# flash4242/Promptable-Counterfactual-GAN

Measured on AMD Instinct MI355X. Metric: images/sec (G+D step) MNIST-28 cDCGAN bs512 @1/2/4/8 MI355X; % MFMA roofline, higher is better.
Workload: dtype f32

## Files before the change

### include/pcgan_hip.h

```cpp
#ifndef PCGAN_HIP_H
#define PCGAN_HIP_H

#include <stddef.h>
#include <stdint.h>

#ifdef __cplusplus
extern "C" {
#endif

typedef void* pcg_stream_t;

typedef enum pcg_status {
  PCG_OK = 0,
  PCG_ERR_INVALID = -1,
  PCG_ERR_WORKSPACE = -2,
  PCG_ERR_LAUNCH = -3,
  PCG_ERR_UNSUPPORTED = -4
} pcg_status;

typedef enum pcg_act {
  PCG_ACT_NONE = 0,
  PCG_ACT_RELU = 1,
  PCG_ACT_LRELU = 2,
  PCG_ACT_TANH = 3,
// ... 96 lines not shown

size_t pcg_bn_workspace_bytes(int64_t rows, int32_t C);
int pcg_bn_train_stats(const float* x, int64_t rows, int32_t C, float eps, float momentum,
                       float* save_mean, float* save_invstd, float* running_mean, float* running_var,
                       int64_t* num_batches_tracked ,
                       void* workspace, size_t workspace_bytes, pcg_stream_t stream);
int pcg_bn_train_stats_coef(const float* x, int64_t rows, int32_t C, float eps, float momentum,
                            float* save_mean, float* save_invstd, float* running_mean, float* running_var,
                            int64_t* num_batches_tracked, const float* gamma, const float* beta, float* coef_out,
                            void* workspace, size_t workspace_bytes, pcg_stream_t stream);
int pcg_bn_apply_act(const float* x, int64_t rows, int32_t C, const float* mean, const float* invstd_or_var,
                     float var_eps, const float* gamma, const float* beta, int act, float slope,
                     const float* residual , float alpha ,
                     float* y, pcg_stream_t stream);
int pcg_bn_act_bwd(const float* dy, const float* x, const float* y , int64_t rows, int32_t C,
                   const float* mean, const float* invstd, const float* gamma,
                   int act, float slope, float dy_scale ,
                   float* dx, float* dgamma, float* dbeta, int accumulate,
                   void* workspace, size_t workspace_bytes, pcg_stream_t stream);
int pcg_bn_act_bwd_premask(const float* dy, const float* x, int64_t rows, int32_t C, const float* mean, const float* invstd,
                           const float* gamma, const float* beta, int act, float slope, float dy_scale, float* dx, float* dgamma,
                           float* dbeta, int accumulate, void* workspace, size_t workspace_bytes, pcg_stream_t stream);

size_t pcg_bn_bwd_partial_workspace_bytes(int32_t C);
int pcg_bn_bwd_partial(const float* dm, const float* x, int64_t rows, int32_t C, const float* mean, const float* invstd,
                       const float* gamma, const void* partial, int32_t nparts, float* dx, float* dgamma, float* dbeta,
                       int accumulate, void* workspace, size_t workspace_bytes, pcg_stream_t stream);

size_t pcg_bn_db_workspace_bytes(int64_t rows, int32_t C);
int pcg_bn_act_bwd_db(const float* dy, const float* x, const float* y , int64_t rows, int32_t C, const float* mean,
                      const float* invstd, const float* gamma, const float* beta , int act, float slope, float dy_scale,
                      float* dx, float* dgamma, float* dbeta, int accumulate, float* dcol, int accumulate_col, void* workspace,
                      size_t workspace_bytes, pcg_stream_t stream);
size_t pcg_bn_bwd_partial_db_workspace_bytes(int32_t C);
int pcg_bn_bwd_partial_db(const float* dm, const float* x, int64_t rows, int32_t C, const float* mean, const float* invstd,
                          const float* gamma, const void* partial, int32_t nparts, float dm_scale, float* dx, float* dgamma,
                          float* dbeta, int accumulate, float* dcol , int accumulate_col, void* workspace,
                          size_t workspace_bytes, pcg_stream_t stream);

int pcg_conv2d_fwd_bn_g(const pcg_conv_geom* g, const float* x, const float* w, const float* bias , float* y, float eps,
                        float momentum, float* save_mean , float* save_invstd ,
                        float* running_mean , float* running_var , int64_t* num_batches_tracked ,
                        int32_t groups, void* workspace , size_t workspace_bytes, pcg_stream_t stream);
int pcg_bn_apply_act_g(const float* x, int64_t rows, int32_t C, const float* mean , const float* invstd ,
                       const float* gamma, const float* beta, int act, float slope, float* y, int32_t groups, pcg_stream_t stream);
int32_t pcg_conv2d_dgrad_bn_phases(const pcg_conv_geom* g);
int pcg_conv2d_dgrad_bnbwd_g(const pcg_conv_geom* g, const float* dy, const float* w, const float* z_below, const float* mean,
                             const float* invstd, const float* gamma, const float* beta, int act, float slope, float* dx,
                             void* partial, size_t partial_bytes, int32_t groups, pcg_stream_t stream);
size_t pcg_bn_bwd_partial_g_workspace_bytes(int32_t C, int32_t groups);
int pcg_bn_bwd_partial_g(const float* dm, const float* x, int64_t rows, int32_t C, const float* mean, const float* invstd,
                         const float* gamma, const void* partial, int32_t nparts, int32_t nphases, float* dx, float* dgamma,
                         float* dbeta, int accumulate, int32_t groups, void* workspace, size_t workspace_bytes, pcg_stream_t stream);
size_t pcg_bn_act_bwd_g_workspace_bytes(int64_t rows, int32_t C, int32_t groups);
int pcg_bn_act_bwd_premask_g(const float* dy, const float* x, int64_t rows, int32_t C, const float* mean, const float* invstd,
                             const float* gamma, const float* beta, int act, float slope, float* dx, float* dgamma, float* dbeta,
                             int accumulate, int32_t groups, void* workspace, size_t workspace_bytes, pcg_stream_t stream);

int32_t pcg_conv2d_fwd_bnbwd_thin_ok(const pcg_conv_geom* g);
size_t pcg_conv2d_fwd_bnbwd_thin_workspace_bytes(const pcg_conv_geom* g);
int pcg_conv2d_fwd_bnbwd_thin(const pcg_conv_geom* g, const float* x, const float* w, const float* z_below, const float* mean,
                              const float* invstd, const float* gamma, const float* beta, int act, float slope, float* dz,
                              float* dgamma , float* dbeta , int accumulate, void* workspace,
                              size_t workspace_bytes, pcg_stream_t stream);
int32_t pcg_conv2d_dgrad_bnbwd_full_ok(const pcg_conv_geom* g, int32_t groups);
size_t pcg_conv2d_dgrad_bnbwd_full_workspace_bytes(const pcg_conv_geom* g, int32_t groups);
int pcg_conv2d_dgrad_bnbwd_full(const pcg_conv_geom* g, const float* dy, const float* w, const float* z_below, const float* mean,
                                const float* invstd, const float* gamma, const float* beta, int act, float slope, float* dz,
                                float* dgamma , float* dbeta , int accumulate, int32_t groups, void* workspace,
                                size_t workspace_bytes, pcg_stream_t stream);

int32_t pcg_conv2d_bnin_full_ok(const pcg_conv_geom* g, int32_t groups);
int pcg_conv2d_fwd_bnin_full(const pcg_conv_geom* g, const float* z, const float* mean, const float* invstd, const float* gamma,
                             const float* beta, int in_act, float in_slope, int32_t groups, const float* w, const float* bias ,
                             int act, float slope, float* y, pcg_stream_t stream);
int pcg_conv2d_wgrad_bnin_full(const pcg_conv_geom* g, const float* z, const float* mean, const float* invstd, const float* gamma,
                               const float* beta, int in_act, float in_slope, int32_t groups, const float* dy, float* dw, int accumulate,
                               void* workspace, size_t workspace_bytes, pcg_stream_t stream);

int pcg_act_fwd(const float* x, int64_t n, int act, float slope, float* y, pcg_stream_t stream);
int pcg_act_bwd(const float* dy, const float* y, int64_t n, int act, float slope, float* dx, pcg_stream_t stream);

int pcg_bce_fwd_bwd(const float* p, const float* target , float target_const,
                    int64_t n, float grad_scale, const float* grad_out_dev ,
                    float* loss , float* dp , pcg_stream_t stream);
int pcg_bce_pair(const float* p, int64_t n_half, float target0, float target1, const float* g0_dev ,
                 const float* g1_dev , const float* g2_dev , float* loss3 , float* dp ,
                 pcg_stream_t stream);
int pcg_bce_logits_fwd_bwd(const float* z, float target_const, int64_t n, float grad_scale,
                           const float* grad_out_dev , float* loss , float* dz ,
                           pcg_stream_t stream);

int pcg_adam_step(float* param, const float* grad, float* exp_avg, float* exp_avg_sq, int64_t n,
                  double lr, double beta1, double beta2, double eps, double weight_decay, int decoupled_wd,
                  int64_t step, pcg_stream_t stream);

int pcg_adam_step_capturable(float* param, const float* grad, float* exp_avg, float* exp_avg_sq, int64_t n,
                             double lr, double beta1, double beta2, double eps, double weight_decay, int decoupled_wd,
                             int64_t* step_counter_dev, float* hyper_scratch2_dev, pcg_stream_t stream);

int pcg_embed_concat_fwd(const float* x, const int64_t* idx, const float* table, const float* mask ,
                         float* out, int32_t B, int32_t HW, int32_t C, int32_t K, pcg_stream_t stream);
int pcg_embed_concat_bwd(const float* dinp, const int64_t* idx, float* dtable , float* dx ,
                         int32_t B, int32_t HW, int32_t C, int32_t K, int accumulate, pcg_stream_t stream);
int pcg_embed_table_grad(const float* dinp, const int64_t* idx, float* dtable, int32_t B, int32_t HW, int32_t C, int32_t ch, int32_t K,
                         int accumulate, pcg_stream_t stream);
// ... 688 lines not shown
```

### promptable-counterfactual-gan_amd/_lib.py

```python
import ctypes
import os

import torch

_HERE = os.path.dirname(os.path.abspath(__file__))
LIB_PATH = os.environ.get("PCG_LIB") or os.path.join(_HERE, "libpcgan_hip.so")

PCG_OK = 0
ACT_NONE, ACT_RELU, ACT_LRELU, ACT_TANH, ACT_SIGMOID = 0, 1, 2, 3, 4
(PLAN_GEMM_ACT, PLAN_GEMM, PLAN_LINEAR_WGRAD, PLAN_LINEAR_WGRAD_GROUPED, PLAN_MEAN, PLAN_ABS_MEAN, PLAN_CROSS_ENTROPY,
 PLAN_EMBED_CONCAT_BWD, PLAN_ACT, PLAN_ELEMENTWISE, PLAN_BN_COLREDUCE, PLAN_BN_APPLY, PLAN_BN_FINALIZE, PLAN_INSTNORM,
 PLAN_SPECTRAL_NORM) = range(15)
PLAN_EW_TABULAR, PLAN_EW_CF_OPS, PLAN_EW_POINTWISE, PLAN_EW_GATHER_CHANNEL = range(4)


class PcgError(RuntimeError):
    pass


class ConvGeom(ctypes.Structure):

    _fields_ = [(n, ctypes.c_int32) for n in ("B", "IH", "IW", "Cin", "OH", "OW", "Cout", "KH", "KW", "stride", "pad")]

    def key(self):
        return tuple(getattr(self, n) for n, _ in self._fields_)


_I, _P = ctypes.c_int32, ctypes.c_void_p


class HouseGDesc(ctypes.Structure):
    _fields_ = ([("fc_in_w", _I), ("fc_in_b", _I)] +
                [(n, _I * 5) for n in ("fc1_w", "fc1_b", "bn1_g", "bn1_b", "fc2_w", "fc2_b", "bn2_g", "bn2_b",
                                       "film_gamma_w", "film_gamma_b", "film_beta_w", "film_beta_b")] +
                [("cont_w", _I), ("cont_b", _I), ("head_w", _I * 8), ("head_b", _I * 8), ("seg", _I * 9)] +
                [(n, _I) for n in ("nheads", "ncont", "D", "NC", "hidden", "nblocks")])


class WgradItem(ctypes.Structure):
    _fields_ = [("dy", _P), ("x", _P), ("dW", _P), ("db", _P)] + [(n, _I) for n in ("ldy", "ldx", "O", "I", "accumulate_w", "accumulate_b",
                                                                                      "tile_x", "tile_y")]


class HouseGFwdArgs(ctypes.Structure):
    _fields_ = ([(n, _P) for n in ("params", "x", "onehot", "mask", "noise", "inp", "H", "Z1", "Z2", "P", "SM")] +
                [("running_mean", _P * 10), ("running_var", _P * 10), ("num_batches_tracked", _P * 10)] +
                [(n, _P) for n in ("cont", "logits", "soft", "hard")] + [("B", ctypes.c_int32)] +
                [(n, ctypes.c_float) for n in ("eps", "momentum", "tau", "res_scale")])


class HouseGBwdArgs(ctypes.Structure):
    _fields_ = ([(n, _P) for n in ("params", "grads", "onehot", "mask", "H", "Z1", "Z2", "SM", "soft", "d_cont", "d_logits", "d_samples",
                                   "DH", "DZ1", "DZ2", "A1", "DN1", "DG", "DB", "DZIN", "DL", "DC", "Q")] +
                [("B", ctypes.c_int32), ("accumulate", ctypes.c_int32), ("tau", ctypes.c_float), ("res_scale", ctypes.c_float)])


class InXform(ctypes.Structure):
    _fields_ = [("scale", _P), ("shift", _P), ("act", _I), ("slope", ctypes.c_float)]


class MoonsCfDesc(ctypes.Structure):
    _fields_ = ([(n, _I) for n in ("hidden", "clf_hidden", "B", "N", "nG", "nD", "nC", "nG_adam", "nD_adam")] +
                [("g_off", _I * 14), ("d_off", _I * 8), ("c_off", _I * 6)] +
                [(n, ctypes.c_double) for n in ("lr_G", "lr_D", "beta1", "beta2", "adam_eps")] +
                [(n, ctypes.c_float) for n in ("bn_eps", "bn_momentum", "sn_eps", "slope", "lambda_cls", "lambda_l1", "lambda_l2",
                                               "lambda_mask")])


class MoonsCfTrainArgs(ctypes.Structure):
    _fields_ = ([(n, _P) for n in ("X", "Y", "rows", "target_y", "mask", "g_flat", "d_flat", "c_flat", "g_exp_avg", "g_exp_avg_sq", "g_step",
                                   "d_exp_avg", "d_exp_avg_sq", "d_step")] +
                [("bn_mean", _P * 3), ("bn_var", _P * 3), ("bn_nbt", _P * 3), ("sn_u", _P * 4), ("sn_v", _P * 4)] +
                [("logs", _P), ("scratch", _P), ("scratch_bytes", ctypes.c_size_t)])


class MoonsCfFwdArgs(ctypes.Structure):
    _fields_ = ([(n, _I) for n in ("which", "train", "B")] + [(n, _P) for n in ("x", "onehot", "mask", "params")] +
                [("bn_mean", _P * 3), ("bn_var", _P * 3), ("bn_nbt", _P * 3), ("sn_u", _P * 4), ("sn_v", _P * 4)] +
                [("out0", _P), ("out1", _P), ("scratch", _P), ("scratch_bytes", ctypes.c_size_t)])


class MoonsCfEvalArgs(ctypes.Structure):
    _fields_ = ([("N", ctypes.c_int64), ("M", _I), ("T", _I), ("group", _I)] +
                [(n, _P) for n in ("x", "y", "masks", "target", "row_mask", "g_flat", "c_flat")] + [("bn_mean", _P * 3), ("bn_var", _P * 3)] +
                [(n, _P) for n in ("raw", "masked", "x_cf", "logits_cf", "logits_x", "pred_cf", "pred_x", "gain", "sums")])


class HouseCfEvalArgs(ctypes.Structure):
    _fields_ = ([("N", ctypes.c_int64)] + [(n, _I) for n in ("T", "group", "clamp_cls", "mask_rows")] + [("g_flat", _P), ("nG", _I)] +
                [("bn_mean", _P * 10), ("bn_var", _P * 10)] + [(n, ctypes.c_float) for n in ("bn_eps", "tau", "res_scale")] +
                [("col_src", _I * 17), ("norm_vals", _P), ("c_w_kmajor", ctypes.POINTER(ctypes.c_void_p)), ("c_bias", ctypes.POINTER(ctypes.c_void_p))] +
                [(n, _P) for n in ("x", "y", "target", "mask", "noise", "cont", "logits", "chosen", "masked", "x_cf", "x_cf_raw", "logits_cf",
                                   "logits_x", "pred_cf", "pred_x", "gain", "tile_sums", "class_sums", "class_counts")])


class PatchMaskBitsArgs(ctypes.Structure):
    _fields_ = [("bits", _P), ("mask", _P)] + [(n, _I) for n in ("n", "H", "W", "ps")]


class MnistCfEntryArgs(ctypes.Structure):
    _fields_ = [(n, _P) for n in ("x", "table", "mask", "target", "out")] + [(n, _I) for n in ("B", "T", "HW", "K", "mask_mode", "q0", "nq")]


class MnistCfTailArgs(ctypes.Structure):
    _fields_ = ([(n, _P) for n in ("c", "x", "mask", "x_cf", "raw", "masked", "sums")] + [("scale", ctypes.c_float)] +
                [(n, _I) for n in ("B", "T", "HW", "mask_mode", "q0", "nq")])

# ... 95 lines not shown
class DeltaGanEntryArgs(ctypes.Structure):
    _fields_ = ([(n, _P) for n in ("x", "y", "target", "y_host", "target_host", "table_g", "table_d", "g_in", "d_in", "labels_2b", "head_w",
                                   "head_w_packed")] + [(n, _I) for n in ("B", "HW", "K", "mode", "head_C", "head_P")])


class DeltaGanTailFwdArgs(ctypes.Structure):
    _fields_ = ([(n, _P) for n in ("x", "delta", "x_cf", "d_in", "loss_reg", "workspace")] + [("workspace_bytes", ctypes.c_size_t)] +
                [(n, _I) for n in ("B", "HW", "grid")])


class LogitHeadFwdArgs(ctypes.Structure):
    _fields_ = [(n, _P) for n in ("a", "w", "bias", "logits", "loss", "dlogit", "db", "workspace")] + [(n, _I) for n in ("R", "F", "mode")]


class LogitHeadBwdArgs(ctypes.Structure):
    _fields_ = [(n, _P) for n in ("a", "w", "dlogit", "da", "dw")] + [("slope", _F)] + [(n, _I) for n in ("R", "F", "dw_C", "dw_P")]


class DeltaGanTailBwdArgs(ctypes.Structure):
    _fields_ = ([(n, _P) for n in ("dD", "dC", "delta", "d_delta")] + [("lambda_cls", _F), ("reg_scale", _F)] +
                [(n, _I) for n in ("B", "HW", "dD_stride")])


class DeltaCfEntryArgs(ctypes.Structure):
    _fields_ = [(n, _P) for n in ("x", "table", "target", "target_host", "out")] + [(n, _I) for n in ("B", "T", "HW", "K", "q0", "nq")]


class DeltaCfTailArgs(ctypes.Structure):
    _fields_ = [(n, _P) for n in ("delta", "x", "x_cf", "sums")] + [(n, _I) for n in ("B", "T", "HW", "q0", "nq")]


class DeltaGanTargetDrawArgs(ctypes.Structure):
    _fields_ = [("target", _P), ("counter", _P), ("seed", ctypes.c_uint64), ("offset", ctypes.c_uint64), ("B", _I), ("K", _I)]


class ProbHeadFwdArgs(ctypes.Structure):
    _fields_ = ([(n, _P) for n in ("a", "w", "bias", "logits", "prob", "loss", "dlogit", "db", "workspace")] +
                [("workspace_bytes", ctypes.c_size_t), ("eps", _F)] + [(n, _I) for n in ("R", "F", "mode", "slabs")])


class LogEpsLossArgs(ctypes.Structure):
    _fields_ = [(n, _P) for n in ("p", "grad_out", "loss", "dp")] + [("eps", _F), ("R", _I), ("mode", _I)]


DELTA_GAN_BUILD, DELTA_GAN_REGATHER = 0, 1
LOGIT_HEAD_D, LOGIT_HEAD_G = 0, 1
DELTA_GAN_CHUNK = 1024
PROB_HEAD_D, PROB_HEAD_G = 0, 1
PROB_HEAD_MAX_SLABS = 16
CLASS_PICK_FIRST, CLASS_PICK_BEST = 0, 1
CLASS_PICK_KMAX = 64
CF_PANELS_GRID, CF_PANELS_PANELS = 0, 1

STRUCTS = {"pcg_conv_geom": ConvGeom, "pcg_in_xform": InXform, "pcg_wgrad_item": WgradItem, "pcg_sn_fwd_batch": SnFwdBatch,
           "pcg_sn_bwd_batch": SnBwdBatch, "pcg_house_g_desc": HouseGDesc, "pcg_house_g_fwd_args": HouseGFwdArgs,
           "pcg_house_g_bwd_args": HouseGBwdArgs, "pcg_house_critic_fwd_args": HouseCriticFwdArgs,
           "pcg_house_critic_bwd_args": HouseCriticBwdArgs, "pcg_house_cls_fwd_args": HouseClsFwdArgs, "pcg_house_cls_bwd_args": HouseClsBwdArgs,
           "pcg_house_res_fwd_args": HouseResFwdArgs, "pcg_house_res_bwd_args": HouseResBwdArgs, "pcg_house_loss_args": HouseLossArgs,
           "pcg_house_diag_args": HouseDiagArgs, "pcg_moons_cf_desc": MoonsCfDesc, "pcg_moons_cf_train_args": MoonsCfTrainArgs,
           "pcg_moons_cf_fwd_args": MoonsCfFwdArgs, "pcg_moons_cf_eval_args": MoonsCfEvalArgs,
           "pcg_house_cf_eval_args": HouseCfEvalArgs, "pcg_patch_mask_bits_args": PatchMaskBitsArgs,
           "pcg_mnist_cf_entry_args": MnistCfEntryArgs, "pcg_mnist_cf_tail_args": MnistCfTailArgs,
           "pcg_mnist_cf_score_args": MnistCfScoreArgs, "pcg_dense_bn": DenseBn,
           "pcg_dense_bn_bwd": DenseBnBwd, "pcg_moons_gan_desc": MoonsGanDesc, "pcg_moons_gan_train_args": MoonsGanTrainArgs,
           "pcg_moons_gan_fwd_args": MoonsGanFwdArgs, "pcg_moons_clf_fit_desc": MoonsClfFitDesc,
           "pcg_moons_clf_fit_args": MoonsClfFitArgs, "pcg_delta_gan_entry_args": DeltaGanEntryArgs,
           "pcg_delta_gan_tail_fwd_args": DeltaGanTailFwdArgs, "pcg_logit_head_fwd_args": LogitHeadFwdArgs,
           "pcg_logit_head_bwd_args": LogitHeadBwdArgs, "pcg_delta_gan_tail_bwd_args": DeltaGanTailBwdArgs,
           "pcg_delta_cf_entry_args": DeltaCfEntryArgs, "pcg_delta_cf_tail_args": DeltaCfTailArgs,
           "pcg_delta_gan_target_draw_args": DeltaGanTargetDrawArgs, "pcg_prob_head_fwd_args": ProbHeadFwdArgs,
           "pcg_log_eps_loss_args": LogEpsLossArgs}

_c = ctypes
_vp, _f, _i, _i64, _sz = _c.c_void_p, _c.c_float, _c.c_int, _c.c_int64, _c.c_size_t
_d = _c.c_double
_i32 = _c.c_int32
_gp = _c.POINTER(ConvGeom)
_xp = _c.POINTER(InXform)

PROTOTYPES = {
    "pcg_abi_version": (_i, []),
    "pcg_abi_struct_bytes": (_sz, [_c.c_char_p]),
    "pcg_last_error": (_c.c_char_p, []),
    "pcg_target_arch": (_c.c_char_p, []),
    "pcg_tune_set": (_i, [_c.c_char_p, _i32]),
    "pcg_debug_stamp_buffer": (_i, [_vp, _i64]),
    "pcg_conv_plan_describe": (_i, [_c.POINTER(ConvGeom), _i32, _i32, _c.c_char_p, _sz]),
    "pcg_launch_plan_describe": (_i, [_i32, _c.POINTER(_i64), _i32, _c.c_char_p, _sz]),
    "pcg_conv_scratch_parts_bytes": (_sz, []),
    "pcg_conv_scratch_arrivals_bytes": (_sz, []),
    "pcg_conv_set_scratch": (_i, [_vp, _vp, _sz, _vp, _sz]),
    "pcg_conv_reset_scratch": (_i, [_vp]),
    "pcg_conv_pixtab_bytes": (_sz, [_gp]),
    "pcg_conv_pixtab_register": (_i, [_gp, _vp, _sz, _vp]),
    "pcg_conv_cliptab_bytes": (_sz, [_gp]),
    "pcg_conv_cliptab_register": (_i, [_gp, _vp, _sz, _vp]),
    "pcg_conv_sched_model": (_d, [_vp, _i32]),
    "pcg_conv_pad_clip_query": (_i, [_gp, _i32, _i32, _i32, _vp, _vp, _vp, _vp]),
    "pcg_conv2d_fwd_bn_g": (_i, [_gp, _vp, _vp, _vp, _vp, _f, _f, _vp, _vp, _vp, _vp, _vp, _i32, _vp, _sz, _vp]),
    "pcg_bn_apply_act_g": (_i, [_vp, _i64, _i32, _vp, _vp, _vp, _vp, _i, _f, _vp, _i32, _vp]),
    "pcg_conv2d_dgrad_bn_phases": (_i32, [_gp]),
    "pcg_conv2d_dgrad_bnbwd_g": (_i, [_gp, _vp, _vp, _vp, _vp, _vp, _vp, _vp, _i, _f, _vp, _vp, _sz, _i32, _vp]),
    "pcg_bn_bwd_partial_g_workspace_bytes": (_sz, [_i32, _i32]),
    "pcg_bn_bwd_partial_g": (_i, [_vp, _vp, _i64, _i32, _vp, _vp, _vp, _vp, _i32, _i32, _vp, _vp, _vp, _i, _i32, _vp, _sz, _vp]),
    "pcg_bn_act_bwd_g_workspace_bytes": (_sz, [_i64, _i32, _i32]),
    "pcg_bn_act_bwd_premask_g": (_i, [_vp, _vp, _i64, _i32, _vp, _vp, _vp, _vp, _i, _f, _vp, _vp, _vp, _i, _i32, _vp, _sz, _vp]),
    "pcg_bce_pair": (_i, [_vp, _i64, _f, _f, _vp, _vp, _vp, _vp, _vp, _vp]),
# ... 21 lines not shown
    "pcg_conv2d_dgrad": (_i, [_gp, _vp, _vp, _vp, _vp, _vp, _sz, _vp]),
    "pcg_conv2d_fwd_act": (_i, [_gp, _vp, _vp, _vp, _i, _f, _vp, _vp, _sz, _vp]),
    "pcg_conv2d_dgrad_act": (_i, [_gp, _vp, _vp, _vp, _i, _f, _vp, _vp, _sz, _vp]),
    "pcg_conv2d_fwd_bn_workspace_bytes": (_sz, [_gp]),
    "pcg_conv2d_dgrad_bn_workspace_bytes": (_sz, [_gp]),
    "pcg_conv2d_fwd_bn": (_i, [_gp, _vp, _vp, _vp, _vp, _f, _f, _vp, _vp, _vp, _vp, _vp, _vp, _sz, _vp]),
    "pcg_conv2d_dgrad_bn": (_i, [_gp, _vp, _vp, _vp, _vp, _f, _f, _vp, _vp, _vp, _vp, _vp, _vp, _sz, _vp]),
    "pcg_conv2d_dgrad_mask": (_i, [_gp, _vp, _vp, _vp, _i, _f, _vp, _vp, _sz, _vp]),
    "pcg_conv2d_dgrad_mask_thin_ok": (_i32, [_gp]),
    "pcg_conv2d_xf_thin_ok": (_i32, [_gp]),
    "pcg_conv2d_fwd_add_mask": (_i, [_gp, _vp, _vp, _vp, _vp, _i, _f, _vp, _vp]),
    "pcg_conv2d_dgrad_add_mask": (_i, [_gp, _vp, _vp, _vp, _vp, _i, _f, _vp, _vp]),
    "pcg_conv2d_fwd_mask": (_i, [_gp, _vp, _vp, _vp, _i, _f, _vp, _vp, _sz, _vp]),
    "pcg_conv2d_dgrad_bnbwd": (_i, [_gp, _vp, _vp, _vp, _vp, _vp, _vp, _vp, _i, _f, _vp, _vp, _sz, _vp]),
    "pcg_conv2d_fwd_bnbwd": (_i, [_gp, _vp, _vp, _vp, _vp, _vp, _vp, _vp, _i, _f, _vp, _vp, _sz, _vp]),
    "pcg_conv2d_dgrad_add": (_i, [_gp, _vp, _vp, _vp, _vp, _vp, _sz, _vp]),
    "pcg_conv2d_fwd_bn_partial_rows": (_c.c_int32, [_gp]),
    "pcg_conv2d_dgrad_bn_partial_rows": (_c.c_int32, [_gp]),
    "pcg_bn_bwd_partial_workspace_bytes": (_sz, [_c.c_int32]),
    "pcg_bn_bwd_partial": (_i, [_vp, _vp, _i64, _c.c_int32, _vp, _vp, _vp, _vp, _c.c_int32, _vp, _vp, _vp, _i, _vp, _sz, _vp]),
    "pcg_conv2d_fwd_bn_xf": (_i, [_gp, _vp, _xp, _vp, _vp, _vp, _f, _f, _vp, _vp, _vp, _vp, _vp, _vp, _vp, _vp, _vp, _sz, _vp]),
    "pcg_conv2d_dgrad_bn_xf": (_i, [_gp, _vp, _xp, _vp, _vp, _vp, _f, _f, _vp, _vp, _vp, _vp, _vp, _vp, _vp, _vp, _vp, _sz, _vp]),
    "pcg_conv2d_fwd_xf": (_i, [_gp, _vp, _xp, _vp, _vp, _i, _f, _vp, _vp, _sz, _vp]),
    "pcg_conv2d_dgrad_xf": (_i, [_gp, _vp, _xp, _vp, _vp, _i, _f, _vp, _vp, _sz, _vp]),
    "pcg_conv2d_wgrad_xf": (_i, [_gp, _vp, _xp, _vp, _xp, _vp, _i, _vp, _sz, _vp]),
    "pcg_bn_train_stats_coef": (_i, [_vp, _i64, _c.c_int32, _f, _f, _vp, _vp, _vp, _vp, _vp, _vp, _vp, _vp, _vp, _sz, _vp]),
    "pcg_bn_db_workspace_bytes": (_sz, [_i64, _c.c_int32]),
    "pcg_bn_act_bwd_db": (_i, [_vp, _vp, _vp, _i64, _c.c_int32, _vp, _vp, _vp, _vp, _i, _f, _f, _vp, _vp, _vp, _i, _vp, _i, _vp, _sz, _vp]),
    "pcg_bn_bwd_partial_db_workspace_bytes": (_sz, [_c.c_int32]),
    "pcg_bn_bwd_partial_db": (_i, [_vp, _vp, _i64, _c.c_int32, _vp, _vp, _vp, _vp, _c.c_int32, _f, _vp, _vp, _vp, _i, _vp, _i, _vp, _sz, _vp]),
    "pcg_conv2d_dgrad_add_bnsum": (_i, [_gp, _vp, _vp, _vp, _vp, _vp, _vp, _f, _vp, _vp, _sz, _vp]),
    "pcg_conv2d_fwd_add": (_i, [_gp, _vp, _vp, _vp, _vp, _vp, _sz, _vp]),
    "pcg_conv2d_fwd_add_bnsum": (_i, [_gp, _vp, _vp, _vp, _vp, _vp, _vp, _f, _vp, _vp, _sz, _vp]),
    "pcg_conv_weight_adjoint": (_i, [_vp, _vp, _i32, _i32, _i32, _i32, _vp]),
    "pcg_conv_weight_adjoint_many": (_i, [_vp, _vp, _i32, _i32, _i32, _i32, _i32, _vp]),
    "pcg_house_losses": (_i, [_vp, _vp, _vp, _i64, _vp, _vp, _vp, _f, _f, _f, _f, _vp, _vp]),
    "pcg_dp_unique_id": (_i, [_vp]),
    "pcg_dp_init": (_i, [_vp, _i32, _i32]),
    "pcg_dp_world": (_i32, []),
    "pcg_dp_rank": (_i32, []),
    "pcg_dp_side_stream": (_vp, []),
    "pcg_dp_allreduce": (_i, [_vp, _i64, _vp]),
    "pcg_dp_allreduce_begin": (_i, [_vp, _i64, _i32, _vp]),
    "pcg_dp_record": (_i, [_i32]),
    "pcg_dp_allreduce_wait": (_i, [_i32, _vp]),
    "pcg_dp_allreduce_sum_f64": (_i, [_vp, _i64, _vp]),
    "pcg_dp_broadcast": (_i, [_vp, _i64, _i32, _vp]),
    "pcg_dp_sync_batchnorm": (_i, [_i32]),
    "pcg_dp_barrier": (_i, [_vp]),
    "pcg_dp_rccl_version": (_i32, []),
    "pcg_dp_shutdown": (_i, []),
    "pcg_conv2d_wgrad_workspace_bytes": (_sz, [_gp]),
    "pcg_conv2d_wgrad": (_i, [_gp, _vp, _vp, _vp, _i, _vp, _sz, _vp]),
    "pcg_colsum_workspace_bytes": (_sz, [_i64, _c.c_int32]),
    "pcg_colsum": (_i, [_vp, _i64, _c.c_int32, _vp, _i, _vp, _sz, _vp]),
    "pcg_bn_workspace_bytes": (_sz, [_i64, _c.c_int32]),
    "pcg_bn_train_stats": (_i, [_vp, _i64, _c.c_int32, _f, _f, _vp, _vp, _vp, _vp, _vp, _vp, _sz, _vp]),
    "pcg_bn_apply_act": (_i, [_vp, _i64, _c.c_int32, _vp, _vp, _f, _vp, _vp, _i, _f, _vp, _f, _vp, _vp]),
    "pcg_bn_act_bwd": (_i, [_vp, _vp, _vp, _i64, _c.c_int32, _vp, _vp, _vp, _i, _f, _f, _vp, _vp, _vp, _i, _vp, _sz, _vp]),
    "pcg_bn_act_bwd_premask": (_i, [_vp, _vp, _i64, _c.c_int32, _vp, _vp, _vp, _vp, _i, _f, _f, _vp, _vp, _vp, _i, _vp, _sz, _vp]),
    "pcg_embed_concat_fwd": (_i, [_vp, _vp, _vp, _vp, _vp, _c.c_int32, _c.c_int32, _c.c_int32, _c.c_int32, _vp]),
    "pcg_embed_concat_bwd": (_i, [_vp, _vp, _vp, _vp, _c.c_int32, _c.c_int32, _c.c_int32, _c.c_int32, _i, _vp]),
    "pcg_embed_table_grad": (_i, [_vp, _vp, _vp, _i32, _i32, _i32, _i32, _i32, _i, _vp]),
    "pcg_gather_channel": (_i, [_vp, _vp, _i32, _i32, _i32, _vp]),
    "pcg_axpby": (_i, [_vp, _f, _vp, _f, _vp, _i64, _vp]),
    "pcg_scale_mask_fwd": (_i, [_vp, _vp, _f, _vp, _vp, _i64, _vp]),
    "pcg_scale_mask_bwd": (_i, [_vp, _vp, _vp, _f, _vp, _i64, _vp]),
    "pcg_clamp_add_fwd": (_i, [_vp, _vp, _f, _f, _vp, _i64, _vp]),
    "pcg_clamp_add_bwd": (_i, [_vp, _vp, _vp, _f, _f, _vp, _i64, _vp]),
    "pcg_abs_mean_workspace_bytes": (_sz, []),
    "pcg_abs_mean_fwd": (_i, [_vp, _vp, _i, _i64, _vp, _vp, _sz, _vp]),
    "pcg_abs_mean_bwd": (_i, [_vp, _vp, _i, _i64, _vp, _f, _vp, _i, _vp]),
    "pcg_avgpool_fwd": (_i, [_vp, _vp, _c.c_int32, _c.c_int32, _c.c_int32, _vp]),
    "pcg_avgpool_bwd": (_i, [_vp, _vp, _c.c_int32, _c.c_int32, _c.c_int32, _vp]),
    "pcg_cross_entropy_fwd_bwd": (_i, [_vp, _vp, _c.c_int32, _c.c_int32, _f, _vp, _vp, _vp, _vp]),
    "pcg_act_fwd": (_i, [_vp, _i64, _i, _f, _vp, _vp]),
    "pcg_act_bwd": (_i, [_vp, _vp, _i64, _i, _f, _vp, _vp]),
    "pcg_bce_fwd_bwd": (_i, [_vp, _vp, _f, _i64, _f, _vp, _vp, _vp, _vp]),
    "pcg_bce_logits_fwd_bwd": (_i, [_vp, _f, _i64, _f, _vp, _vp, _vp, _vp]),
    "pcg_adam_step": (_i, [_vp, _vp, _vp, _vp, _i64, _d, _d, _d, _d, _d, _i, _i64, _vp]),
    "pcg_adam_step_capturable": (_i, [_vp, _vp, _vp, _vp, _i64, _d, _d, _d, _d, _d, _i, _vp, _vp, _vp]),
    "pcg_patch_mask": (_i, [_vp, _c.c_int32, _c.c_int32, _c.c_int32, _c.c_int32, _c.c_int32, _c.c_uint64, _c.c_uint64, _vp]),
    "pcg_randint": (_i, [_vp, _i64, _c.c_int32, _c.c_int32, _vp, _c.c_uint64, _c.c_uint64, _vp]),
    "pcg_randn": (_i, [_vp, _i64, _f, _f, _c.c_uint64, _c.c_uint64, _vp]),
    "pcg_fill": (_i, [_vp, _i64, _f, _vp]),
    "pcg_add_bias_rows": (_i, [_vp, _i64, _i32, _vp, _vp]),
    "pcg_sumsq": (_i, [_vp, _i64, _vp, _i, _vp]),
    "pcg_norm_sum": (_i, [_vp, _vp, _i32, _vp, _vp]),
    "pcg_instnorm_fwd": (_i, [_vp, _i32, _i32, _i32, _vp, _vp, _f, _i, _f, _vp, _vp, _vp, _vp]),
    "pcg_instnorm_bwd": (_i, [_vp, _vp, _i32, _i32, _i32, _vp, _vp, _vp, _vp, _vp, _vp, _vp]),
    "pcg_instnorm_bwd_bwd": (_i, [_vp, _vp, _vp, _i32, _i32, _i32, _vp, _vp, _vp, _vp, _vp, _vp, _vp]),
    "pcg_instnorm_bwd_fused": (_i, [_vp, _vp, _f, _vp, _i32, _i32, _i32, _vp, _vp, _vp, _vp, _vp, _vp, _vp, _vp, _vp, _vp]),
    "pcg_instnorm_bwd_bwd_act": (_i, [_vp, _vp, _vp, _i32, _i32, _i32, _vp, _vp, _vp, _vp, _f, _vp, _vp, _vp, _vp]),
    "pcg_rowsum3": (_i, [_i32, _vp, _vp, _i, _vp, _vp, _i, _vp, _vp, _i, _i32, _i32, _vp]),
    "pcg_nhwc_to_nchw_flat": (_i, [_vp, _vp, _i32, _i32, _i32, _i, _vp]),
    "pcg_interpolate": (_i, [_vp, _vp, _vp, _vp, _i32, _i32, _vp]),
    "pcg_interpolate_stack": (_i, [_vp, _vp, _vp, _vp, _i32, _i32, _vp]),
    "pcg_gradient_penalty_fwd": (_i, [_vp, _i32, _i32, _f, _vp, _vp, _vp]),
    "pcg_gradient_penalty_bwd": (_i, [_vp, _vp, _vp, _i32, _i32, _f, _vp, _vp]),
    "pcg_rand_uniform": (_i, [_vp, _i64, _c.c_uint64, _c.c_uint64, _vp]),
    "pcg_cross_entropy_weighted_fwd_bwd": (_i, [_vp, _vp, _vp, _i32, _i32, _f, _vp, _vp, _vp, _vp]),
    "pcg_dropout_apply": (_i, [_vp, _vp, _i64, _i32, _i32, _f, _vp, _vp]),
    "pcg_rand_bernoulli": (_i, [_vp, _i64, _f, _c.c_uint64, _c.c_uint64, _vp]),
    "pcg_resize8_normalize": (_i, [_vp, _i32, _i32, _i32, _i32, _i32, _vp, _vp, _i32, _vp, _vp, _i32, _f, _f, _vp, _vp]),
    "pcg_house_g_fwd": (_i, [_c.POINTER(HouseGDesc), _c.POINTER(HouseGFwdArgs), _vp]),
    "pcg_house_g_bwd": (_i, [_c.POINTER(HouseGDesc), _c.POINTER(HouseGBwdArgs), _vp]),
# ... 124 lines not shown
```

### promptable-counterfactual-gan_amd/csrc/batchnorm.hip

```cpp
#include "pcg_common.h"
#include "launch_plan.h"
#include <cstdlib>

namespace pcg {
bool dp_sync_bn();
int dp_world();
int dp_allreduce_f64(double* buf, int64_t n, hipStream_t s);

namespace {

constexpr int CR_THREADS = 256;
constexpr int CR_MAX_BLOCKS = 512;
constexpr int FIN_CH = 8, FIN_SL = 128;
static inline int fin_threads(int nparts) { return nparts <= 1024 ? FIN_CH * 32 : FIN_CH * FIN_SL; }

struct ColPlan { int vec, CG, TX, TY, nblocks, rows_per_block; };

ColPlan plan_cols(int64_t rows, int C, bool aligned16) {
  ColPlan p;
  p.vec = (C % 4 == 0 && aligned16) ? 4 : 1;
  p.CG = C / p.vec;
  int tx = 1;
  while (tx * 2 <= p.CG && tx * 2 <= CR_THREADS) tx *= 2;
  p.TX = tx;
  p.TY = CR_THREADS / tx;
  int64_t rpb = ceil_div64(rows, CR_MAX_BLOCKS);
  const int64_t min_rpb = (int64_t)p.TY * 4;
  if (rpb < min_rpb) rpb = min_rpb;
  p.rows_per_block = (int)rpb;
  p.nblocks = (int)ceil_div64(rows, rpb);
  if (p.nblocks < 1) p.nblocks = 1;
  return p;
}

template <int VEC>
__device__ __forceinline__ void ldv(const float* p, size_t idx, float (&v)[VEC]) {
  if constexpr (VEC == 4) {
    const float4 q = *reinterpret_cast<const float4*>(p + idx);
    v[0] = q.x; v[1] = q.y; v[2] = q.z; v[3] = q.w;
  } else {
    v[0] = p[idx];
  }
}
struct FnStats {
  static constexpr int NVAL = 2;
  const float* x;
  template <int VEC>
  __device__ __forceinline__ void eval(size_t idx, int c0, double (&o)[2][VEC]) const {
    (void)c0;
    float v[VEC];
    ldv<VEC>(x, idx, v);
#pragma unroll
    for (int e = 0; e < VEC; ++e) { o[0][e] = (double)v[e]; o[1][e] = (double)v[e] * (double)v[e]; }
  }
// ... 305 lines not shown
      float sc, sh;
      bn_fold(gamma ? gamma[c] : 1.f, beta ? beta[c] : 0.f, mean[c], is, sc, sh);
      v[e] = fmaf(alpha, act_apply(fmaf(v[e], sc, sh), act, slope), rs[e]);
    }
    if constexpr (VEC == 4) reinterpret_cast<float4*>(y)[i] = make_float4(v[0], v[1], v[2], v[3]);
    else y[i] = v[0];
  }
}

template <int VEC>
__global__ void __launch_bounds__(256) bn_bwd_apply_kernel(const float* __restrict__ dy, const float* __restrict__ x,
                                                           const float* __restrict__ y, size_t n, int C,
                                                           const float* __restrict__ mean, const float* __restrict__ invstd,
                                                           const float* __restrict__ coef, int act, float slope,
                                                           float dy_scale, float* __restrict__ dx, const float* __restrict__ gamma,
                                                           const float* __restrict__ beta) {
  const size_t nv = n / VEC;
  for (size_t i = (size_t)blockIdx.x * blockDim.x + threadIdx.x; i < nv; i += (size_t)gridDim.x * blockDim.x) {
    const int c0 = (int)((i * VEC) % (size_t)C);
    float g[VEC], xv[VEC], yv[VEC];
    if constexpr (VEC == 4) {
      const float4 a = reinterpret_cast<const float4*>(dy)[i];
      const float4 b = reinterpret_cast<const float4*>(x)[i];
      const float4 c = (act != PCG_ACT_NONE && y) ? reinterpret_cast<const float4*>(y)[i] : make_float4(1.f, 1.f, 1.f, 1.f);
      g[0] = a.x; g[1] = a.y; g[2] = a.z; g[3] = a.w;
      xv[0] = b.x; xv[1] = b.y; xv[2] = b.z; xv[3] = b.w;
      yv[0] = c.x; yv[1] = c.y; yv[2] = c.z; yv[3] = c.w;
    } else {
      g[0] = dy[i]; xv[0] = x[i]; yv[0] = (act != PCG_ACT_NONE && y) ? y[i] : 1.f;
    }
#pragma unroll
    for (int e = 0; e < VEC; ++e) {
      const int c = c0 + e;
      if (act != PCG_ACT_NONE && !y) { float sc, sh; bn_fold(gamma[c], beta[c], mean[c], invstd[c], sc, sh); yv[e] = fmaf(xv[e], sc, sh); }
      const float dz = dy_scale * g[e] * (act != PCG_ACT_NONE ? act_grad_from_out(yv[e], act, slope) : 1.f);
      const float xh = (xv[e] - mean[c]) * invstd[c];
      g[e] = coef[c] * (dz - coef[C + c] - xh * coef[2 * C + c]);
    }
    if constexpr (VEC == 4) reinterpret_cast<float4*>(dx)[i] = make_float4(g[0], g[1], g[2], g[3]);
    else dx[i] = g[0];
  }
}

struct BnTune { int blocks, depth, nt; size_t nt_bytes; };
static const BnTune& bn_tune() {
  static const BnTune t = [] {
    auto env = [](const char* k, int d) { const char* e = getenv(k); return e ? atoi(e) : d; };
    return BnTune{env("PCG_BN_BLOCKS", 4096), env("PCG_BN_DEPTH", 2), env("PCG_BN_NT", -1), (size_t)env("PCG_BN_NT_MB", 160) * 1000000u};
  }();
  return t;
}
static bool bn_use_nt(size_t n4) { const BnTune& t = bn_tune(); return t.nt < 0 ? n4 * 16 >= t.nt_bytes : t.nt != 0; }
static int bn_apply_depth() { return bn_tune().depth == 4 ? 4 : 2; }
template <bool NT>
__device__ __forceinline__ void bn_store4(float4* at, const float4& v) {
  typedef float nt_f32x4 __attribute__((ext_vector_type(4)));
  if constexpr (NT) __builtin_nontemporal_store(nt_f32x4{v.x, v.y, v.z, v.w}, reinterpret_cast<nt_f32x4*>(at)); else *at = v;
}

template <int DEPTH, bool NT>
__global__ void __launch_bounds__(256) bn_apply_act_fast_kernel(const float4* __restrict__ x, size_t n4, int C,
                                                                const float* __restrict__ mean, const float* __restrict__ invstd,
                                                                float var_eps, const float* __restrict__ gamma,
                                                                const float* __restrict__ beta, int act, float slope,
                                                                const float4* __restrict__ residual, float alpha,
                                                                float4* __restrict__ y, size_t group_n4) {
  if (group_n4) {
    const size_t g = blockIdx.y;
    x += g * group_n4; y += g * group_n4; if (residual) residual += g * group_n4;
    mean += g * C; invstd += g * C; n4 = group_n4;
  }
  const size_t gtid = (size_t)blockIdx.x * 256 + threadIdx.x, stride = (size_t)gridDim.x * 256;
  const int c0 = (int)(gtid % (size_t)(C >> 2)) * 4;
  float sc[4], sh[4];
#pragma unroll
  for (int e = 0; e < 4; ++e) {
    const int c = c0 + e;
    const float is = var_eps >= 0.f ? 1.f / sqrtf(invstd[c] + var_eps) : invstd[c];
    bn_fold(gamma ? gamma[c] : 1.f, beta ? beta[c] : 0.f, mean[c], is, sc[e], sh[e]);
  }
  auto one = [&](float4 q, float4 r) {
    q.x = fmaf(alpha, act_apply(fmaf(q.x, sc[0], sh[0]), act, slope), r.x);
    q.y = fmaf(alpha, act_apply(fmaf(q.y, sc[1], sh[1]), act, slope), r.y);
    q.z = fmaf(alpha, act_apply(fmaf(q.z, sc[2], sh[2]), act, slope), r.z);
    q.w = fmaf(alpha, act_apply(fmaf(q.w, sc[3], sh[3]), act, slope), r.w);
    return q;
  };
  const float4 zero = make_float4(0.f, 0.f, 0.f, 0.f);
  auto put = [&](size_t at, const float4& v) { bn_store4<NT>(y + at, v); };
  size_t i = gtid;
  for (; i + (DEPTH - 1) * stride < n4; i += DEPTH * stride) {
    float4 q[DEPTH], r[DEPTH];
#pragma unroll
    for (int j = 0; j < DEPTH; ++j) { q[j] = x[i + j * stride]; r[j] = residual ? residual[i + j * stride] : zero; }
#pragma unroll
    for (int j = 0; j < DEPTH; ++j) put(i + j * stride, one(q[j], r[j]));
  }
  for (; i < n4; i += stride) put(i, one(x[i], residual ? residual[i] : zero));
}
template <class... A>
static void launch_bn_apply_fast(dim3 grid, hipStream_t s, size_t n4_all, A... a) {
  const int depth = bn_apply_depth();
  const bool nt = bn_use_nt(n4_all);
  if (depth == 4 && nt) hipLaunchKernelGGL((bn_apply_act_fast_kernel<4, true>), grid, dim3(256), 0, s, a...);
  else if (depth == 4) hipLaunchKernelGGL((bn_apply_act_fast_kernel<4, false>), grid, dim3(256), 0, s, a...);
  else if (nt) hipLaunchKernelGGL((bn_apply_act_fast_kernel<2, true>), grid, dim3(256), 0, s, a...);
  else hipLaunchKernelGGL((bn_apply_act_fast_kernel<2, false>), grid, dim3(256), 0, s, a...);
}

template <bool NT>
__global__ void __launch_bounds__(256) bn_bwd_apply_fast_kernel(const float4* __restrict__ dy, const float4* __restrict__ x,
                                                                const float4* __restrict__ y, size_t n4, int C,
                                                                const float* __restrict__ mean, const float* __restrict__ invstd,
                                                                const float* __restrict__ coef, int act, float slope,
                                                                float dy_scale, float4* __restrict__ dx, const float* __restrict__ gamma,
                                                                const float* __restrict__ beta, double* __restrict__ colpart,
                                                                size_t group_n4) {
  if (group_n4) {
    const size_t g = blockIdx.y;
    dy += g * group_n4; x += g * group_n4; dx += g * group_n4; if (y) y += g * group_n4;
    mean += g * C; invstd += g * C; coef += g * 3 * C; n4 = group_n4;
  }
  const size_t gtid = (size_t)blockIdx.x * 256 + threadIdx.x, stride = (size_t)gridDim.x * 256;
  const int c0 = (int)(gtid % (size_t)(C >> 2)) * 4;
  float mu[4], is[4], k0[4], k1[4], k2[4], msc[4], msh[4];
  double cs[4] = {0.0, 0.0, 0.0, 0.0};
  const bool premask = act != PCG_ACT_NONE && y == nullptr;
#pragma unroll
  for (int e = 0; e < 4; ++e) {
    const int c = c0 + e;
    mu[e] = mean[c]; is[e] = invstd[c]; k0[e] = coef[c]; k1[e] = coef[C + c]; k2[e] = coef[2 * C + c];
    msc[e] = 0.f; msh[e] = 0.f;
    if (premask) bn_fold(gamma[c], beta[c], mean[c], invstd[c], msc[e], msh[e]);
  }
  const bool has_act = act != PCG_ACT_NONE;
  auto one = [&](float4 g, float4 xv, float4 yv) {
    float gg[4] = {g.x, g.y, g.z, g.w}, xx[4] = {xv.x, xv.y, xv.z, xv.w}, yy[4] = {yv.x, yv.y, yv.z, yv.w};
#pragma unroll
    for (int e = 0; e < 4; ++e) {
      if (premask) yy[e] = fmaf(xx[e], msc[e], msh[e]);
      const float grad = has_act ? act_grad_from_out(yy[e], act, slope) : 1.f;
      const float xh = (xx[e] - mu[e]) * is[e];
      gg[e] = k0[e] * fmaf(-xh, k2[e], fmaf(dy_scale * gg[e], grad, -k1[e]));
    }
    return make_float4(gg[0], gg[1], gg[2], gg[3]);
  };
  const float4 ones = make_float4(1.f, 1.f, 1.f, 1.f);
  auto tally = [&](const float4& v) { cs[0] += (double)v.x; cs[1] += (double)v.y; cs[2] += (double)v.z; cs[3] += (double)v.w; };
  size_t i = gtid;
  for (; i + stride < n4; i += 2 * stride) {
    const float4 g0 = dy[i], g1 = dy[i + stride], x0 = x[i], x1 = x[i + stride];
    const float4 y0 = (has_act && !premask) ? y[i] : ones, y1 = (has_act && !premask) ? y[i + stride] : ones;
    const float4 o0 = one(g0, x0, y0), o1 = one(g1, x1, y1);
    bn_store4<NT>(dx + i, o0);
    bn_store4<NT>(dx + i + stride, o1);
    if (colpart) { tally(o0); tally(o1); }
  }
  if (i < n4) {
    const float4 o = one(dy[i], x[i], (has_act && !premask) ? y[i] : ones);
    bn_store4<NT>(dx + i, o);
    if (colpart) tally(o);
  }
  if (colpart) {
    __shared__ double red[4][256];
#pragma unroll
    for (int e = 0; e < 4; ++e) red[e][threadIdx.x] = cs[e];
    __syncthreads();
    const int nq = C >> 2;
    if ((int)threadIdx.x < nq) {
#pragma unroll
      for (int e = 0; e < 4; ++e) {
        double sum = 0.0;
        for (int t = threadIdx.x; t < 256; t += nq) sum += red[e][t];
        colpart[(size_t)blockIdx.x * C + 4 * threadIdx.x + e] = sum;
      }
    }
  }
}

template <class... A>
static void launch_bn_bwd_apply_fast(dim3 grid, hipStream_t s, size_t n4_all, A... a) {
  if (bn_use_nt(n4_all)) hipLaunchKernelGGL((bn_bwd_apply_fast_kernel<true>), grid, dim3(256), 0, s, a...);
  else hipLaunchKernelGGL((bn_bwd_apply_fast_kernel<false>), grid, dim3(256), 0, s, a...);
}

bool fast_channels(int C) { return C % 4 == 0 && C / 4 <= 256 && ((C / 4) & (C / 4 - 1)) == 0; }

template <class Fn>
int launch_colreduce(const Fn& fn, int64_t rows, int C, const ColPlan& cp, double* partial, hipStream_t s) {
  if (cp.vec == 4)
    hipLaunchKernelGGL((colreduce_kernel<4, Fn>), dim3(cp.nblocks), dim3(CR_THREADS), 0, s, fn, rows, C, cp.CG, cp.TX, cp.TY,
                       cp.rows_per_block, partial);
  else
    hipLaunchKernelGGL((colreduce_kernel<1, Fn>), dim3(cp.nblocks), dim3(CR_THREADS), 0, s, fn, rows, C, cp.CG, cp.TX, cp.TY,
                       cp.rows_per_block, partial);
  return launch_status("colreduce_kernel");
}

unsigned ew_blocks(size_t nv) {
  size_t b = (nv + 255) / 256;
  if (b > 8192) b = 8192;
  if (b < 1) b = 1;
  return (unsigned)b;
}

bool al16(const void* p) { return ((uintptr_t)p & 15) == 0; }

constexpr int COL_MAX_BLOCKS = 4096;
constexpr int COL_SUM_BLOCKS = 1024;
enum { BN_PASS_APPLY = 0, BN_PASS_BWD = 1, BN_PASS_BWD_COLSUM = 2 };
enum { BN_LANES_FAST = 0, BN_LANES_FLOAT4 = 1, BN_LANES_SCALAR = 2 };
struct ApplyPlan { int lanes, depth; bool nt; unsigned blocks; };
ApplyPlan plan_apply(int pass, int64_t rows, int C, bool aligned) {
  const size_t n = (size_t)rows * C;
  if (fast_channels(C) && aligned) {
    const unsigned cap = pass == BN_PASS_APPLY ? (unsigned)bn_tune().blocks : pass == BN_PASS_BWD_COLSUM ? COL_SUM_BLOCKS : COL_MAX_BLOCKS;
    unsigned blocks = (unsigned)((n / 4 + 511) / 512);
    if (blocks > cap) blocks = cap;
    if (blocks < 1) blocks = 1;
    return ApplyPlan{BN_LANES_FAST, pass == BN_PASS_APPLY ? bn_apply_depth() : 2, bn_use_nt(n / 4), blocks};
  }
  if (C % 4 == 0 && aligned) return ApplyPlan{BN_LANES_FLOAT4, 1, false, ew_blocks(n / 4)};
  return ApplyPlan{BN_LANES_SCALAR, 1, false, ew_blocks(n)};
}

}
}

namespace pcg {
size_t bn_partial_buffer_bytes(int nparts, int C) {
  const PrePlan q = plan_presum(nparts);
  return (presum_offset(nparts, 2 * C) + (size_t)q.nchunks * 2 * C + 4 * (size_t)C) * sizeof(double);
}
int launch_bn_bwd_finalize(const double* partial, int nblocks, int64_t rows, int C, const float* gamma, const float* invstd, float* coef,
                           float* dgamma, float* dbeta, int accumulate, hipStream_t s) {
  PCG_REQUIRE(!dp_sync_bn(), "fused thin BatchNorm backward: not available in the exact global-batch mode");
  hipLaunchKernelGGL(bn_bwd_finalize_kernel<double>, dim3((C + FIN_CH - 1) / FIN_CH), dim3(fin_threads(nblocks)), 0, s, partial, nblocks, C,
                     1.0 / (double)rows, gamma, invstd, coef, dgamma, dbeta, accumulate, (const double*)nullptr);
  return launch_status("bn_bwd_finalize_kernel");
}
int launch_bn_bwd_finalize_g(const double* partial, int rows_per_group, int groups, int64_t rows_g, int C, const float* gamma, const float* invstd,
                             float* coef, float* dgamma, float* dbeta, int accumulate, hipStream_t s) {
  PCG_REQUIRE(!dp_sync_bn(), "fused thin BatchNorm backward: not available in the exact global-batch mode");
  hipLaunchKernelGGL(bn_bwd_finalize_g_kernel<double>, dim3((C + FIN_CH - 1) / FIN_CH), dim3(fin_threads(rows_per_group)), 0, s, partial,
                     rows_per_group, groups, rows_per_group, rows_per_group * groups, C, 1.0 / (double)rows_g, gamma, invstd, coef, dgamma, dbeta,
                     accumulate);
  return launch_status("bn_bwd_finalize_g_kernel");
}
int launch_bn_stats_finalize(const double* partial, int nparts, int64_t rows, int C, float eps, float momentum, float* save_mean,
                             float* save_invstd, float* running_mean, float* running_var, int64_t* nbt, hipStream_t s,
                             bool has_presum_tail, const float* gamma, const float* beta, float* coef) {
  int nchunks = 0;
  const double* pre = has_presum_tail ? launch_presum(partial, nparts, 2 * C, &nchunks, s) : nullptr;
  if (dp_sync_bn()) {
    PCG_REQUIRE(has_presum_tail, "exact BatchNorm: buffer without scratch tail");
    double* scratch = const_cast<double*>(partial) + presum_offset(nparts, 2 * C) + (size_t)plan_presum(nparts).nchunks * 2 * C;
    if (int e = sync_exchange(pre ? pre : partial, pre ? nchunks : nparts, C, scratch, s)) return e;
    partial = scratch + 2 * C; nparts = 1; pre = nullptr;
    rows *= dp_world();
  }
  const double unbias = rows > 1 ? (double)rows / (double)(rows - 1) : 1.0;
  if (pre)
    hipLaunchKernelGGL(bn_stats_finalize_kernel<double>, dim3((C + FIN_CH - 1) / FIN_CH), dim3(fin_threads(nchunks)), 0, s, pre, nchunks, C,
                       1.0 / (double)rows, unbias, eps, momentum, save_mean, save_invstd, running_mean, running_var, nbt, gamma, beta, coef);
  else
    hipLaunchKernelGGL(bn_stats_finalize_kernel<double>, dim3((C + FIN_CH - 1) / FIN_CH), dim3(fin_threads(nparts)), 0, s, partial, nparts, C,
                       1.0 / (double)rows, unbias, eps, momentum, save_mean, save_invstd, running_mean, running_var, nbt, gamma, beta, coef);
  return launch_status("bn_stats_finalize_kernel");
}
}

using namespace pcg;

extern "C" size_t pcg_bn_workspace_bytes(int64_t rows, int32_t C) {
  if (rows <= 0 || C <= 0) return 0;
  const ColPlan a = plan_cols(rows, C, true), b = plan_cols(rows, C, false);
  const int nb = a.nblocks > b.nblocks ? a.nblocks : b.nblocks;
  return ((size_t)nb * 2 * C + 4 * (size_t)C) * sizeof(double) + 3 * (size_t)C * sizeof(float);
}
// ... 99 lines not shown
    launch_bn_bwd_apply_fast(dim3(blocks), s, n / 4, reinterpret_cast<const float4*>(dy),
                             reinterpret_cast<const float4*>(x), reinterpret_cast<const float4*>(y), n / 4, C, mean, invstd,
                             (const float*)coef, act, slope, dy_scale, reinterpret_cast<float4*>(dx), gamma, beta, fused_col ? colpart : (double*)nullptr,
                             (size_t)0);
    if (fused_col) {
      if (int e = launch_status("bn_bwd_apply_kernel")) return e;
      hipLaunchKernelGGL(colsum_finalize_kernel, dim3((C + FIN_CH - 1) / FIN_CH), dim3(fin_threads((int)blocks)), 0, s, (const double*)colpart,
                         (int)blocks, C, dcol, accumulate_col);
      return launch_status("colsum_finalize_kernel");
    }
  } else if (ap.lanes == BN_LANES_FLOAT4)
    hipLaunchKernelGGL(bn_bwd_apply_kernel<4>, dim3(ap.blocks), dim3(256), 0, s, dy, x, y, n, C, mean, invstd,
                       (const float*)coef, act, slope, dy_scale, dx, gamma, beta);
  else
    hipLaunchKernelGGL(bn_bwd_apply_kernel<1>, dim3(ap.blocks), dim3(256), 0, s, dy, x, y, n, C, mean, invstd,
                       (const float*)coef, act, slope, dy_scale, dx, gamma, beta);
  if (int e = launch_status("bn_bwd_apply_kernel")) return e;
  if (dcol) {
    const ColPlan cq = plan_cols(rows, C, al16(dx));
    FnSum fs{dx};
    if (int e = launch_colreduce(fs, rows, C, cq, partial, s)) return e;
    hipLaunchKernelGGL(colsum_finalize_kernel, dim3((C + FIN_CH - 1) / FIN_CH), dim3(fin_threads(cq.nblocks)), 0, s, (const double*)partial, cq.nblocks, C,
                       dcol, accumulate_col);
    return launch_status("colsum_finalize_kernel");
  }
  return PCG_OK;
}

extern "C" int pcg_bn_act_bwd(const float* dy, const float* x, const float* y, int64_t rows, int32_t C, const float* mean,
                              const float* invstd, const float* gamma, int act, float slope, float dy_scale, float* dx,
                              float* dgamma, float* dbeta, int accumulate, void* workspace, size_t workspace_bytes,
                              pcg_stream_t stream) {
  PCG_REQUIRE(y || act == PCG_ACT_NONE, "pcg_bn_act_bwd: y is required with an activation (or use pcg_bn_act_bwd_premask)");
  return bn_act_bwd_impl(dy, x, y, rows, C, mean, invstd, gamma, nullptr, act, slope, dy_scale, dx, dgamma, dbeta, accumulate, workspace,
                         workspace_bytes, stream);
}

extern "C" int pcg_bn_act_bwd_premask(const float* dy, const float* x, int64_t rows, int32_t C, const float* mean, const float* invstd,
                                      const float* gamma, const float* beta, int act, float slope, float dy_scale, float* dx,
                                      float* dgamma, float* dbeta, int accumulate, void* workspace, size_t workspace_bytes,
                                      pcg_stream_t stream) {
  return bn_act_bwd_impl(dy, x, nullptr, rows, C, mean, invstd, gamma, beta, act, slope, dy_scale, dx, dgamma, dbeta, accumulate, workspace,
                         workspace_bytes, stream);
}

extern "C" size_t pcg_bn_bwd_partial_workspace_bytes(int32_t C) { return (size_t)3 * C * sizeof(float); }
extern "C" size_t pcg_bn_bwd_partial_db_workspace_bytes(int32_t C) {
  return C > 0 ? (((size_t)3 * C * sizeof(float) + 7) & ~(size_t)7) + (size_t)4096 * C * sizeof(double) : 0;
}

static int bn_bwd_partial_impl(const float* dm, const float* x, int64_t rows, int32_t C, const float* mean, const float* invstd,
                               const float* gamma, const void* partial_, int32_t nparts, float* dx, float* dgamma, float* dbeta,
                               int accumulate, void* workspace, size_t workspace_bytes, pcg_stream_t stream, float* dcol,
                               int accumulate_col, float dm_scale = 1.f) {
  const double* partial = static_cast<const double*>(partial_);
  PCG_REQUIRE(!dcol || workspace_bytes >= pcg_bn_bwd_partial_db_workspace_bytes(C),
              "pcg_bn_bwd_partial_db: workspace smaller than pcg_bn_bwd_partial_db_workspace_bytes");
  PCG_REQUIRE(dm && x && mean && invstd && partial && dx && rows > 0 && C > 0 && nparts > 0, "pcg_bn_bwd_partial: bad arguments");
  PCG_REQUIRE(((uintptr_t)partial & 7) == 0, "pcg_bn_bwd_partial: the partial-sum buffer must be 8-byte aligned");
  if (!workspace || workspace_bytes < pcg_bn_bwd_partial_workspace_bytes(C)) {
    set_error("pcg_bn_bwd_partial: workspace %zu B < required %zu B", workspace_bytes, pcg_bn_bwd_partial_workspace_bytes(C));
    return PCG_ERR_WORKSPACE;
  }
  hipStream_t s = (hipStream_t)stream;
  float* coef = (float*)workspace;
  int nchunks = 0;
  const double* pre = launch_presum(partial, nparts, 2 * C, &nchunks, s);
  const double* src = pre ? pre : partial;
  const double* local = nullptr;
  int nsrc = pre ? nchunks : nparts;
  int64_t rows_all = rows;
  if (dp_sync_bn()) {
    double* scratch = const_cast<double*>(partial) + presum_offset(nparts, 2 * C) + (size_t)plan_presum(nparts).nchunks * 2 * C;
    if (int e = sync_exchange(src, nsrc, C, scratch, s)) return e;
    src = scratch + 2 * C; nsrc = 1; local = scratch;
    rows_all = rows * dp_world();
  }
  hipLaunchKernelGGL(bn_bwd_finalize_kernel<double>, dim3((C + FIN_CH - 1) / FIN_CH), dim3(fin_threads(nsrc)), 0, s, src, nsrc, C,
                     1.0 / (double)rows_all, gamma, invstd, coef, dgamma, dbeta, accumulate, local);
  if (int e = launch_status("bn_bwd_finalize_kernel")) return e;
  const bool aligned = al16(dm) && al16(x) && al16(dx);
  const size_t n = (size_t)rows * C;
  double* colpart = reinterpret_cast<double*>(reinterpret_cast<char*>(workspace) + (((size_t)3 * C * sizeof(float) + 7) & ~(size_t)7));
  const ApplyPlan ap = plan_apply(dcol ? BN_PASS_BWD_COLSUM : BN_PASS_BWD, rows, C, aligned);
  if (ap.lanes == BN_LANES_FAST) {
    const unsigned blocks = ap.blocks;
    launch_bn_bwd_apply_fast(dim3(blocks), s, n / 4, reinterpret_cast<const float4*>(dm),
                             reinterpret_cast<const float4*>(x), (const float4*)nullptr, n / 4, C, mean, invstd, (const float*)coef, (int)PCG_ACT_NONE,
                             0.f, dm_scale, reinterpret_cast<float4*>(dx), gamma, (const float*)nullptr, dcol ? colpart : (double*)nullptr, (size_t)0);
    if (int e = launch_status("bn_bwd_apply_kernel")) return e;
    if (dcol) {
      hipLaunchKernelGGL(colsum_finalize_kernel, dim3((C + FIN_CH - 1) / FIN_CH), dim3(fin_threads((int)blocks)), 0, s, (const double*)colpart,
                         (int)blocks, C, dcol, accumulate_col);
      return launch_status("colsum_finalize_kernel");
    }
    return PCG_OK;
  } else if (ap.lanes == BN_LANES_FLOAT4)
    hipLaunchKernelGGL(bn_bwd_apply_kernel<4>, dim3(ap.blocks), dim3(256), 0, s, dm, x, (const float*)nullptr, n, C, mean, invstd,
                       (const float*)coef, PCG_ACT_NONE, 0.f, dm_scale, dx, gamma, (const float*)nullptr);
  else
    hipLaunchKernelGGL(bn_bwd_apply_kernel<1>, dim3(ap.blocks), dim3(256), 0, s, dm, x, (const float*)nullptr, n, C, mean, invstd,
                       (const float*)coef, PCG_ACT_NONE, 0.f, dm_scale, dx, gamma, (const float*)nullptr);
  if (int e = launch_status("bn_bwd_apply_kernel")) return e;
  if (dcol) {
    const ColPlan cq = plan_cols(rows, C, al16(dx));
    FnSum fs{dx};
    if (int e = launch_colreduce(fs, rows, C, cq, colpart, s)) return e;
    hipLaunchKernelGGL(colsum_finalize_kernel, dim3((C + FIN_CH - 1) / FIN_CH), dim3(fin_threads(cq.nblocks)), 0, s, (const double*)colpart, cq.nblocks, C,
                       dcol, accumulate_col);
    return launch_status("colsum_finalize_kernel");
  }
  return PCG_OK;
}

extern "C" int pcg_bn_bwd_partial(const float* dm, const float* x, int64_t rows, int32_t C, const float* mean, const float* invstd,
                                  const float* gamma, const void* partial, int32_t nparts, float* dx, float* dgamma, float* dbeta,
                                  int accumulate, void* workspace, size_t workspace_bytes, pcg_stream_t stream) {
  return bn_bwd_partial_impl(dm, x, rows, C, mean, invstd, gamma, partial, nparts, dx, dgamma, dbeta, accumulate, workspace, workspace_bytes,
                             stream, nullptr, 0);
}
extern "C" int pcg_bn_bwd_partial_db(const float* dm, const float* x, int64_t rows, int32_t C, const float* mean, const float* invstd,
                                     const float* gamma, const void* partial, int32_t nparts, float dm_scale, float* dx, float* dgamma,
                                     float* dbeta, int accumulate, float* dcol, int accumulate_col, void* workspace,
                                     size_t workspace_bytes, pcg_stream_t stream) {
  return bn_bwd_partial_impl(dm, x, rows, C, mean, invstd, gamma, partial, nparts, dx, dgamma, dbeta, accumulate, workspace, workspace_bytes,
                             stream, dcol, accumulate_col, dm_scale);
}
extern "C" size_t pcg_bn_db_workspace_bytes(int64_t rows, int32_t C) {
  return rows > 0 && C > 0 ? ((pcg_bn_workspace_bytes(rows, C) + 7) & ~(size_t)7) + colpart_bytes(C) : 0;
}
extern "C" int pcg_bn_act_bwd_db(const float* dy, const float* x, const float* y, int64_t rows, int32_t C, const float* mean,
                                 const float* invstd, const float* gamma, const float* beta, int act, float slope, float dy_scale, float* dx,
                                 float* dgamma, float* dbeta, int accumulate, float* dcol, int accumulate_col, void* workspace,
                                 size_t workspace_bytes, pcg_stream_t stream) {
  PCG_REQUIRE(dcol != nullptr, "pcg_bn_act_bwd_db: null column-sum output");
  return bn_act_bwd_impl(dy, x, y, rows, C, mean, invstd, gamma, beta, act, slope, dy_scale, dx, dgamma, dbeta, accumulate, workspace,
                         workspace_bytes, stream, dcol, accumulate_col);
}

namespace pcg {
int launch_bn_stats_finalize_g(const double* partial, int nparts, int nphases, int groups, int64_t rows_per_group, int C, float eps,
                               float momentum, float* save_mean, float* save_invstd, float* running_mean, float* running_var,
                               int64_t* nbt, hipStream_t s) {
  PCG_REQUIRE(!dp_sync_bn(), "grouped BatchNorm: not available in the exact global-batch mode (pcg_dp_sync_batchnorm)");
  PCG_REQUIRE(groups >= 1 && nphases >= 1 && nparts % (nphases * groups) == 0, "grouped BatchNorm: %d partial rows do not split into %d phases x %d groups", nparts, nphases, groups);
  int per_phase = nparts / nphases, seg = per_phase / groups;
  const GroupPre gp = launch_presum_g(&partial, nparts, 2 * C, &per_phase, &seg, s);
  (void)gp;
  const int rpg = seg * nphases;
  const double unbias = rows_per_group > 1 ? (double)rows_per_group / (double)(rows_per_group - 1) : 1.0;
  hipLaunchKernelGGL(bn_stats_finalize_g_kernel<double>, dim3((C + FIN_CH - 1) / FIN_CH), dim3(fin_threads(rpg)), 0, s, partial, rpg, groups,
                     seg, per_phase, C, 1.0 / (double)rows_per_group, unbias, eps, momentum, save_mean, save_invstd, running_mean, running_var, nbt);
  return launch_status("bn_stats_finalize_g_kernel");
}
}

static bool grouped_shape_ok(int64_t rows, int32_t C, int32_t groups) {
  return groups >= 1 && groups <= 8 && rows > 0 && rows % groups == 0 && fast_channels(C);
}
static unsigned grouped_apply_blocks(size_t n4_group) {
  unsigned blocks = (unsigned)((n4_group + 511) / 512);
  if (blocks > (unsigned)bn_tune().blocks) blocks = (unsigned)bn_tune().blocks;
  return blocks < 1 ? 1 : blocks;
}

extern "C" int pcg_bn_apply_act_g(const float* x, int64_t rows, int32_t C, const float* mean, const float* invstd, const float* gamma,
                                  const float* beta, int act, float slope, float* y, int32_t groups, pcg_stream_t stream) {
  PCG_REQUIRE(x && y && mean && invstd, "pcg_bn_apply_act_g: null pointer");
  PCG_REQUIRE(grouped_shape_ok(rows, C, groups) && al16(x) && al16(y),
              "pcg_bn_apply_act_g: needs rows %% groups == 0, C / 4 a power of two <= 256 and 16-byte aligned tensors (rows %lld, C %d, groups %d)",
              (long long)rows, C, groups);
  const size_t n4g = (size_t)(rows / groups) * C / 4;
  launch_bn_apply_fast(dim3(grouped_apply_blocks(n4g), groups), (hipStream_t)stream, n4g * groups,
                       reinterpret_cast<const float4*>(x), n4g, C, mean, invstd, -1.f, gamma, beta, act, slope, (const float4*)nullptr, 1.f,
                       reinterpret_cast<float4*>(y), n4g);
  return launch_status("bn_apply_act_fast_kernel");
}

extern "C" size_t pcg_bn_bwd_partial_g_workspace_bytes(int32_t C, int32_t groups) { return (size_t)3 * C * groups * sizeof(float); }

static int launch_bwd_finalize_apply_g(const float* dm, const float* x, int64_t rows, int32_t C, const float* mean, const float* invstd,
                                       const float* gamma, const float* beta, int act, float slope, const double* partial, int rpg, int seg,
                                       int seg_stride, float* dx, float* dgamma, float* dbeta, int accumulate, int32_t groups, float* coef,
                                       hipStream_t s) {
  const int64_t rows_g = rows / groups;
  hipLaunchKernelGGL(bn_bwd_finalize_g_kernel<double>, dim3((C + FIN_CH - 1) / FIN_CH), dim3(fin_threads(rpg)), 0, s, partial, rpg, groups, seg,
                     seg_stride, C, 1.0 / (double)rows_g, gamma, invstd, coef, dgamma, dbeta, accumulate);
  if (int e = launch_status("bn_bwd_finalize_g_kernel")) return e;
  const size_t n4g = (size_t)rows_g * C / 4;
  launch_bn_bwd_apply_fast(dim3(grouped_apply_blocks(n4g), groups), s, n4g * groups, reinterpret_cast<const float4*>(dm),
                           reinterpret_cast<const float4*>(x), (const float4*)nullptr, n4g, C, mean, invstd, (const float*)coef, act, slope, 1.f,
                           reinterpret_cast<float4*>(dx), gamma, beta, (double*)nullptr, n4g);
  return launch_status("bn_bwd_apply_fast_kernel");
}

extern "C" int pcg_bn_bwd_partial_g(const float* dm, const float* x, int64_t rows, int32_t C, const float* mean, const float* invstd,
                                    const float* gamma, const void* partial_, int32_t nparts, int32_t nphases, float* dx, float* dgamma,
                                    float* dbeta, int accumulate, int32_t groups, void* workspace, size_t workspace_bytes, pcg_stream_t stream) {
  const double* partial = static_cast<const double*>(partial_);
  PCG_REQUIRE(dm && x && mean && invstd && partial && dx && nparts > 0 && nphases > 0, "pcg_bn_bwd_partial_g: bad arguments");
  PCG_REQUIRE(grouped_shape_ok(rows, C, groups) && al16(dm) && al16(x) && al16(dx) && ((uintptr_t)partial & 7) == 0,
              "pcg_bn_bwd_partial_g: needs rows %% groups == 0, C / 4 a power of two <= 256 and aligned tensors (rows %lld, C %d, groups %d)",
              (long long)rows, C, groups);
  PCG_REQUIRE(nparts % (nphases * groups) == 0, "pcg_bn_bwd_partial_g: %d partial rows do not split into %d phases x %d groups", nparts, nphases, groups);
  PCG_REQUIRE(!dp_sync_bn(), "pcg_bn_bwd_partial_g: not available in the exact global-batch mode");
  if (!workspace || workspace_bytes < pcg_bn_bwd_partial_g_workspace_bytes(C, groups)) {
    set_error("pcg_bn_bwd_partial_g: workspace %zu B < required %zu B", workspace_bytes, pcg_bn_bwd_partial_g_workspace_bytes(C, groups));
    return PCG_ERR_WORKSPACE;
  }
  int per_phase = nparts / nphases, seg = per_phase / groups;
  (void)launch_presum_g(&partial, nparts, 2 * C, &per_phase, &seg, (hipStream_t)stream);
  return launch_bwd_finalize_apply_g(dm, x, rows, C, mean, invstd, gamma, nullptr, PCG_ACT_NONE, 0.f, partial, seg * nphases, seg, per_phase, dx,
                                     dgamma, dbeta, accumulate, groups, (float*)workspace, (hipStream_t)stream);
}

extern "C" size_t pcg_bn_act_bwd_g_workspace_bytes(int64_t rows, int32_t C, int32_t groups) {
  if (rows <= 0 || C <= 0 || groups <= 0 || rows % groups) return 0;
  const ColPlan a = plan_cols(rows / groups, C, true);
  return ((size_t)groups * a.nblocks * 2 * C) * sizeof(double) + (size_t)3 * C * groups * sizeof(float);
}
extern "C" int pcg_bn_act_bwd_premask_g(const float* dy, const float* x, int64_t rows, int32_t C, const float* mean, const float* invstd,
                                        const float* gamma, const float* beta, int act, float slope, float* dx, float* dgamma, float* dbeta,
                                        int accumulate, int32_t groups, void* workspace, size_t workspace_bytes, pcg_stream_t stream) {
  PCG_REQUIRE(dy && x && mean && invstd && gamma && beta && dx, "pcg_bn_act_bwd_premask_g: null pointer");
  PCG_REQUIRE(act == PCG_ACT_NONE || act == PCG_ACT_RELU || act == PCG_ACT_LRELU, "pcg_bn_act_bwd_premask_g: activation %d is not none / ReLU / LeakyReLU", act);
  PCG_REQUIRE(grouped_shape_ok(rows, C, groups) && al16(dy) && al16(x) && al16(dx) && ((rows / groups) * C) % 4 == 0,
              "pcg_bn_act_bwd_premask_g: needs rows %% groups == 0, C / 4 a power of two <= 256 and aligned tensors (rows %lld, C %d, groups %d)",
              (long long)rows, C, groups);
  PCG_REQUIRE(!dp_sync_bn(), "pcg_bn_act_bwd_premask_g: not available in the exact global-batch mode");
  const size_t need = pcg_bn_act_bwd_g_workspace_bytes(rows, C, groups);
  if (!workspace || workspace_bytes < need) { set_error("pcg_bn_act_bwd_premask_g: workspace %zu B < required %zu B", workspace_bytes, need); return PCG_ERR_WORKSPACE; }
  hipStream_t s = (hipStream_t)stream;
  const int64_t rows_g = rows / groups;
  const ColPlan cp = plan_cols(rows_g, C, true);
  double* partial = (double*)workspace;
  float* coef = reinterpret_cast<float*>(partial + (size_t)groups * cp.nblocks * 2 * C);
  for (int g = 0; g < groups; ++g) {
    const size_t off = (size_t)g * rows_g * C;
    FnBnBwd fn{dy + off, x + off, nullptr, mean + (size_t)g * C, invstd + (size_t)g * C, act, slope, 1.f, gamma, beta};
    if (int e = launch_colreduce(fn, rows_g, C, cp, partial + (size_t)g * cp.nblocks * 2 * C, s)) return e;
  }
  return launch_bwd_finalize_apply_g(dy, x, rows, C, mean, invstd, gamma, beta, act, slope, partial, cp.nblocks, cp.nblocks, cp.nblocks * groups,
                                     dx, dgamma, dbeta, accumulate, groups, coef, s);
}

extern "C" int pcg_colsum(const float* dy, int64_t rows, int32_t C, float* db, int accumulate, void* workspace,
                          size_t workspace_bytes, pcg_stream_t stream) {
  PCG_REQUIRE(dy && db && rows > 0 && C > 0, "pcg_colsum: bad arguments");
  if (!workspace || workspace_bytes < pcg_colsum_workspace_bytes(rows, C)) {
    set_error("pcg_colsum: workspace %zu B < required %zu B", workspace_bytes, pcg_colsum_workspace_bytes(rows, C));
    return PCG_ERR_WORKSPACE;
  }
  hipStream_t s = (hipStream_t)stream;
  const ColPlan cp = plan_cols(rows, C, al16(dy));
  double* partial = (double*)workspace;
  FnSum fn{dy};
  if (int e = launch_colreduce(fn, rows, C, cp, partial, s)) return e;
  hipLaunchKernelGGL(colsum_finalize_kernel, dim3((C + FIN_CH - 1) / FIN_CH), dim3(fin_threads(cp.nblocks)), 0, s, (const double*)partial, cp.nblocks, C, db, accumulate);
  return launch_status("colsum_finalize_kernel");
}

int pcg::describe_batchnorm_plan(int32_t op, const int64_t* a, int32_t n_args, char* buf, size_t bytes) {
  switch (op) {
    case PCG_PLAN_BN_COLREDUCE: {
      PCG_REQUIRE(n_args == 3 && a[0] > 0 && a[1] > 0 && a[1] <= INT32_MAX, "pcg_launch_plan_describe: bn_colreduce takes (rows, C, aligned)");
      const ColPlan p = plan_cols(a[0], (int)a[1], a[2] != 0);
// ... 37 lines not shown
```

### promptable-counterfactual-gan_amd/csrc/conv_igemm.hip

```cpp
#include <string.h>
#include <array>
#include <map>
#include <mutex>
#include "conv_loaders.h"
#include "conv_pixtab.h"
#include "conv_cliptab.h"
#include "thin_conv.h"

namespace pcg {
namespace {

__device__ __forceinline__ int wave_id() { return __builtin_amdgcn_readfirstlane((int)(threadIdx.x >> 6)); }

__device__ __forceinline__ void prio_entry(const ConvP& p) { if (p.edge_prio & 1) __builtin_amdgcn_s_setprio(3); }
__device__ __forceinline__ void prio_epilogue(const ConvP& p) { if (p.edge_prio & 2) __builtin_amdgcn_s_setprio(3); }

__device__ __forceinline__ int epi_group_off(const ConvP& p, int m_block) {
  return p.epi.group_rows > 0 ? __builtin_amdgcn_readfirstlane(m_block / p.epi.group_rows) * p.N : 0;
}

template <class Cfg, bool XF, bool CLIP = false>
__global__ void __launch_bounds__(IG_THREADS, Cfg::MINW) conv_fwd_kernel(ConvP p) {
  extern __shared__ __attribute__((aligned(16))) float smem[];
  prio_entry(p);
  if constexpr (CLIP) {
    uint32_t nt, idx;
    clip_block_tile(blockIdx.x, (uint32_t)p.tilesN, gridDim.x / (uint32_t)p.tilesN, p.clip_order, false, 0u, nt, idx);
    nt = __builtin_amdgcn_readfirstlane(nt); idx = __builtin_amdgcn_readfirstlane(idx);
    const ClipTile t = clip_tile(p, 0, idx, Cfg::BM);
    const int n_block = (int)nt * Cfg::BN;
    const int ktiles = t.nh * t.nw * ((p.Cin + IG_BK - 1) / IG_BK);
    if (wave_id() >= 4) {
      const int tid = threadIdx.x - IG_LOADERS;
      FwdALoader<Cfg::BM, XF, true> la(p, t, tid);
      FwdBLoader<Cfg::BN, true> lb(p, n_block, tid);
      lb.it.clip(t.h0, t.nh, t.w0, t.nw);
      igemm_produce<Cfg>(la, lb, ktiles, smem, tid, ClockStamp{p.stamps, p.stamp_slots});
      return;
    }
    f32x16 acc[Cfg::TM][Cfg::TN];
    ClockStamp cs{p.stamps, p.stamp_slots};
    cs.phase(0);
    igemm_consume<Cfg, true, true>(ktiles, acc, smem, cs);
    prio_epilogue(p);
    const size_t npix = (size_t)p.OH * p.OW;
    igemm_store_tile<Cfg>(acc, smem, n_block, p.N, p.bias, [&](int row) -> float* {
      const int b = t.img0 + row;
      return b < p.B ? p.out + ((size_t)b * npix + t.pos) * p.N + n_block : nullptr;
    }, p.stat_partial ? p.stat_partial + (size_t)t.stat_tile * Cfg::WAVES_M * 2 * p.N : nullptr, p.act, p.slope, &p.epi,
       p.epi.group_rows > 0 ? t.group * p.N : 0);
    cs.phase(3);
    return;
  }
  const uint32_t tile = xcd_remap(blockIdx.x, gridDim.x);
  const int mt = tile / p.tilesN, nt = tile % p.tilesN;
  const int m_block = mt * Cfg::BM, n_block = nt * Cfg::BN;
  const int kt_begin = blockIdx.y * p.ktiles_per_split;
  int ktiles = p.ktiles - kt_begin;
  if (ktiles > p.ktiles_per_split) ktiles = p.ktiles_per_split;

// ... 223 lines not shown
  const int nseg = sk_segments(sk, s0, s1);
  fwd_sk_segment<Cfg, XF>(p, sk, s0, smem);
  if (nseg == 1) return;
  lds_barrier();
  fwd_sk_segment<Cfg, XF>(p, sk, s1, smem);
}

template <class Cfg, bool XF>
__device__ __forceinline__ void dgrad_sk_segment(const ConvP& p, const DgradPhases& phases, const SkPlan& sk, const SkSeg& sg, int tiles_per_phase,
                                                 float* smem, int* rowpix) {
  const int py = __builtin_amdgcn_readfirstlane(sg.tile / tiles_per_phase), tile = sg.tile - py * tiles_per_phase;
  const PhaseInfo& f = phases.p[py];
  const int mt = __builtin_amdgcn_readfirstlane(tile / p.tilesN), nt = tile - mt * p.tilesN;
  const int m_block = mt * Cfg::BM, n_block = nt * Cfg::BN;
  if (wave_id() >= 4) {
    const int tid = threadIdx.x - IG_LOADERS;
    for (int r = tid; r < Cfg::BM; r += IG_LOADERS) {
      const int m = m_block + r;
      int pix = -1;
      if (m < f.Mp) {
        uint32_t t, cc, b, aa;
        f.dPHw.divmod((uint32_t)m, t, cc);
        f.dPHh.divmod(t, b, aa);
        pix = ((int)b * p.IH + (int)aa * p.stride + f.ph) * p.IW + (int)cc * p.stride + f.pw;
      }
      rowpix[r] = pix;
    }
    DgradALoader<Cfg::BM, XF> la(p, f, m_block, tid);
    DgradBLoader<Cfg::BN> lb(p, f, n_block, tid);
    if (sg.kt_begin) { la.seek(sg.kt_begin); lb.seek(sg.kt_begin); }
    igemm_produce<Cfg>(la, lb, sg.nkt, smem, tid, ClockStamp{nullptr, 0});
    return;
  }
  f32x16 acc[Cfg::TM][Cfg::TN];
  igemm_consume<Cfg, true, false>(sg.nkt, acc, smem);
  if (sk_combine<Cfg>(sk, sg, acc))
    igemm_store_tile<Cfg>(acc, smem, n_block, p.N, p.bias, [&](int row) -> float* {
      const int pix = rowpix[row];
      return pix >= 0 ? p.out + (size_t)pix * p.Cin + n_block : nullptr;
    }, p.stat_partial ? p.stat_partial + (size_t)(f.prow0 + mt * Cfg::WAVES_M) * 2 * p.N : nullptr, p.act, p.slope, &p.epi, epi_group_off(p, m_block));
}
template <class Cfg, bool XF>
__global__ void __launch_bounds__(IG_THREADS, Cfg::MINW) conv_dgrad_sk_kernel(ConvP p, DgradPhases phases, SkPlan sk, int tiles_per_phase) {
  extern __shared__ __attribute__((aligned(16))) float smem[];
  __shared__ int rowpix[Cfg::BM];
  SkSeg s0, s1{};
  const int nseg = sk_segments(sk, s0, s1);
  dgrad_sk_segment<Cfg, XF>(p, phases, sk, s0, tiles_per_phase, smem, rowpix);
  if (nseg == 1) return;
  lds_barrier();
  dgrad_sk_segment<Cfg, XF>(p, phases, sk, s1, tiles_per_phase, smem, rowpix);
}

template <class Cfg, bool XFA, bool XFB, bool TAB = false>
__global__ void __launch_bounds__(IG_THREADS, 4) conv_wgrad_kernel(ConvP p, int ktiles_total, int ktiles_per_split, int tiles,
                                                                   int slice_major) {
  extern __shared__ __attribute__((aligned(16))) float smem[];
  prio_entry(p);
  uint32_t tile, split;
  if (slice_major) {
    const uint32_t l = xcd_remap(blockIdx.x, gridDim.x);
    split = l / (uint32_t)tiles; tile = l - split * (uint32_t)tiles;
  } else {
    tile = xcd_remap(blockIdx.x, gridDim.x); split = blockIdx.y;
  }
  const int mt = tile / p.tilesN, nt = tile % p.tilesN;
  const int m_block = mt * Cfg::BM, n_block = nt * Cfg::BN;
  const int kt_begin = split * ktiles_per_split;
  int ktiles = ktiles_total - kt_begin;
  if (ktiles > ktiles_per_split) ktiles = ktiles_per_split;

  if (wave_id() >= 4) {
    const int tid = threadIdx.x - IG_LOADERS;
    WgradALoader<Cfg::BM, XFA> la(p, m_block, kt_begin, tid);
    WgradBLoader<Cfg::BN, XFB, TAB> lb(p, n_block, kt_begin, tid);
    igemm_produce<Cfg>(la, lb, ktiles, smem, tid, ClockStamp{p.stamps, p.stamp_slots});
    return;
  }
  f32x16 acc[Cfg::TM][Cfg::TN];
  igemm_consume<Cfg, false, false>(ktiles, acc, smem, ClockStamp{p.stamps, p.stamp_slots});
  prio_epilogue(p);
  float* slab = p.out + (size_t)split * (size_t)p.M * (size_t)p.N;
  igemm_store_tile<Cfg>(acc, smem, n_block, p.N, nullptr, [&](int row) -> float* {
    const int m = m_block + row;
    return m < p.M ? slab + (size_t)m * p.N + n_block : nullptr;
  });
}


struct SkNPlan {
  int nph, blocks, total;
  int tile0[5], it0[5], kt[4];
  float* parts; int* arrivals;
};
__device__ __forceinline__ int skn_start(int g, const SkNPlan& sk) {
  return __builtin_amdgcn_readfirstlane((int)((uint32_t)g * (uint32_t)sk.total / (uint32_t)sk.blocks));
}
__device__ __forceinline__ int skn_owner(int x, const SkNPlan& sk) {
  return __builtin_amdgcn_readfirstlane((int)((((uint32_t)x + 1u) * (uint32_t)sk.blocks - 1u) / (uint32_t)sk.total));
}
struct SkNSeg { int py, tin, t_begin, e, kt_begin, nkt, fb, nparts, mt, nt; };
__device__ __forceinline__ SkNSeg skn_segment(int it, int it1, const SkNPlan& sk, int tilesN) {
  SkNSeg s;
  s.py = 0;
  if (sk.nph > 1 && it >= sk.it0[1]) s.py = 1;
  if (sk.nph > 2 && it >= sk.it0[2]) s.py = 2;
  if (sk.nph > 3 && it >= sk.it0[3]) s.py = 3;
  const int KT = sk.kt[s.py], local = it - sk.it0[s.py];
  s.tin = __builtin_amdgcn_readfirstlane(local / KT);
  s.t_begin = sk.it0[s.py] + s.tin * KT;
  const int t_end = s.t_begin + KT;
  s.e = it1 < t_end ? it1 : t_end;
  s.kt_begin = it - s.t_begin; s.nkt = s.e - it;
  s.fb = skn_owner(s.t_begin, sk); s.nparts = skn_owner(t_end - 1, sk) - s.fb + 1;
  s.mt = __builtin_amdgcn_readfirstlane(s.tin / tilesN); s.nt = s.tin - s.mt * tilesN;
  return s;
}
template <class Cfg, bool XF>
__global__ void __launch_bounds__(IG_THREADS, Cfg::MINW) conv_dgrad_skn_kernel(ConvP p, DgradPhases phases, SkNPlan sk) {
  extern __shared__ __attribute__((aligned(16))) float smem[];
  __shared__ int rowpix[Cfg::BM];
  const int g = (int)xcd_remap(blockIdx.x, (uint32_t)sk.blocks);
  const int it1 = skn_start(g + 1, sk);
  if (wave_id() >= 4) {
    const int tid = threadIdx.x - IG_LOADERS;
#pragma unroll 1
    for (int it = skn_start(g, sk); it < it1;) {
      const SkNSeg sg = skn_segment(it, it1, sk, p.tilesN);
      const PhaseInfo& f = phases.p[sg.py];
      const int m_block = sg.mt * Cfg::BM, n_block = sg.nt * Cfg::BN;
      for (int r = tid; r < Cfg::BM; r += IG_LOADERS) {
        const int m = m_block + r;
        int pix = -1;
        if (m < f.Mp) {
          uint32_t t, cc, b, aa;
          f.dPHw.divmod((uint32_t)m, t, cc);
          f.dPHh.divmod(t, b, aa);
          pix = ((int)b * p.IH + (int)aa * p.stride + f.ph) * p.IW + (int)cc * p.stride + f.pw;
        }
// ... 108 lines not shown
    for (int kh = 0; kh < KH; ++kh) {
      const int th = (int)ih + pad - kh;
      if (th < 0 || th % stride) continue;
      const int oh = th / stride;
      if (oh >= OH) continue;
      for (int kw = 0; kw < KW; ++kw) {
        const int tw = (int)iw + pad - kw;
        if (tw < 0 || tw % stride) continue;
        const int ow = tw / stride;
        if (ow >= OW) continue;
        const float4 v = dcol[((size_t)(((int)b * OH + oh) * OW + ow) * (KH * KW) + (kh * KW + kw)) * CQ + cq];
        acc.x += v.x; acc.y += v.y; acc.z += v.z; acc.w += v.w;
      }
    }
    if (act != PCG_ACT_NONE) {
      acc.x = act_neg_scale(acc.x, neg); acc.y = act_neg_scale(acc.y, neg); acc.z = act_neg_scale(acc.z, neg); acc.w = act_neg_scale(acc.w, neg);
    }
    dx[idx] = acc;
  }
}

using Cfg128x128 = TileCfg<128, 128, 2, 2>;
#ifndef PCG_PAD_CLIP_DEFAULT
#define PCG_PAD_CLIP_DEFAULT 1
#endif
#ifndef PCG_TILE64_SWZ
#define PCG_TILE64_SWZ 1
#endif
using Cfg128x64P = TileCfg<128, 64, 2, 2>;
#if PCG_TILE64_SWZ
using Cfg128x64 = TileCfg<128, 64, 2, 2, true, 6, 1>;
#else
using Cfg128x64 = Cfg128x64P;
#endif

template <class C>
using Bf16Twin = TileCfg<C::BM, C::BN, C::WAVES_M, C::WAVES_N, false, C::MINW, C::PF, true>;


int check_geom(const pcg_conv_geom* g) {
  PCG_REQUIRE(g != nullptr, "conv geometry is null");
  PCG_REQUIRE(g->B > 0 && g->IH > 0 && g->IW > 0 && g->Cin > 0 && g->OH > 0 && g->OW > 0 && g->Cout > 0,
              "conv geometry: non-positive extent");
  PCG_REQUIRE(g->KH > 0 && g->KW > 0 && g->stride > 0 && g->pad >= 0, "conv geometry: bad kernel/stride/pad");
  PCG_REQUIRE(g->OH == (g->IH + 2 * g->pad - g->KH) / g->stride + 1 && g->OW == (g->IW + 2 * g->pad - g->KW) / g->stride + 1,
              "conv geometry: OH/OW inconsistent with IH/IW, kernel %dx%d stride %d pad %d", g->KH, g->KW, g->stride, g->pad);
  PCG_REQUIRE((int64_t)g->B * g->IH * g->IW * g->Cin * 4 < (1ll << 31) && (int64_t)g->B * g->OH * g->OW * g->Cout * 4 < (1ll << 31) &&
                  (int64_t)g->Cout * g->KH * g->KW * g->Cin * 4 < (1ll << 31),
              "conv geometry: an operand tensor reaches 2 GiB (32-bit buffer offsets); split the batch");
  PCG_REQUIRE(g->KH * g->KW <= 32, "conv geometry: more than 32 taps (%dx%d) unsupported", g->KH, g->KW);
  return PCG_OK;
}

struct Tune { int edge_prio = -1, dgrad_swz3 = -1, wgrad_rounds = -1, korder = -1, wgrad_order = -1, dgrad_interleave = -1, fwd_splits = -1, stream_k = -1, sk_blocks = -1, dgrad_gemm = -1, t64 = -1, wgrad_pixtab = -1, pad_clip = -1, pad_clip_dgrad = -1; unsigned long long* stamps = nullptr; int stamp_slots = 0; };
Tune g_tune;

ConvP make_params(const pcg_conv_geom* g) {
  ConvP p{};
  static const int korder_env = getenv("PCG_KORDER") ? atoi(getenv("PCG_KORDER")) : 1;
  p.korder = g_tune.korder >= 0 ? g_tune.korder : korder_env;
  static const int edge_env = getenv("PCG_EDGE_PRIO") ? atoi(getenv("PCG_EDGE_PRIO")) : 2;
  p.edge_prio = g_tune.edge_prio >= 0 ? g_tune.edge_prio : edge_env;
  p.stamps = g_tune.stamps; p.stamp_slots = g_tune.stamp_slots;
  p.B = g->B; p.IH = g->IH; p.IW = g->IW; p.Cin = g->Cin; p.OH = g->OH; p.OW = g->OW; p.Cout = g->Cout;
  p.KH = g->KH; p.KW = g->KW; p.stride = g->stride; p.pad = g->pad;
  p.dOW = FastDiv((uint32_t)g->OW);
  p.dOH = FastDiv((uint32_t)g->OH);
  p.dOHW = FastDiv((uint32_t)(g->OH * g->OW));
  p.x_bytes = (uint32_t)((int64_t)g->B * g->IH * g->IW * g->Cin * 4);
  p.dy_bytes = (uint32_t)((int64_t)g->B * g->OH * g->OW * g->Cout * 4);
  p.w_bytes = (uint32_t)((int64_t)g->Cout * g->KH * g->KW * g->Cin * 4);
  return p;
}

int set_xform(const char* who, const pcg_in_xform* xf, int C, ConvP* p) {
  if (!xf || !xf->scale) return PCG_OK;
  PCG_REQUIRE(xf->shift != nullptr, "%s: input transform without shift", who);
  PCG_REQUIRE(xf->act == PCG_ACT_NONE || xf->act == PCG_ACT_RELU || xf->act == PCG_ACT_LRELU,
              "%s: input transform activation %d is not none / ReLU / LeakyReLU", who, xf->act);
  PCG_REQUIRE(C % 4 == 0 && (((uintptr_t)xf->scale | (uintptr_t)xf->shift) & 15) == 0,
              "%s: input transform needs a channel count %% 4 == 0 and 16-byte aligned scale / shift", who);
  p->in_sc = xf->scale; p->in_sh = xf->shift; p->in_neg = act_neg_of(xf->act, xf->slope); p->in_c_bytes = (uint32_t)C * 4u;
  return PCG_OK;
}

template <class Cfg, bool AK, bool BK_>
constexpr size_t smem_bytes() {
  constexpr int a = igemm_smem_floats<Cfg, AK, BK_>(), b = epilogue_smem_floats<Cfg>();
  return sizeof(float) * (size_t)(a > b ? a : b);
}

template <class K>
int set_smem(K kernel, size_t bytes) {
  hipError_t e = hipFuncSetAttribute(reinterpret_cast<const void*>(kernel), hipFuncAttributeMaxDynamicSharedMemorySize, (int)bytes);
  if (e != hipSuccess) { set_error("hipFuncSetAttribute(max dynamic LDS=%zu): %s", bytes, hipGetErrorString(e)); return PCG_ERR_LAUNCH; }
  return PCG_OK;
}

constexpr int SK_MAX_BLOCKS = 512, SK_MAX_TILES = 4096;
constexpr size_t SK_PARTS_BYTES = (size_t)2 * SK_MAX_BLOCKS * 128 * 128 * sizeof(float);
constexpr size_t SK_ARRIVALS_BYTES = (size_t)SK_MAX_TILES * 4 * sizeof(int);
struct SkScratch { int device; hipStream_t stream; float* parts; int* arrivals; };
SkScratch g_sk_scratch[64];
int g_sk_scratch_n = 0;
std::mutex g_sk_mutex;
int current_device() { int d = 0; return hipGetDevice(&d) == hipSuccess ? d : 0; }
bool sk_scratch_of(hipStream_t s, SkPlan* sk) {
// ... 983 lines not shown
                                           const float* invstd, const float* gamma, const float* beta, int act, float slope, float* dz,
                                           float* dgamma, float* dbeta, int accumulate, int32_t groups, void* workspace, size_t workspace_bytes,
                                           pcg_stream_t stream) {
  if (int e = check_geom(g)) return e;
  PCG_REQUIRE(dy && w && z_below && mean && invstd && gamma && beta && dz, "pcg_conv2d_dgrad_bnbwd_full: null pointer");
  PCG_REQUIRE(act == PCG_ACT_NONE || act == PCG_ACT_RELU || act == PCG_ACT_LRELU, "pcg_conv2d_dgrad_bnbwd_full: activation %d is not none / ReLU / LeakyReLU", act);
  PCG_REQUIRE(pcg_conv2d_dgrad_bnbwd_full_ok(g, groups), "pcg_conv2d_dgrad_bnbwd_full: geometry / batch not eligible (pcg_conv2d_dgrad_bnbwd_full_ok)");
  PCG_REQUIRE((((uintptr_t)z_below | (uintptr_t)dz | (uintptr_t)w) & 15) == 0, "pcg_conv2d_dgrad_bnbwd_full: tensors must be 16-byte aligned");
  return thin_conv_dgrad_bnbwd_full(g, dy, w, z_below, mean, invstd, gamma, beta, act, slope, dz, dgamma, dbeta, accumulate, groups, workspace,
                                    workspace_bytes, (hipStream_t)stream);
}
extern "C" int32_t pcg_conv2d_bnin_full_ok(const pcg_conv_geom* g, int32_t groups) {
  return check_geom(g) == PCG_OK && thin_conv_bnin_full_ok(g, groups) ? 1 : 0;
}
static int bnin_args(const char* who, const pcg_conv_geom* g, const float* z, const float* mean, const float* invstd, const float* gamma, const float* beta,
                     int in_act, int32_t groups) {
  if (int e = check_geom(g)) return e;
  PCG_REQUIRE(z && mean && invstd && gamma && beta, "%s: null pointer", who);
  PCG_REQUIRE(in_act == PCG_ACT_NONE || in_act == PCG_ACT_RELU || in_act == PCG_ACT_LRELU, "%s: input activation %d is not none / ReLU / LeakyReLU", who, in_act);
  PCG_REQUIRE(pcg_conv2d_bnin_full_ok(g, groups), "%s: geometry / batch not eligible (pcg_conv2d_bnin_full_ok)", who);
  return PCG_OK;
}
extern "C" int pcg_conv2d_fwd_bnin_full(const pcg_conv_geom* g, const float* z, const float* mean, const float* invstd, const float* gamma,
                                        const float* beta, int in_act, float in_slope, int32_t groups, const float* w, const float* bias, int act,
                                        float slope, float* y, pcg_stream_t stream) {
  if (int e = bnin_args("pcg_conv2d_fwd_bnin_full", g, z, mean, invstd, gamma, beta, in_act, groups)) return e;
  PCG_REQUIRE(w && y && act >= PCG_ACT_NONE && act <= PCG_ACT_SIGMOID, "pcg_conv2d_fwd_bnin_full: bad arguments");
  const ThinBnIn bi{mean, invstd, gamma, beta, in_act, in_slope, groups};
  return thin_conv_fwd(g, z, w, bias, y, nullptr, 0, (hipStream_t)stream, act, slope, &bi);
}
extern "C" int pcg_conv2d_wgrad_bnin_full(const pcg_conv_geom* g, const float* z, const float* mean, const float* invstd, const float* gamma,
                                          const float* beta, int in_act, float in_slope, int32_t groups, const float* dy, float* dw, int accumulate,
                                          void* workspace, size_t workspace_bytes, pcg_stream_t stream) {
  if (int e = bnin_args("pcg_conv2d_wgrad_bnin_full", g, z, mean, invstd, gamma, beta, in_act, groups)) return e;
  PCG_REQUIRE(dy && dw, "pcg_conv2d_wgrad_bnin_full: null pointer");
  const ThinBnIn bi{mean, invstd, gamma, beta, in_act, in_slope, groups};
  return thin_conv_wgrad(g, z, dy, dw, accumulate, workspace, workspace_bytes, (hipStream_t)stream, nullptr, &bi);
}
extern "C" int32_t pcg_conv2d_fwd_bn_partial_rows(const pcg_conv_geom* g) { return check_geom(g) == PCG_OK ? fwd_stat_rows(g) : 0; }
extern "C" int32_t pcg_conv2d_dgrad_bn_partial_rows(const pcg_conv_geom* g) { return check_geom(g) == PCG_OK ? dgrad_stat_rows(g) : 0; }

extern "C" int pcg_slab_defer_begin(pcg_stream_t stream) { return slab_defer_begin((hipStream_t)stream); }
extern "C" int pcg_slab_defer_flush(pcg_stream_t stream) { return slab_defer_flush((hipStream_t)stream); }
extern "C" int32_t pcg_slab_defer_pending(void) { return slab_defer_pending(); }

extern "C" size_t pcg_conv2d_wgrad_workspace_bytes(const pcg_conv_geom* g) {
  if (check_geom(g) != PCG_OK) return 0;
  if (thin_is_cin(g) || thin_is_cout(g)) return thin_conv_wgrad_workspace_bytes(g);
  const WgradPlan w = plan_wgrad(g);
  return (size_t)w.splits * (size_t)g->Cout * (size_t)g->KH * g->KW * g->Cin * sizeof(float);
}

template <class Cfg, bool XFA, bool XFB, bool TAB = false>
static int launch_wgrad_x(const ConvP& p, const WgradPlan& wp, int slice_major, hipStream_t s) {
  if constexpr (!TAB) {
    if (p.pixtab) return launch_wgrad_x<Cfg, XFA, XFB, true>(p, wp, slice_major, s);
  }
  constexpr size_t smem = smem_bytes<Cfg, false, false>();
  static int once = set_smem(conv_wgrad_kernel<Cfg, XFA, XFB, TAB>, smem);
  if (once != PCG_OK) return once;
  hipLaunchKernelGGL((conv_wgrad_kernel<Cfg, XFA, XFB, TAB>), slice_major ? dim3((unsigned)wp.tiles * wp.splits) : dim3((unsigned)wp.tiles, wp.splits),
                     dim3(IG_THREADS), smem, s, p, wp.ktiles_total, wp.ktiles_per_split, wp.tiles, slice_major);
  return launch_status("conv_wgrad_kernel");
}
template <class Cfg, bool XFA, bool XFB, bool TAB = false>
static int launch_wgrad_sk_x(const ConvP& p, const SkPlan& sk, hipStream_t s) {
  if constexpr (!Cfg::BF16) {
    if (conv_bf16()) return launch_wgrad_sk_x<Bf16Twin<Cfg>, XFA, XFB>(p, sk, s);
  }
  if constexpr (!TAB) {
    if (p.pixtab) return launch_wgrad_sk_x<Cfg, XFA, XFB, true>(p, sk, s);
  }
  constexpr size_t smem = smem_bytes<Cfg, false, false>();
  static int once = set_smem(conv_wgrad_sk_kernel<Cfg, XFA, XFB, TAB>, smem);
  if (once != PCG_OK) return once;
  hipLaunchKernelGGL((conv_wgrad_sk_kernel<Cfg, XFA, XFB, TAB>), dim3((unsigned)(sk.dp_tiles + sk.sk_blocks)), dim3(IG_THREADS), smem, s, p, sk);
  return launch_status("conv_wgrad_sk_kernel");
}
template <class Cfg, bool TAB = false>
static int launch_wgrad192(const ConvP& p, const WgradPlan& wp, int slice_major, hipStream_t s) {
  if constexpr (!TAB) {
    if (p.pixtab) return launch_wgrad192<Cfg, true>(p, wp, slice_major, s);
  }
  constexpr size_t smem = smem_bytes<Cfg, false, false>();
  static int once = set_smem(conv_wgrad192_kernel<Cfg, TAB>, smem);
  if (once != PCG_OK) return once;
  hipLaunchKernelGGL((conv_wgrad192_kernel<Cfg, TAB>), slice_major ? dim3((unsigned)wp.tiles * wp.splits) : dim3((unsigned)wp.tiles, wp.splits),
                     dim3(IG_THREADS), smem, s, p, wp.ktiles_total, wp.ktiles_per_split, wp.tiles, slice_major);
  return launch_status("conv_wgrad192_kernel");
}
template <class Cfg>
static int launch_wgrad(const ConvP& p, const WgradPlan& wp, int slice_major, int xf_side, hipStream_t s) {
  if constexpr (!Cfg::BF16) {
    if (conv_bf16()) return launch_wgrad<Bf16Twin<Cfg>>(p, wp, slice_major, xf_side, s);
  }
  if (xf_side == 1) return launch_wgrad_x<Cfg, false, true>(p, wp, slice_major, s);
  if (xf_side == 2) return launch_wgrad_x<Cfg, true, false>(p, wp, slice_major, s);
  return launch_wgrad_x<Cfg, false, false>(p, wp, slice_major, s);
}

extern "C" int pcg_conv2d_wgrad_xf(const pcg_conv_geom* g, const float* x, const pcg_in_xform* xf_x, const float* dy,
                                   const pcg_in_xform* xf_dy, float* dw, int accumulate, void* workspace, size_t workspace_bytes,
                                   pcg_stream_t stream) {
  if (int e = check_geom(g)) return e;
  PCG_REQUIRE(x && dy && dw, "pcg_conv2d_wgrad: null pointer");
  const bool hx = xf_x && xf_x->scale, hy = xf_dy && xf_dy->scale;
  PCG_REQUIRE(!(hx && hy), "pcg_conv2d_wgrad_xf: at most one operand can carry an input transform");
  if (thin_is_cin(g) || thin_is_cout(g)) {
    PCG_REQUIRE(!hx && (!hy || thin_conv_xf_ok(g)), "pcg_conv2d_wgrad: input transforms on the MFMA path (Cin > 3 and Cout > 3) and, on the dy side, on the thin forms of pcg_conv2d_xf_thin_ok only");
    PCG_REQUIRE(!hy || (xf_dy->act == PCG_ACT_NONE || xf_dy->act == PCG_ACT_RELU || xf_dy->act == PCG_ACT_LRELU), "pcg_conv2d_wgrad: transform activation %d", hy ? xf_dy->act : 0);
    const ThinXf tx{hy ? xf_dy->scale : nullptr, hy ? xf_dy->shift : nullptr, hy ? act_neg_of(xf_dy->act, xf_dy->slope) : 1.f};
    return thin_conv_wgrad(g, x, dy, dw, accumulate, workspace, workspace_bytes, (hipStream_t)stream, &tx);
  }
  PCG_REQUIRE(g->Cin % 4 == 0 && g->Cout % 4 == 0, "pcg_conv2d_wgrad: Cin=%d and Cout=%d must be multiples of 4", g->Cin, g->Cout);
  const WgradPlan wp = plan_wgrad(g);
  const size_t need = pcg_conv2d_wgrad_workspace_bytes(g);
  if (workspace == nullptr || workspace_bytes < need) {
    set_error("pcg_conv2d_wgrad: workspace %zu B < required %zu B", workspace_bytes, need);
    return PCG_ERR_WORKSPACE;
  }
  PCG_REQUIRE(((uintptr_t)workspace & 15) == 0 && ((uintptr_t)dw & 15) == 0, "pcg_conv2d_wgrad: workspace/dw must be 16-byte aligned");
  ConvP p = make_params(g);
  p.x = x; p.dy = dy; p.out = (float*)workspace;
  p.M = g->Cout; p.N = g->KH * g->KW * g->Cin;
  p.tilesN = ceil_div(p.N, 128);
  p.pixtab = pixtab_of(g);
  if (int e = hx ? set_xform("pcg_conv2d_wgrad_xf", xf_x, g->Cin, &p) : set_xform("pcg_conv2d_wgrad_xf", xf_dy, g->Cout, &p)) return e;
  hipStream_t s = (hipStream_t)stream;
  static const int order_env0 = getenv("PCG_WGRAD_ORDER") ? atoi(getenv("PCG_WGRAD_ORDER")) : -1;
  const int order_env = g_tune.wgrad_order >= 0 ? g_tune.wgrad_order : order_env0;
  const int slice_major = order_env >= 0 ? order_env : (wp.tiles <= 8 ? 1 : 0);
  const int side = hx ? 1 : hy ? 2 : 0;
  if (!wp.narrow && !wp.wide192 && wp.tiles > 96 && sk_mode() != 0) {
    SkPlan sk{};
    bool take = plan_sk(wp.tiles, wp.ktiles_total, s, &sk);
    if (!take && wp.splits == 1) { sk = SkPlan{wp.tiles, 0, 0, wp.ktiles_total, nullptr, nullptr}; take = true; }
    if (take) {
      p.out = dw;
      if (accumulate) { p.epi.mode = EPI_ADD; p.epi.neg = 1.f; p.epi.delta_bytes = 0; }
      return side == 1 ? launch_wgrad_sk_x<Cfg128x128, false, true>(p, sk, s)
           : side == 2 ? launch_wgrad_sk_x<Cfg128x128, true, false>(p, sk, s) : launch_wgrad_sk_x<Cfg128x128, false, false>(p, sk, s);
    }
  }
  int rc;
  if (wp.wide192 && side == 0) {
    p.tilesN = p.N / 192;
    rc = conv_bf16() ? launch_wgrad192<Bf16Twin<Cfg64x192>>(p, wp, slice_major, s) : launch_wgrad192<Cfg64x192>(p, wp, slice_major, s);
  } else {
    WgradPlan wq = wp;
    if (wp.wide192) {
      wq.wide192 = false;
      wq.tiles = ceil_div(p.M, 64) * ceil_div(p.N, 128);
    }
    rc = wq.narrow ? launch_wgrad<TileCfg<64, 128, 1, 4>>(p, wq, slice_major, side, s) : launch_wgrad<Cfg128x128>(p, wq, slice_major, side, s);
  }
  if (rc != PCG_OK) return rc;
  const size_t n = (size_t)p.M * p.N;
  return launch_slab_reduce((const float*)workspace, dw, n, n, wp.splits, accumulate, s, true);
}

extern "C" int pcg_conv2d_wgrad(const pcg_conv_geom* g, const float* x, const float* dy, float* dw, int accumulate,
                                void* workspace, size_t workspace_bytes, pcg_stream_t stream) {
  return pcg_conv2d_wgrad_xf(g, x, nullptr, dy, nullptr, dw, accumulate, workspace, workspace_bytes, stream);
}

extern "C" int pcg_conv_plan_describe(const pcg_conv_geom* g, int32_t op, int32_t assume_scratch, char* out, size_t out_bytes) {
  if (int e = check_geom(g)) return e;
  PCG_REQUIRE(out && out_bytes > 0 && op >= 0 && op <= 2, "pcg_conv_plan_describe: bad arguments");
  const int have = assume_scratch ? (sk_mode() != 0 ? 1 : 0) : (have_sk_scratch() ? 1 : 0);
  char buf[512];
  buf[0] = 0;
  auto say = [&](const char* fmt, auto... a) { snprintf(buf + strlen(buf), sizeof(buf) - strlen(buf), fmt, a...); };
  if (thin_is_cin(g) || thin_is_cout(g)) {
    say("%s", "thin (Cin or Cout <= 3): no matrix-core launch");
  } else if (op == 0) {
    const int M = g->B * g->OH * g->OW, N = g->Cout, kt = g->KH * g->KW * ceil_div(g->Cin, IG_BK);
    const FwdPlan f = plan_fwd(g, have);
    SkPlan sk{};
    if (N <= 64) say("128x64 tiles: %d", ceil_div(M, 128));
    else if (fwd_use_t64(M, N, f.splits)) say("64x128 tiles: %d", ceil_div(M, 64) * ceil_div(N, 128));
    else if (f.splits == 1 && have && plan_sk_shape(ceil_div(M, 128) * ceil_div(N, 128), kt, &sk))
      say("stream-K: %d whole tiles + %d tiles x %d k-tiles over %d ranges", sk.dp_tiles, sk.sk_tiles, kt, sk.sk_blocks);
    else if (f.splits > 1) say("128x128 tiles: %d x %d K-slices of %d k-tiles (slabs)", ceil_div(M, 128) * ceil_div(N, 128), f.splits, f.ktiles_per_split);
    else say("128x128 tiles: %d", ceil_div(M, 128) * ceil_div(N, 128));
  } else if (op == 1) {
    if (dgrad_as_gemm(g, have)) {
      const int M = g->B * g->OH * g->OW, N = g->KH * g->KW * g->Cin, kt = ceil_div(g->Cout, IG_BK), tiles = ceil_div(M, 128) * ceil_div(N, 128);
      SkPlan sk{};
      say("%s", "GEMM + col2im: ");
      if (have && plan_sk_shape(tiles, kt, &sk)) say("stream-K: %d whole tiles + %d tiles x %d k-tiles over %d ranges", sk.dp_tiles, sk.sk_tiles, kt, sk.sk_blocks);
      else say("128x128 tiles: %d", tiles);
    } else {
      DgradPhases ph{};
      int maxMp = 0;
      const int nph = build_phases(g, &ph, &maxMp);
      const int N = g->Cin, tilesN = ceil_div(N, N > 64 ? 128 : 64);
      bool uniform = true;
      for (int i = 0; i < nph; ++i)
        uniform = uniform && ph.p[i].Mp == ph.p[0].Mp && ph.p[i].nth * ph.p[i].ntw == ph.p[0].nth * ph.p[0].ntw && ph.p[i].nth > 0 && ph.p[i].ntw > 0;
      SkNPlan sn{};
      SkPlan sk{};
      say("%d phase%s: ", nph, nph == 1 ? "" : "s");
      if (N > 64 && have && !uniform && plan_skn_shape(ph, nph, 128, tilesN, g->Cout, &sn))
        say("stream-K over unequal phases: %d tiles, %d k-tile iterations over %d ranges", sn.tile0[nph], sn.total, sn.blocks);
      else if (N > 64 && have && uniform && nph > 0 &&
               plan_sk_shape(ceil_div(maxMp, 128) * tilesN * nph, ph.p[0].nth * ph.p[0].ntw * ceil_div(g->Cout, IG_BK), &sk))
        say("stream-K: %d whole tiles + %d tiles over %d ranges", sk.dp_tiles, sk.sk_tiles, sk.sk_blocks);
      else say("%s tiles: %d per phase", N > 64 ? "128x128" : "128x64", ceil_div(maxMp, 128) * tilesN);
    }
  } else {
    const WgradPlan w = plan_wgrad(g);
    SkPlan sk{};
    if (!w.narrow && !w.wide192 && w.tiles > 96 && have && plan_sk_shape(w.tiles, w.ktiles_total, &sk))
      say("stream-K: %d whole tiles + %d tiles x %d k-tiles over %d ranges, dw written by the epilogue", sk.dp_tiles, sk.sk_tiles, w.ktiles_total, sk.sk_blocks);
    else if (!w.narrow && !w.wide192 && w.tiles > 96 && w.splits == 1 && sk_mode() != 0) say("128x128 tiles: %d, dw written by the epilogue", w.tiles);
    else say("%s tiles: %d x %d K-slices of %d k-tiles (slabs + slab_reduce)", w.wide192 ? "64x192" : w.narrow ? "64x128" : "128x128", w.tiles, w.splits, w.ktiles_per_split);
  }
  snprintf(out, out_bytes, "%s", buf);
  return PCG_OK;
}

extern "C" int pcg_conv_pad_clip_query(const pcg_conv_geom* g, int32_t op, int32_t groups, int32_t assume_scratch, int32_t* taken,
                                       int32_t* order, int32_t* tile_rows, double* predicted) {
  if (int e = check_geom(g)) return e;
  PCG_REQUIRE((op == 0 || op == 1) && groups >= 1, "pcg_conv_pad_clip_query: bad arguments");
  const int have = assume_scratch && sk_mode() != 0 ? 1 : 0;
  ClipPlan cp{false, 0, 0, 1.0};
  if (mfma_layer(g) && op == 0) {
    const int M = g->B * g->OH * g->OW, N = g->Cout, kt = g->KH * g->KW * ceil_div(g->Cin, IG_BK);
    const FwdPlan f = plan_fwd(g, have);
    const bool t64 = fwd_use_t64(M, N, f.splits);
    SkPlan sk{};
    const bool plain = f.splits == 1 && !(N > 64 && !t64 && have && plan_sk_shape(ceil_div(M, 128) * ceil_div(N, 128), kt, &sk));
    cp = clip_fwd_plan(g, groups, t64, plain);
  } else if (mfma_layer(g) && g->stride <= 2 && !dgrad_as_gemm(g, have)) {
    DgradPhases ph{};
    int maxMp = 0;
    const int nph = build_phases(g, &ph, &maxMp);
    SkPlan sk{};
    const bool plain = nph == 4 && !(g->Cin > 64 && have && plan_sk_shape(ceil_div(maxMp, 128) * ceil_div(g->Cin, 128) * nph, 4 * ceil_div(g->Cout, IG_BK), &sk));
    const uint32_t w_bytes = (uint32_t)((int64_t)g->Cout * g->KH * g->KW * g->Cin * 4);
    cp = clip_dgrad_plan(g, groups, dgrad_interleaved(w_bytes, ph, nph), plain);
  }
  if (taken) *taken = cp.take && cliptab_of(g) ? 1 : 0;
  if (order) *order = cp.order;
  if (tile_rows) *tile_rows = cp.bm;
  if (predicted) *predicted = cp.ratio;
  return PCG_OK;
}

extern "C" int pcg_tune_set(const char* name, int32_t value) {
  PCG_REQUIRE(name != nullptr, "pcg_tune_set: null name");
  if (!strcmp(name, "korder")) g_tune.korder = value;
  else if (!strcmp(name, "edge_prio")) g_tune.edge_prio = value;
  else if (!strcmp(name, "dgrad_swz3")) g_tune.dgrad_swz3 = value;
  else if (!strcmp(name, "wgrad_rounds")) g_tune.wgrad_rounds = value;
  else if (!strcmp(name, "wgrad_order")) g_tune.wgrad_order = value;
  else if (!strcmp(name, "dgrad_interleave")) g_tune.dgrad_interleave = value;
  else if (!strcmp(name, "fwd_splits")) g_tune.fwd_splits = value;
  else if (!strcmp(name, "stream_k")) g_tune.stream_k = value;
  else if (!strcmp(name, "sk_blocks")) g_tune.sk_blocks = value;
  else if (!strcmp(name, "dgrad_gemm")) g_tune.dgrad_gemm = value;
  else if (!strcmp(name, "t64")) g_tune.t64 = value;
  else if (!strcmp(name, "wgrad_pixtab")) g_tune.wgrad_pixtab = value;
  else if (!strcmp(name, "pad_clip")) g_tune.pad_clip = value;
  else if (!strcmp(name, "pad_clip_dgrad")) {
    PCG_REQUIRE(value >= -1 && value <= 2, "pcg_tune_set: pad_clip_dgrad is 0, 1 or 2 (-1: built-in), not %d", (int)value);
    g_tune.pad_clip_dgrad = value;
  }
  else {
    set_error("pcg_tune_set: unknown switch '%s' (korder, edge_prio, dgrad_swz3, wgrad_rounds, wgrad_order, dgrad_interleave, fwd_splits, "
              "stream_k, sk_blocks, dgrad_gemm, t64); the loader switches wgrad_pixtab, pad_clip and pad_clip_dgrad are accepted as well", name);
    return PCG_ERR_INVALID;
  }
  return PCG_OK;
}

extern "C" int pcg_debug_stamp_buffer(void* buf, int64_t bytes) {
  g_tune.stamps = static_cast<unsigned long long*>(buf);
  g_tune.stamp_slots = buf ? (int)(bytes / 16) : 0;
#ifdef PCG_CLOCK_STAMP
  return 1;
#else
  return 0;
#endif
}
```

### promptable-counterfactual-gan_amd/csrc/runtime.hip

```cpp
#include "pcg_common.h"
#include <stdarg.h>
#include <stdio.h>
#include <string.h>

namespace pcg {
namespace {
thread_local char g_err[512] = "";
thread_local int32_t g_conv_prec = PCG_PREC_F32;
}

bool conv_bf16() { return g_conv_prec == PCG_PREC_BF16; }

void set_error(const char* fmt, ...) {
  va_list ap;
  va_start(ap, fmt);
  vsnprintf(g_err, sizeof(g_err), fmt, ap);
  va_end(ap);
}

int launch_status(const char* what) {
  const hipError_t e = hipGetLastError();
  if (e == hipSuccess) return PCG_OK;
  set_error("%s: launch failed: %s", what, hipGetErrorString(e));
  return PCG_ERR_LAUNCH;
}
}

extern "C" int pcg_abi_version(void) { return 6; }
extern "C" size_t pcg_abi_struct_bytes(const char* name) {
#define PCG_STRUCT(T) {#T, sizeof(T)}
  static const struct { const char* name; size_t bytes; } table[] = {
      PCG_STRUCT(pcg_conv_geom), PCG_STRUCT(pcg_in_xform), PCG_STRUCT(pcg_wgrad_item), PCG_STRUCT(pcg_sn_fwd_batch), PCG_STRUCT(pcg_sn_bwd_batch),
      PCG_STRUCT(pcg_house_g_desc), PCG_STRUCT(pcg_house_g_fwd_args), PCG_STRUCT(pcg_house_g_bwd_args), PCG_STRUCT(pcg_house_critic_fwd_args),
      PCG_STRUCT(pcg_house_critic_bwd_args), PCG_STRUCT(pcg_house_cls_fwd_args), PCG_STRUCT(pcg_house_cls_bwd_args),
      PCG_STRUCT(pcg_house_res_fwd_args), PCG_STRUCT(pcg_house_res_bwd_args), PCG_STRUCT(pcg_house_loss_args), PCG_STRUCT(pcg_house_diag_args),
      PCG_STRUCT(pcg_moons_cf_desc), PCG_STRUCT(pcg_moons_cf_train_args), PCG_STRUCT(pcg_moons_cf_fwd_args), PCG_STRUCT(pcg_moons_cf_eval_args),
      PCG_STRUCT(pcg_house_cf_eval_args), PCG_STRUCT(pcg_patch_mask_bits_args), PCG_STRUCT(pcg_mnist_cf_entry_args),
      PCG_STRUCT(pcg_mnist_cf_tail_args), PCG_STRUCT(pcg_mnist_cf_score_args),
      PCG_STRUCT(pcg_dense_bn), PCG_STRUCT(pcg_dense_bn_bwd), PCG_STRUCT(pcg_moons_gan_desc), PCG_STRUCT(pcg_moons_gan_train_args),
      PCG_STRUCT(pcg_moons_gan_fwd_args), PCG_STRUCT(pcg_moons_clf_fit_desc), PCG_STRUCT(pcg_moons_clf_fit_args),
      PCG_STRUCT(pcg_delta_gan_entry_args), PCG_STRUCT(pcg_delta_gan_tail_fwd_args), PCG_STRUCT(pcg_logit_head_fwd_args),
      PCG_STRUCT(pcg_logit_head_bwd_args), PCG_STRUCT(pcg_delta_gan_tail_bwd_args), PCG_STRUCT(pcg_delta_cf_entry_args),
      PCG_STRUCT(pcg_delta_cf_tail_args), PCG_STRUCT(pcg_delta_gan_target_draw_args), PCG_STRUCT(pcg_prob_head_fwd_args),
      PCG_STRUCT(pcg_log_eps_loss_args)};
#undef PCG_STRUCT
  if (name)
    for (const auto& t : table)
      if (!strcmp(t.name, name)) return t.bytes;
  return 0;
}
extern "C" const char* pcg_last_error(void) { return pcg::g_err; }
extern "C" const char* pcg_target_arch(void) { return "gfx950"; }
extern "C" int pcg_conv_precision_set(int32_t precision) {
  PCG_REQUIRE(precision == PCG_PREC_F32 || precision == PCG_PREC_BF16, "pcg_conv_precision_set: unknown precision %d (0 fp32, 1 bf16)", precision);
  pcg::g_conv_prec = precision;
  return PCG_OK;
}
extern "C" int32_t pcg_conv_precision_get(void) { return pcg::g_conv_prec; }
```

### promptable-counterfactual-gan_amd/nn.py

```python
import contextlib
import functools
import os

import torch
import torch.nn as nn

from . import ops
from ._lib import ACT_LRELU, ACT_NONE, ACT_RELU, ACT_SIGMOID, ACT_TANH, PcgError


def _pad4(n):
    return (n + 3) // 4 * 4


def in_conv_precision(fn):
    @functools.wraps(fn)
    def run(self, *args, **kwargs):
        with ops.conv_precision(self.conv_precision):
            return fn(self, *args, **kwargs)
    return run


class FlatModule(nn.Module):

# ... 226 lines not shown
        if isinstance(m, nn.BatchNorm2d):
            if b.bn is not None or b.act != ACT_NONE:
                raise PcgError("expected conv -> [BatchNorm2d] -> [activation]")
            if not m.affine or not m.track_running_stats or m.momentum is None:
                raise PcgError(f"unsupported BatchNorm2d configuration: {m}")
            b.bn = m
        elif isinstance(m, nn.LeakyReLU):
            b.act, b.slope = ACT_LRELU, float(m.negative_slope)
        elif isinstance(m, nn.ReLU):
            b.act = ACT_RELU
        elif isinstance(m, nn.Tanh):
            b.act = ACT_TANH
        elif isinstance(m, nn.Sigmoid):
            b.act = ACT_SIGMOID
        else:
            raise PcgError(f"layer {type(m).__name__} has no libpcgan_hip implementation")
    if not blocks:
        raise PcgError("empty network")
    return blocks


class _WgradDefer:

    def __init__(self, side, main):
        self.side, self.main, self.job, self.inflight = side, main, None, False

    def submit(self, fn, tensors):
        self.job = (fn, tensors)

    def start_pending(self):
        if self.job is None:
            return
        fn, tensors = self.job
        self.job = None
        self.side.wait_stream(self.main)
        for t in tensors:
            t.record_stream(self.side)
        with torch.cuda.stream(self.side):
            fn()
        self.inflight = True

    def join(self):
        if self.inflight:
            self.main.wait_stream(self.side)
            self.inflight = False

    def finish(self):
        if self.job is not None:
            fn, _ = self.job
            self.job = None
            self.join()
            fn()
        self.join()


class _SeqFn(torch.autograd.Function):

    @staticmethod
    def forward(ctx, net, x, *params):
        y, saved = net._run_forward(x)
        ctx.net, ctx.saved = net, saved
        return y

    @staticmethod
    def backward(ctx, dy):
        need_x = ctx.needs_input_grad[1]
        need_p = any(ctx.needs_input_grad[2:])
        dx = ctx.net._run_backward(ctx.saved, dy, need_x, need_p)
        return (None, dx) + (None,) * (len(ctx.needs_input_grad) - 2)


class _SeqGroupFn(torch.autograd.Function):

    @staticmethod
    def forward(ctx, net, ngroups, *rest):
        xs = rest[:ngroups]
        y, saved = net._run_forward_groups(xs)
        ctx.net, ctx.saved, ctx.ngroups = net, saved, ngroups
        return y

    @staticmethod
    def backward(ctx, dy):
        if any(ctx.needs_input_grad[2:2 + ctx.ngroups]):
            raise PcgError("forward_groups: gradients w.r.t. the inputs are not implemented (detach them: the D step of mnist_dcgan.py:159)")
        if any(ctx.needs_input_grad[2 + ctx.ngroups:]):
            ctx.net._run_backward_groups(ctx.saved, dy)
        return (None,) * len(ctx.needs_input_grad)


class SequentialConvNet(FlatModule):

    fuse_backward_epilogue = True
    fold_bn_apply = False
    fold_bn_apply_thin = os.environ.get("PCG_FOLD_THIN", "1") != "0"

    def __init__(self, main):
        super().__init__()
        self.main = main
        self._blocks = None

    def forward(self, input):
        self._ensure_flat()
        if self._blocks is None:
            self._blocks = _compile(self.main)
        flat_in = input.dim() == 2
        if flat_in:
# ... 156 lines not shown
    @in_conv_precision
    def _run_forward_groups(self, xs, keep=True):
        G = len(xs)
        B, H, W, C = xs[0].shape
        saved = []
        a = None
        xf = None
        for idx, b in enumerate(self._blocks):
            c = b.conv
            w = _w_ohwi(c.weight.data)
            bias = c.bias.data if c.bias is not None else None
            mean = invstd = z = None
            xf_in, xf = xf, None
            if idx == 0:
                g = ops.conv_geom(B, H, W, c.in_channels, c.out_channels, b.kh, b.kw, b.stride, b.pad)
                y = torch.empty((G * B, g.OH, g.OW, c.out_channels), dtype=torch.float32, device=xs[0].device)
                for k, x in enumerate(xs):
                    ops.conv2d_fwd(g, x, w, bias, out=y[k * B:(k + 1) * B], act=b.act, slope=b.slope)
                a_in = tuple(xs)
            else:
                g = ops.conv_geom(G * B, H, W, c.in_channels, c.out_channels, b.kh, b.kw, b.stride, b.pad)
                a_in = a
                if b.bn is not None and b.bn.training:
                    bn = b.bn
                    z, mean, invstd = ops.conv_bn_train_g(g, a, w, bias, bn.eps, bn.momentum, bn.running_mean, bn.running_var,
                                                          bn.num_batches_tracked, G)
                    if self._next_reads_bn_input(idx, G * B, g.OH, g.OW, G):
                        y, xf = None, ops.BnInput(mean, invstd, bn.weight.data, bn.bias.data, b.act, b.slope, G)
                    else:
                        y = ops.bn_apply_act_g(z, c.out_channels, mean, invstd, bn.weight.data, bn.bias.data, b.act, b.slope, G)
                elif b.bn is not None:
                    bn = b.bn
                    z = ops.conv2d_fwd(g, a, w, bias)
                    y = ops.bn_apply_act(z, c.out_channels, bn.running_mean, bn.running_var, bn.weight.data, bn.bias.data, b.act, b.slope,
                                         var_eps=bn.eps, out=z)
                    z = None
                else:
                    y = ops.conv2d_fwd(g, a, w, bias, act=b.act, slope=b.slope, xf=xf_in)
            if xf_in is not None and (idx == 0 or b.bn is not None):
                raise PcgError("grouped forward: a BatchNorm input reached a layer that cannot read it")
            if keep:
                saved.append((g, a_in, z, mean, invstd, y, b.bn is not None and not b.bn.training, xf_in))
            a, H, W = (y if xf is None else z), g.OH, g.OW
        return a, (saved, G, B)

    @in_conv_precision
    def _run_backward_groups(self, saved_all, dy):
        saved, G, B = saved_all
        if not dy.is_contiguous():
            dy = dy.contiguous()
        d, own = dy, False
        fused = None
        defer = self._defer()
        try:
            with ops.slab_reductions_deferred(self.defer_slab_reductions and defer is None):
                self._run_backward_groups_impl(saved, G, B, d, own, fused, defer)
        finally:
            if defer is not None:
                defer.finish()

    def _run_backward_groups_impl(self, saved, G, B, d, own, fused, defer):
        for idx in range(len(self._blocks) - 1, -1, -1):
            b = self._blocks[idx]
            g, a, z, mean, invstd, y, bn_eval, xf_in = saved[idx]
            c = b.conv
            C = c.out_channels
            if defer is not None:
                defer.start_pending()
            if b.bn is not None:
                if bn_eval:
                    raise PcgError("backward through an eval-mode BatchNorm2d is not implemented")
                bn = b.bn
                dg = db = None
                acc = False
                if bn.weight.requires_grad:
                    dg, acc = self._grad_view(bn.weight)
                    db, _ = self._grad_view(bn.bias)
                if fused is not None and fused[0] == "done":
                    dz = d
                elif fused is not None:
                    dz = ops.bn_bwd_partial_g(d, z, C, mean, invstd, bn.weight.data, fused[1], fused[2], fused[3], dg, db, acc, G, out=d)
                else:
                    dz = ops.bn_act_bwd_g(d, z, C, mean, invstd, bn.weight.data, bn.bias.data, b.act, b.slope, dg, db, acc, G,
                                          out=d if own else None)
            elif fused is not None or b.act == ACT_NONE:
                dz = d
            else:
                dz = ops.act_bwd(d, y, b.act, b.slope, out=d if own else None)
            own = True
            if c.weight.requires_grad:
                gw, acc = self._grad_view(c.weight)
                gw = _w_ohwi(gw)

                def wgrad_job(idx=idx, g=g, a=a, dz=dz, gw=gw, acc=acc, c=c, C=C, xf_in=xf_in):
                    if idx == 0:
                        for k, x in enumerate(a):
                            ops.conv2d_wgrad(g, x, dz[k * B:(k + 1) * B], gw, acc or k > 0)
                    else:
                        ops.conv2d_wgrad(g, a, dz, gw, acc, xf_x=xf_in)
                    if c.bias is not None and c.bias.requires_grad:
                        gb, accb = self._grad_view(c.bias)
                        ops.colsum(dz.numel() // C, C, dz, gb, accb)
                if defer is not None:
                    defer.join()
                if defer is not None and idx > 0 and g.Cin > 3 and g.Cout > 3:
                    defer.submit(wgrad_job, (dz, a))
                else:
                    wgrad_job()
            elif defer is not None:
                defer.join()
            if idx == 0:
                return None
            lo = self._blocks[idx - 1]
            _, _, zl, ml, il, yl, lo_eval, _ = saved[idx - 1]
            w = _w_ohwi(c.weight.data)
            fused = None
            mfma = g.Cin > 3 and g.Cout > 3 and g.Cin % 4 == 0 and g.Cout % 4 == 0 and g.stride <= 2
            if self.fuse_backward_epilogue and mfma and lo.act in (ACT_NONE, ACT_RELU, ACT_LRELU):
                if lo.bn is not None and not lo_eval and zl is not None and ops.group_dgrad_ok(g, G):
                    d, partial, nparts, nphases = ops.conv_bwd_data_fused_g(g, dz, w, lo.act, lo.slope, zl,
                                                                            (ml, il, lo.bn.weight.data, lo.bn.bias.data), G)
                    fused = ("bn", partial, nparts, nphases)
                    continue
                if lo.bn is None and lo.act != ACT_NONE:
                    res = ops.conv_bwd_data_fused(g, dz, w, False, lo.act, lo.slope, a_below=yl)
                    if res is not None:
                        d, fused = res[0], ("mask",)
                        continue
            if (self.fuse_backward_epilogue and lo.bn is not None and lo.act in (ACT_NONE, ACT_RELU, ACT_LRELU) and not lo_eval and zl is not None
                    and lo.bn.weight.requires_grad and self.fuse_full_window_bn and ops.full_dgrad_bn_bwd_ok(g, G)):
                dgl, accl = self._grad_view(lo.bn.weight)
                dbl, _ = self._grad_view(lo.bn.bias)
                d = ops.full_dgrad_bn_bwd(g, dz, w, zl, ml, il, lo.bn.weight.data, lo.bn.bias.data, lo.act, lo.slope, dgl, dbl, accl, groups=G)
                fused = ("done",)
                continue
            d = ops.conv2d_dgrad(g, dz, w)

    defer_slab_reductions = False

    fuse_full_window_bn = True

    wgrad_stream = None

    wgrad_overlap = None

    def _defer(self):
        if self.wgrad_overlap != "bn":
            return None
        side = self.__dict__.get("_overlap_stream")
        if side is None:
            side = self.__dict__["_overlap_stream"] = torch.cuda.Stream()
        return _WgradDefer(side, torch.cuda.current_stream())

    @in_conv_precision
    def _run_backward(self, saved, dy, need_x, need_p):
        if not dy.is_contiguous():
            dy = dy.contiguous()
        side = self.wgrad_stream
        main = torch.cuda.current_stream() if side is not None else None
        defer = self._defer() if side is None else None
        try:
            with ops.slab_reductions_deferred(self.defer_slab_reductions and side is None and defer is None):
                return self._run_backward_impl(saved, dy, need_x, need_p, side, main, defer)
        finally:
            if side is not None:
                main.wait_stream(side)
            if defer is not None:
                defer.finish()

    def _run_backward_impl(self, saved, dy, need_x, need_p, side, main, defer=None):
        d = dy
        own = False
        nblk = len(self._blocks)
        fused = None
        for idx in range(nblk - 1, -1, -1):
            b = self._blocks[idx]
            g, a, z, mean, invstd, y, bn_eval, xf_in = saved[idx]
            c = b.conv
            C = c.out_channels
            if defer is not None:
                defer.start_pending()
            if b.bn is not None:
                if bn_eval:
                    raise PcgError("backward through an eval-mode BatchNorm2d is not implemented")
                bn = b.bn
                dg = db = None
                acc = False
                if need_p and bn.weight.requires_grad:
                    dg, acc = self._grad_view(bn.weight)
                    db, acc2 = self._grad_view(bn.bias)
                    if acc != acc2:
                        raise PcgError("inconsistent .grad state on BatchNorm weight/bias")
                if fused is not None and fused[0] == "done":
                    dz = d
                elif fused is not None:
                    dz = ops.bn_bwd_partial(d, z, C, mean, invstd, bn.weight.data, fused[1], fused[2], dg, db, acc, out=d)
                else:
                    dz = ops.bn_act_bwd(d, z, None if b.act in (ACT_RELU, ACT_LRELU) else y, C, mean, invstd, bn.weight.data, b.act, b.slope, dg,
                                        db, acc, beta=bn.bias.data)
            elif fused is not None or b.act == ACT_NONE:
                dz = d
            else:
                dz = ops.act_bwd(d, y, b.act, b.slope, out=d if own else None)
            own = True
            if need_p and c.weight.requires_grad:
                gw, acc = self._grad_view(c.weight)
                gw = _w_ohwi(gw)
                if side is not None:
                    side.wait_stream(main)
                    dz.record_stream(side); a.record_stream(side)

                def wgrad_job(b=b, g=g, a=a, dz=dz, gw=gw, acc=acc, xf_in=xf_in, c=c, C=C):
                    if not b.transposed:
                        ops.conv2d_wgrad(g, a, dz, gw, acc, xf_x=xf_in)
                    else:
                        ops.conv2d_wgrad(g, dz, a, gw, acc, xf_dy=xf_in)
                    if c.bias is not None and c.bias.requires_grad:
                        gb, accb = self._grad_view(c.bias)
                        ops.colsum(dz.numel() // C, C, dz, gb, accb)
                mfma = g.Cin > 3 and g.Cout > 3
                if defer is not None and mfma and idx > 0:
                    defer.join()
                    defer.submit(wgrad_job, (dz, a))
                else:
                    if defer is not None:
                        defer.join()
                    with torch.cuda.stream(side) if side is not None else contextlib.nullcontext():
                        wgrad_job()
            elif defer is not None:
                defer.join()
            last = idx == 0
            if last and not need_x:
                return None
            fused = None
            if not last and self.fuse_backward_epilogue:
                lo = self._blocks[idx - 1]
                _, _, zl, ml, il, yl, lo_eval, _ = saved[idx - 1]
                w = _w_ohwi(c.weight.data)
                res = None
                if lo.act in (ACT_NONE, ACT_RELU, ACT_LRELU) and not (b.transposed and b.flat):
                    if lo.bn is not None and not lo_eval and zl is not None:
                        res = ops.conv_bwd_data_fused(g, dz, w, b.transposed, lo.act, lo.slope, z_below=zl,
                                                      bn=(ml, il, lo.bn.weight.data, lo.bn.bias.data))
                        if res is not None:
                            d, fused = res[0], ("bn", res[1], res[2])
                    elif lo.bn is None and lo.act != ACT_NONE:
                        res = ops.conv_bwd_data_fused(g, dz, w, b.transposed, lo.act, lo.slope, a_below=yl)
                        if res is not None:
                            d, fused = res[0], ("mask",)
                if res is not None:
                    continue
            if not b.transposed:
                lo = self._blocks[idx - 1] if not last else None
                if (lo is not None and self.fuse_backward_epilogue and lo.bn is not None and lo.act in (ACT_NONE, ACT_RELU, ACT_LRELU)
                        and not saved[idx - 1][6] and saved[idx - 1][2] is not None
                        and self.fuse_full_window_bn and ops.full_dgrad_bn_bwd_ok(g)):
                    _, _, zl, ml, il, _, _, _ = saved[idx - 1]
                    dgl = dbl = None
                    accl = False
                    if need_p and lo.bn.weight.requires_grad:
                        dgl, accl = self._grad_view(lo.bn.weight)
                        dbl, _ = self._grad_view(lo.bn.bias)
                    d = ops.full_dgrad_bn_bwd(g, dz, _w_ohwi(c.weight.data), zl, ml, il, lo.bn.weight.data, lo.bn.bias.data, lo.act, lo.slope,
                                              dgl, dbl, accl)
                    fused = ("done",)
                    continue
                d = ops.conv2d_dgrad(g, dz, _w_ohwi(c.weight.data))
            else:
                lo = self._blocks[idx - 1] if not last else None
                if (lo is not None and self.fuse_backward_epilogue and lo.bn is not None and lo.act in (ACT_NONE, ACT_RELU, ACT_LRELU)
                        and not saved[idx - 1][6] and saved[idx - 1][2] is not None and lo.bn.weight.requires_grad and need_p
                        and ops.thin_fwd_bn_bwd_ok(g)):
                    _, _, zl, ml, il, _, _, _ = saved[idx - 1]
                    dgl, accl = self._grad_view(lo.bn.weight)
                    dbl, _ = self._grad_view(lo.bn.bias)
                    d = ops.thin_fwd_bn_bwd(g, dz, _w_ohwi(c.weight.data), zl, ml, il, lo.bn.weight.data, lo.bn.bias.data, lo.act, lo.slope,
# ... 290 lines not shown
```

### promptable-counterfactual-gan_amd/ops.py

```python
import ctypes
import threading

import torch

from . import _lib
from ._lib import ACT_LRELU, ACT_NONE, ACT_RELU, ACT_SIGMOID, ACT_TANH, ConvGeom, check

_ws_cache = {}

_conv_hook = None


def set_conv_hook(hook):
    global _conv_hook
    _conv_hook = hook


def _conv_label(g, op):
    if g.Cin <= 3 or g.Cout <= 3:
        return f"thin_{op}"
    if op == "wgrad":
        n = g.KH * g.KW * g.Cin
        if g.Cout <= 64:
            return "conv_wgrad192_kernel<64x192>" if (n % 192 == 0 and n % 128 != 0) else "conv_wgrad_kernel<64x128>"
# ... 466 lines not shown
    return "bf16" if _lib.load().pcg_conv_precision_get() == 1 else "fp32"


_slab_defer = threading.local()
_SLAB_SLOT0 = 16


class slab_reductions_deferred:

    def __init__(self, enabled=True):
        self.enabled = enabled and not getattr(_slab_defer, "on", False)

    def __enter__(self):
        if self.enabled:
            check(_lib.load().pcg_slab_defer_begin(_stream()), "pcg_slab_defer_begin")
            _slab_defer.on, _slab_defer.n = True, 0
        return self

    def __exit__(self, et, ev, tb):
        if self.enabled:
            _slab_defer.on = False
            rc = _lib.load().pcg_slab_defer_flush(_stream())
            if et is None:
                check(rc, "pcg_slab_defer_flush")
        return False


def conv2d_wgrad(g, x, dy, dw, accumulate, xf_x=None, xf_dy=None):
    _chk(x, "x"); _chk(dy, "dy"); _chk(dw, "dw")
    assert dw.numel() == g.Cout * g.KH * g.KW * g.Cin
    lib = _lib.load()
    need = lib.pcg_conv2d_wgrad_workspace_bytes(ctypes.byref(g))
    if getattr(_slab_defer, "on", False):
        ws = _scratch(_SLAB_SLOT0 + _slab_defer.n, need, x.device)
        _slab_defer.n += 1
    else:
        ws = workspace(need, x.device)
    if g.Cin > 3 and g.Cout > 3 and _pixtab_key(g, x.device.index) not in _pixtabs:
        prepare_conv_pixtab(g, x.device)
    with _Timed(g, "wgrad"):
        if isinstance(xf_x, BnInput):
            check(lib.pcg_conv2d_wgrad_bnin_full(ctypes.byref(g), _p(x), _p(xf_x.mean), _p(xf_x.invstd), _p(xf_x.gamma), _p(xf_x.beta), xf_x.act,
                                                 xf_x.slope, xf_x.groups, _p(dy), _p(dw), int(bool(accumulate)), _p(ws), ws.numel(), _stream()),
                  "pcg_conv2d_wgrad_bnin_full")
        elif xf_x is None and xf_dy is None:
            check(lib.pcg_conv2d_wgrad(ctypes.byref(g), _p(x), _p(dy), _p(dw), int(bool(accumulate)), _p(ws), ws.numel(), _stream()),
                  "pcg_conv2d_wgrad")
        else:
            check(lib.pcg_conv2d_wgrad_xf(ctypes.byref(g), _p(x), _xref(xf_x), _p(dy), _xref(xf_dy), _p(dw), int(bool(accumulate)), _p(ws),
                                          ws.numel(), _stream()), "pcg_conv2d_wgrad_xf")
    return dw


def colsum(dy2d_rows, C, dy, db, accumulate):
    lib = _lib.load()
    need = lib.pcg_colsum_workspace_bytes(dy2d_rows, C)
    ws = workspace(need, dy.device)
    check(lib.pcg_colsum(_p(dy), dy2d_rows, C, _p(db), int(bool(accumulate)), _p(ws), ws.numel(), _stream()), "pcg_colsum")
    return db


def bn_train_stats(x, C, eps, momentum, running_mean=None, running_var=None, num_batches_tracked=None, gamma=None, beta=None):
    _chk(x, "x")
    rows = x.numel() // C
    mean = torch.empty(C, dtype=torch.float32, device=x.device)
    invstd = torch.empty(C, dtype=torch.float32, device=x.device)
    coef = torch.empty(2 * C, dtype=torch.float32, device=x.device) if gamma is not None else None
    lib = _lib.load()
    ws = workspace(lib.pcg_bn_workspace_bytes(rows, C), x.device)
    check(lib.pcg_bn_train_stats_coef(_p(x), rows, C, eps, momentum, _p(mean), _p(invstd), _p(running_mean), _p(running_var),
                                      _p(num_batches_tracked), _p(gamma), _p(beta), _p(coef), _p(ws), ws.numel(), _stream()),
          "pcg_bn_train_stats")
    return (mean, invstd, coef) if gamma is not None else (mean, invstd)


def bn_apply_act(x, C, mean, invstd_or_var, gamma, beta, act, slope=0.0, var_eps=-1.0, out=None, residual=None, alpha=1.0):
    _chk(x, "x")
    y = out if out is not None else torch.empty_like(x)
    check(_lib.load().pcg_bn_apply_act(_p(x), x.numel() // C, C, _p(mean), _p(invstd_or_var), var_eps, _p(gamma), _p(beta),
                                       act, slope, _p(residual), alpha, _p(y), _stream()), "pcg_bn_apply_act")
    return y


def bn_act_bwd(dy, x, y, C, mean, invstd, gamma, act, slope, dgamma, dbeta, accumulate, out=None, dy_scale=1.0, beta=None, dcol=None,
               accumulate_col=False):
    _chk(dy, "dy"); _chk(x, "x")
    if y is not None:
        _chk(y, "y")
    rows = x.numel() // C
    dx = out if out is not None else torch.empty_like(x)
    lib = _lib.load()
    if dcol is not None:
        premask = y is None and act in (ACT_RELU, ACT_LRELU)
        if premask and beta is None:
            raise _lib.PcgError("bn_act_bwd: pass y, or beta to recompute the activation mask")
        ws = workspace(lib.pcg_bn_db_workspace_bytes(rows, C), x.device)
        check(lib.pcg_bn_act_bwd_db(_p(dy), _p(x), _p(y), rows, C, _p(mean), _p(invstd), _p(gamma), _p(beta if premask else None), act, slope,
                                    dy_scale, _p(dx), _p(dgamma), _p(dbeta), int(bool(accumulate)), _p(dcol), int(bool(accumulate_col)),
                                    _p(ws), ws.numel(), _stream()), "pcg_bn_act_bwd_db")
        return dx
    ws = workspace(lib.pcg_bn_workspace_bytes(rows, C), x.device)
    if y is None and act in (ACT_RELU, ACT_LRELU):
        if beta is None:
            raise _lib.PcgError("bn_act_bwd: pass y, or beta to recompute the activation mask")
        check(lib.pcg_bn_act_bwd_premask(_p(dy), _p(x), rows, C, _p(mean), _p(invstd), _p(gamma), _p(beta), act, slope, dy_scale, _p(dx),
                                         _p(dgamma), _p(dbeta), int(bool(accumulate)), _p(ws), ws.numel(), _stream()), "pcg_bn_act_bwd_premask")
# ... 1651 lines not shown
```

Before: 53440.

## Fuse BN backward apply into conv wgrad kernel as a rider

```diff
diff --git a/include/pcgan_hip.h b/include/pcgan_hip.h
--- a/include/pcgan_hip.h
+++ b/include/pcgan_hip.h
@@ -172,6 +172,25 @@
 int pcg_bn_bwd_partial_g(const float* dm, const float* x, int64_t rows, int32_t C, const float* mean, const float* invstd,
                          const float* gamma, const void* partial, int32_t nparts, int32_t nphases, float* dx, float* dgamma,
                          float* dbeta, int accumulate, int32_t groups, void* workspace, size_t workspace_bytes, pcg_stream_t stream);
+#define PCG_RIDER_NOT_CARRIED 1
+typedef struct pcg_bn_apply_rider {
+  const float* dm; const float* x; float* dx;
+  int64_t rows; int32_t C; int32_t groups;
+  const float* mean; const float* invstd;
+  const float* coef;
+} pcg_bn_apply_rider;
+int pcg_bn_bwd_partial_finalize(int64_t rows, int32_t C, const float* mean, const float* invstd, const float* gamma, const void* partial,
+                                int32_t nparts, float* dgamma, float* dbeta, int accumulate, void* workspace, size_t workspace_bytes,
+                                pcg_stream_t stream);
+int pcg_bn_bwd_partial_finalize_g(int64_t rows, int32_t C, const float* mean, const float* invstd, const float* gamma,
+                                  const void* partial, int32_t nparts, int32_t nphases, float* dgamma, float* dbeta, int accumulate,
+                                  int32_t groups, void* workspace, size_t workspace_bytes, pcg_stream_t stream);
+int pcg_bn_bwd_apply_coef(const pcg_bn_apply_rider* r, pcg_stream_t stream);
+int pcg_conv2d_wgrad_rider(const pcg_conv_geom* g, const float* x, const float* dy, float* dw, int accumulate,
+                           const pcg_bn_apply_rider* rider, void* workspace, size_t workspace_bytes, pcg_stream_t stream);
+int32_t pcg_conv2d_wgrad_rider_mode(void);
+int32_t pcg_conv2d_wgrad_rider_ok(const pcg_conv_geom* g, pcg_stream_t stream);
+int pcg_bn_rider_share(uint64_t n4, int32_t C, uint32_t grid, uint32_t b, uint64_t* first, uint64_t* count);
 size_t pcg_bn_act_bwd_g_workspace_bytes(int64_t rows, int32_t C, int32_t groups);
 int pcg_bn_act_bwd_premask_g(const float* dy, const float* x, int64_t rows, int32_t C, const float* mean, const float* invstd,
                              const float* gamma, const float* beta, int act, float slope, float* dx, float* dgamma, float* dbeta,
diff --git a/promptable-counterfactual-gan_amd/_lib.py b/promptable-counterfactual-gan_amd/_lib.py
--- a/promptable-counterfactual-gan_amd/_lib.py
+++ b/promptable-counterfactual-gan_amd/_lib.py
@@ -53,6 +53,11 @@
     _fields_ = ([(n, _P) for n in ("params", "grads", "onehot", "mask", "H", "Z1", "Z2", "SM", "soft", "d_cont", "d_logits", "d_samples",
                                    "DH", "DZ1", "DZ2", "A1", "DN1", "DG", "DB", "DZIN", "DL", "DC", "Q")] +
                 [("B", ctypes.c_int32), ("accumulate", ctypes.c_int32), ("tau", ctypes.c_float), ("res_scale", ctypes.c_float)])
+
+
+class BnApplyRider(ctypes.Structure):
+    _fields_ = ([(n, _P) for n in ("dm", "x", "dx")] + [("rows", ctypes.c_int64), ("C", _I), ("groups", _I)] +
+                [(n, _P) for n in ("mean", "invstd", "coef")])
 
 
 class InXform(ctypes.Structure):
@@ -254,7 +259,7 @@
 CLASS_PICK_KMAX = 64
 CF_PANELS_GRID, CF_PANELS_PANELS = 0, 1
 
-STRUCTS = {"pcg_conv_geom": ConvGeom, "pcg_in_xform": InXform, "pcg_wgrad_item": WgradItem, "pcg_sn_fwd_batch": SnFwdBatch,
+STRUCTS = {"pcg_conv_geom": ConvGeom, "pcg_in_xform": InXform, "pcg_bn_apply_rider": BnApplyRider, "pcg_wgrad_item": WgradItem, "pcg_sn_fwd_batch": SnFwdBatch,
            "pcg_sn_bwd_batch": SnBwdBatch, "pcg_house_g_desc": HouseGDesc, "pcg_house_g_fwd_args": HouseGFwdArgs,
            "pcg_house_g_bwd_args": HouseGBwdArgs, "pcg_house_critic_fwd_args": HouseCriticFwdArgs,
            "pcg_house_critic_bwd_args": HouseCriticBwdArgs, "pcg_house_cls_fwd_args": HouseClsFwdArgs, "pcg_house_cls_bwd_args": HouseClsBwdArgs,
@@ -382,6 +387,13 @@
     "pcg_dp_shutdown": (_i, []),
     "pcg_conv2d_wgrad_workspace_bytes": (_sz, [_gp]),
     "pcg_conv2d_wgrad": (_i, [_gp, _vp, _vp, _vp, _i, _vp, _sz, _vp]),
+    "pcg_conv2d_wgrad_rider": (_i, [_gp, _vp, _vp, _vp, _i, _c.POINTER(BnApplyRider), _vp, _sz, _vp]),
+    "pcg_bn_bwd_partial_finalize": (_i, [_i64, _i32, _vp, _vp, _vp, _vp, _i32, _vp, _vp, _i, _vp, _sz, _vp]),
+    "pcg_bn_bwd_partial_finalize_g": (_i, [_i64, _i32, _vp, _vp, _vp, _vp, _i32, _i32, _vp, _vp, _i, _i32, _vp, _sz, _vp]),
+    "pcg_bn_bwd_apply_coef": (_i, [_c.POINTER(BnApplyRider), _vp]),
+    "pcg_conv2d_wgrad_rider_mode": (_i32, []),
+    "pcg_conv2d_wgrad_rider_ok": (_i32, [_gp, _vp]),
+    "pcg_bn_rider_share": (_i, [_c.c_uint64, _i32, _c.c_uint32, _c.c_uint32, _c.POINTER(_c.c_uint64), _c.POINTER(_c.c_uint64)]),
     "pcg_colsum_workspace_bytes": (_sz, [_i64, _c.c_int32]),
     "pcg_colsum": (_i, [_vp, _i64, _c.c_int32, _vp, _i, _vp, _sz, _vp]),
     "pcg_bn_workspace_bytes": (_sz, [_i64, _c.c_int32]),
diff --git a/promptable-counterfactual-gan_amd/csrc/batchnorm.hip b/promptable-counterfactual-gan_amd/csrc/batchnorm.hip
--- a/promptable-counterfactual-gan_amd/csrc/batchnorm.hip
+++ b/promptable-counterfactual-gan_amd/csrc/batchnorm.hip
@@ -1,5 +1,6 @@
 #include "pcg_common.h"
 #include "launch_plan.h"
+#include "bn_apply_share.h"
 #include <cstdlib>
 
 namespace pcg {
@@ -411,12 +412,6 @@
 }
 static bool bn_use_nt(size_t n4) { const BnTune& t = bn_tune(); return t.nt < 0 ? n4 * 16 >= t.nt_bytes : t.nt != 0; }
 static int bn_apply_depth() { return bn_tune().depth == 4 ? 4 : 2; }
-template <bool NT>
-__device__ __forceinline__ void bn_store4(float4* at, const float4& v) {
-  typedef float nt_f32x4 __attribute__((ext_vector_type(4)));
-  if constexpr (NT) __builtin_nontemporal_store(nt_f32x4{v.x, v.y, v.z, v.w}, reinterpret_cast<nt_f32x4*>(at)); else *at = v;
-}
-
 template <int DEPTH, bool NT>
 __global__ void __launch_bounds__(256) bn_apply_act_fast_kernel(const float4* __restrict__ x, size_t n4, int C,
                                                                 const float* __restrict__ mean, const float* __restrict__ invstd,
@@ -481,45 +476,12 @@
     mean += g * C; invstd += g * C; coef += g * 3 * C; n4 = group_n4;
   }
   const size_t gtid = (size_t)blockIdx.x * 256 + threadIdx.x, stride = (size_t)gridDim.x * 256;
-  const int c0 = (int)(gtid % (size_t)(C >> 2)) * 4;
-  float mu[4], is[4], k0[4], k1[4], k2[4], msc[4], msh[4];
   double cs[4] = {0.0, 0.0, 0.0, 0.0};
-  const bool premask = act != PCG_ACT_NONE && y == nullptr;
-#pragma unroll
-  for (int e = 0; e < 4; ++e) {
-    const int c = c0 + e;
-    mu[e] = mean[c]; is[e] = invstd[c]; k0[e] = coef[c]; k1[e] = coef[C + c]; k2[e] = coef[2 * C + c];
-    msc[e] = 0.f; msh[e] = 0.f;
-    if (premask) bn_fold(gamma[c], beta[c], mean[c], invstd[c], msc[e], msh[e]);
-  }
-  const bool has_act = act != PCG_ACT_NONE;
-  auto one = [&](float4 g, float4 xv, float4 yv) {
-    float gg[4] = {g.x, g.y, g.z, g.w}, xx[4] = {xv.x, xv.y, xv.z, xv.w}, yy[4] = {yv.x, yv.y, yv.z, yv.w};
-#pragma unroll
-    for (int e = 0; e < 4; ++e) {
-      if (premask) yy[e] = fmaf(xx[e], msc[e], msh[e]);
-      const float grad = has_act ? act_grad_from_out(yy[e], act, slope) : 1.f;
-      const float xh = (xx[e] - mu[e]) * is[e];
-      gg[e] = k0[e] * fmaf(-xh, k2[e], fmaf(dy_scale * gg[e], grad, -k1[e]));
-    }
-    return make_float4(gg[0], gg[1], gg[2], gg[3]);
-  };
-  const float4 ones = make_float4(1.f, 1.f, 1.f, 1.f);
-  auto tally = [&](const float4& v) { cs[0] += (double)v.x; cs[1] += (double)v.y; cs[2] += (double)v.z; cs[3] += (double)v.w; };
-  size_t i = gtid;
-  for (; i + stride < n4; i += 2 * stride) {
-    const float4 g0 = dy[i], g1 = dy[i + stride], x0 = x[i], x1 = x[i + stride];
-    const float4 y0 = (has_act && !premask) ? y[i] : ones, y1 = (has_act && !premask) ? y[i + stride] : ones;
-    const float4 o0 = one(g0, x0, y0), o1 = one(g1, x1, y1);
-    bn_store4<NT>(dx + i, o0);
-    bn_store4<NT>(dx + i + stride, o1);
-    if (colpart) { tally(o0); tally(o1); }
-  }
-  if (i < n4) {
-    const float4 o = one(dy[i], x[i], (has_act && !premask) ? y[i] : ones);
-    bn_store4<NT>(dx + i, o);
-    if (colpart) tally(o);
-  }
+  if (colpart)
+    bn_bwd_apply_range<NT>(dy, x, y, dx, 0, n4, stride, gtid, C, mean, invstd, coef, act, slope, dy_scale, gamma, beta,
+                           [&](const float4& v) { cs[0] += (double)v.x; cs[1] += (double)v.y; cs[2] += (double)v.z; cs[3] += (double)v.w; });
+  else
+    bn_bwd_apply_range<NT>(dy, x, y, dx, 0, n4, stride, gtid, C, mean, invstd, coef, act, slope, dy_scale, gamma, beta);
   if (colpart) {
     __shared__ double red[4][256];
 #pragma unroll
@@ -584,6 +546,8 @@
 }
 
 }
+bool bn_apply_fast_channels(int C) { return fast_channels(C); }
+bool bn_apply_use_nt(size_t n4) { return bn_use_nt(n4); }
 }
 
 namespace pcg {
@@ -789,11 +753,11 @@
 static int bn_bwd_partial_impl(const float* dm, const float* x, int64_t rows, int32_t C, const float* mean, const float* invstd,
                                const float* gamma, const void* partial_, int32_t nparts, float* dx, float* dgamma, float* dbeta,
                                int accumulate, void* workspace, size_t workspace_bytes, pcg_stream_t stream, float* dcol,
-                               int accumulate_col, float dm_scale = 1.f) {
+                               int accumulate_col, float dm_scale = 1.f, bool apply = true) {
   const double* partial = static_cast<const double*>(partial_);
   PCG_REQUIRE(!dcol || workspace_bytes >= pcg_bn_bwd_partial_db_workspace_bytes(C),
               "pcg_bn_bwd_partial_db: workspace smaller than pcg_bn_bwd_partial_db_workspace_bytes");
-  PCG_REQUIRE(dm && x && mean && invstd && partial && dx && rows > 0 && C > 0 && nparts > 0, "pcg_bn_bwd_partial: bad arguments");
+  PCG_REQUIRE((!apply || (dm && x && dx)) && mean && invstd && partial && rows > 0 && C > 0 && nparts > 0, "pcg_bn_bwd_partial: bad arguments");
   PCG_REQUIRE(((uintptr_t)partial & 7) == 0, "pcg_bn_bwd_partial: the partial-sum buffer must be 8-byte aligned");
   if (!workspace || workspace_bytes < pcg_bn_bwd_partial_workspace_bytes(C)) {
     set_error("pcg_bn_bwd_partial: workspace %zu B < required %zu B", workspace_bytes, pcg_bn_bwd_partial_workspace_bytes(C));
@@ -816,6 +780,7 @@
   hipLaunchKernelGGL(bn_bwd_finalize_kernel<double>, dim3((C + FIN_CH - 1) / FIN_CH), dim3(fin_threads(nsrc)), 0, s, src, nsrc, C,
                      1.0 / (double)rows_all, gamma, invstd, coef, dgamma, dbeta, accumulate, local);
   if (int e = launch_status("bn_bwd_finalize_kernel")) return e;
+  if (!apply) return PCG_OK;
   const bool aligned = al16(dm) && al16(x) && al16(dx);
   const size_t n = (size_t)rows * C;
   double* colpart = reinterpret_cast<double*>(reinterpret_cast<char*>(workspace) + (((size_t)3 * C * sizeof(float) + 7) & ~(size_t)7));
@@ -856,6 +821,12 @@
   return bn_bwd_partial_impl(dm, x, rows, C, mean, invstd, gamma, partial, nparts, dx, dgamma, dbeta, accumulate, workspace, workspace_bytes,
                              stream, nullptr, 0);
 }
+extern "C" int pcg_bn_bwd_partial_finalize(int64_t rows, int32_t C, const float* mean, const float* invstd, const float* gamma, const void* partial,
+                                           int32_t nparts, float* dgamma, float* dbeta, int accumulate, void* workspace, size_t workspace_bytes,
+                                           pcg_stream_t stream) {
+  return bn_bwd_partial_impl(nullptr, nullptr, rows, C, mean, invstd, gamma, partial, nparts, nullptr, dgamma, dbeta, accumulate, workspace,
+                             workspace_bytes, stream, nullptr, 0, 1.f, false);
+}
 extern "C" int pcg_bn_bwd_partial_db(const float* dm, const float* x, int64_t rows, int32_t C, const float* mean, const float* invstd,
                                      const float* gamma, const void* partial, int32_t nparts, float dm_scale, float* dx, float* dgamma,
                                      float* dbeta, int accumulate, float* dcol, int accumulate_col, void* workspace,
@@ -919,11 +890,12 @@
 static int launch_bwd_finalize_apply_g(const float* dm, const float* x, int64_t rows, int32_t C, const float* mean, const float* invstd,
                                        const float* gamma, const float* beta, int act, float slope, const double* partial, int rpg, int seg,
                                        int seg_stride, float* dx, float* dgamma, float* dbeta, int accumulate, int32_t groups, float* coef,
-                                       hipStream_t s) {
+                                       hipStream_t s, bool apply = true) {
   const int64_t rows_g = rows / groups;
   hipLaunchKernelGGL(bn_bwd_finalize_g_kernel<double>, dim3((C + FIN_CH - 1) / FIN_CH), dim3(fin_threads(rpg)), 0, s, partial, rpg, groups, seg,
                      seg_stride, C, 1.0 / (double)rows_g, gamma, invstd, coef, dgamma, dbeta, accumulate);
   if (int e = launch_status("bn_bwd_finalize_g_kernel")) return e;
+  if (!apply) return PCG_OK;
   const size_t n4g = (size_t)rows_g * C / 4;
   launch_bn_bwd_apply_fast(dim3(grouped_apply_blocks(n4g), groups), s, n4g * groups, reinterpret_cast<const float4*>(dm),
                            reinterpret_cast<const float4*>(x), (const float4*)nullptr, n4g, C, mean, invstd, (const float*)coef, act, slope, 1.f,
@@ -931,24 +903,65 @@
   return launch_status("bn_bwd_apply_fast_kernel");
 }
 
-extern "C" int pcg_bn_bwd_partial_g(const float* dm, const float* x, int64_t rows, int32_t C, const float* mean, const float* invstd,
-                                    const float* gamma, const void* partial_, int32_t nparts, int32_t nphases, float* dx, float* dgamma,
-                                    float* dbeta, int accumulate, int32_t groups, void* workspace, size_t workspace_bytes, pcg_stream_t stream) {
+static int bn_bwd_partial_g_impl(const char* who, const float* dm, const float* x, int64_t rows, int32_t C, const float* mean, const float* invstd,
+                                 const float* gamma, const void* partial_, int32_t nparts, int32_t nphases, float* dx, float* dgamma,
+                                 float* dbeta, int accumulate, int32_t groups, void* workspace, size_t workspace_bytes, pcg_stream_t stream, bool apply) {
   const double* partial = static_cast<const double*>(partial_);
-  PCG_REQUIRE(dm && x && mean && invstd && partial && dx && nparts > 0 && nphases > 0, "pcg_bn_bwd_partial_g: bad arguments");
+  PCG_REQUIRE((!apply || (dm && x && dx)) && mean && invstd && partial && nparts > 0 && nphases > 0, "%s: bad arguments", who);
   PCG_REQUIRE(grouped_shape_ok(rows, C, groups) && al16(dm) && al16(x) && al16(dx) && ((uintptr_t)partial & 7) == 0,
-              "pcg_bn_bwd_partial_g: needs rows %% groups == 0, C / 4 a power of two <= 256 and aligned tensors (rows %lld, C %d, groups %d)",
+              "%s: needs rows %% groups == 0, C / 4 a power of two <= 256 and aligned tensors (rows %lld, C %d, groups %d)", who,
               (long long)rows, C, groups);
-  PCG_REQUIRE(nparts % (nphases * groups) == 0, "pcg_bn_bwd_partial_g: %d partial rows do not split into %d phases x %d groups", nparts, nphases, groups);
-  PCG_REQUIRE(!dp_sync_bn(), "pcg_bn_bwd_partial_g: not available in the exact global-batch mode");
+  PCG_REQUIRE(nparts % (nphases * groups) == 0, "%s: %d partial rows do not split into %d phases x %d groups", who, nparts, nphases, groups);
+  PCG_REQUIRE(!dp_sync_bn(), "%s: not available in the exact global-batch mode", who);
   if (!workspace || workspace_bytes < pcg_bn_bwd_partial_g_workspace_bytes(C, groups)) {
-    set_error("pcg_bn_bwd_partial_g: workspace %zu B < required %zu B", workspace_bytes, pcg_bn_bwd_partial_g_workspace_bytes(C, groups));
+    set_error("%s: workspace %zu B < required %zu B", who, workspace_bytes, pcg_bn_bwd_partial_g_workspace_bytes(C, groups));
     return PCG_ERR_WORKSPACE;
   }
   int per_phase = nparts / nphases, seg = per_phase / groups;
   (void)launch_presum_g(&partial, nparts, 2 * C, &per_phase, &seg, (hipStream_t)stream);
   return launch_bwd_finalize_apply_g(dm, x, rows, C, mean, invstd, gamma, nullptr, PCG_ACT_NONE, 0.f, partial, seg * nphases, seg, per_phase, dx,
-                                     dgamma, dbeta, accumulate, groups, (float*)workspace, (hipStream_t)stream);
+                                     dgamma, dbeta, accumulate, groups, (float*)workspace, (hipStream_t)stream, apply);
+}
+extern "C" int pcg_bn_bwd_partial_g(const float* dm, const float* x, int64_t rows, int32_t C, const float* mean, const float* invstd,
+                                    const float* gamma, const void* partial, int32_t nparts, int32_t nphases, float* dx, float* dgamma,
+                                    float* dbeta, int accumulate, int32_t groups, void* workspace, size_t workspace_bytes, pcg_stream_t stream) {
+  return bn_bwd_partial_g_impl("pcg_bn_bwd_partial_g", dm, x, rows, C, mean, invstd, gamma, partial, nparts, nphases, dx, dgamma, dbeta, accumulate,
+                               groups, workspace, workspace_bytes, stream, true);
+}
+extern "C" int pcg_bn_bwd_partial_finalize_g(int64_t rows, int32_t C, const float* mean, const float* invstd, const float* gamma,
+                                             const void* partial, int32_t nparts, int32_t nphases, float* dgamma, float* dbeta, int accumulate,
+                                             int32_t groups, void* workspace, size_t workspace_bytes, pcg_stream_t stream) {
+  return bn_bwd_partial_g_impl("pcg_bn_bwd_partial_finalize_g", nullptr, nullptr, rows, C, mean, invstd, gamma, partial, nparts, nphases, nullptr,
+                               dgamma, dbeta, accumulate, groups, workspace, workspace_bytes, stream, false);
+}
+
+extern "C" int pcg_bn_bwd_apply_coef(const pcg_bn_apply_rider* r, pcg_stream_t stream) {
+  PCG_REQUIRE(r && r->dm && r->x && r->dx && r->mean && r->invstd && r->coef && r->rows > 0 && r->C > 0 && r->groups >= 1,
+              "pcg_bn_bwd_apply_coef: bad arguments");
+  hipStream_t s = (hipStream_t)stream;
+  const bool aligned = al16(r->dm) && al16(r->x) && al16(r->dx);
+  const int C = r->C;
+  if (r->groups > 1) {
+    PCG_REQUIRE(grouped_shape_ok(r->rows, C, r->groups) && aligned, "pcg_bn_bwd_apply_coef: grouped form needs rows %% groups == 0, C / 4 a power of two <= 256 and aligned tensors");
+    const size_t n4g = (size_t)(r->rows / r->groups) * C / 4;
+    launch_bn_bwd_apply_fast(dim3(grouped_apply_blocks(n4g), r->groups), s, n4g * r->groups, reinterpret_cast<const float4*>(r->dm),
+                             reinterpret_cast<const float4*>(r->x), (const float4*)nullptr, n4g, C, r->mean, r->invstd, r->coef, (int)PCG_ACT_NONE, 0.f, 1.f,
+                             reinterpret_cast<float4*>(r->dx), (const float*)nullptr, (const float*)nullptr, (double*)nullptr, n4g);
+    return launch_status("bn_bwd_apply_fast_kernel");
+  }
+  const size_t n = (size_t)r->rows * C;
+  const ApplyPlan ap = plan_apply(BN_PASS_BWD, r->rows, C, aligned);
+  if (ap.lanes == BN_LANES_FAST)
+    launch_bn_bwd_apply_fast(dim3(ap.blocks), s, n / 4, reinterpret_cast<const float4*>(r->dm), reinterpret_cast<const float4*>(r->x),
+                             (const float4*)nullptr, n / 4, C, r->mean, r->invstd, r->coef, (int)PCG_ACT_NONE, 0.f, 1.f,
+                             reinterpret_cast<float4*>(r->dx), (const float*)nullptr, (const float*)nullptr, (double*)nullptr, (size_t)0);
+  else if (ap.lanes == BN_LANES_FLOAT4)
+    hipLaunchKernelGGL(bn_bwd_apply_kernel<4>, dim3(ap.blocks), dim3(256), 0, s, r->dm, r->x, (const float*)nullptr, n, C, r->mean, r->invstd,
+                       r->coef, PCG_ACT_NONE, 0.f, 1.f, r->dx, (const float*)nullptr, (const float*)nullptr);
+  else
+    hipLaunchKernelGGL(bn_bwd_apply_kernel<1>, dim3(ap.blocks), dim3(256), 0, s, r->dm, r->x, (const float*)nullptr, n, C, r->mean, r->invstd,
+                       r->coef, PCG_ACT_NONE, 0.f, 1.f, r->dx, (const float*)nullptr, (const float*)nullptr);
+  return launch_status("bn_bwd_apply_kernel");
 }
 
 extern "C" size_t pcg_bn_act_bwd_g_workspace_bytes(int64_t rows, int32_t C, int32_t groups) {
diff --git a/promptable-counterfactual-gan_amd/csrc/bn_apply_share.h b/promptable-counterfactual-gan_amd/csrc/bn_apply_share.h
--- /dev/null
+++ b/promptable-counterfactual-gan_amd/csrc/bn_apply_share.h
@@ -0,0 +1,86 @@
+#pragma once
+#include "pcg_common.h"
+
+namespace pcg {
+
+template <bool NT>
+__device__ __forceinline__ void bn_store4(float4* at, const float4& v) {
+  typedef float nt_f32x4 __attribute__((ext_vector_type(4)));
+  if constexpr (NT) __builtin_nontemporal_store(nt_f32x4{v.x, v.y, v.z, v.w}, reinterpret_cast<nt_f32x4*>(at)); else *at = v;
+}
+
+struct BnNoSink { __device__ __forceinline__ void operator()(const float4&) const {} };
+
+template <bool NT, class Sink = BnNoSink>
+__device__ __forceinline__ void bn_bwd_apply_range(const float4* __restrict__ dy, const float4* __restrict__ x, const float4* __restrict__ y,
+                                                   float4* __restrict__ dx, size_t first, size_t count, size_t stride, size_t t, int C,
+                                                   const float* __restrict__ mean, const float* __restrict__ invstd,
+                                                   const float* __restrict__ coef, int act, float slope, float dy_scale,
+                                                   const float* __restrict__ gamma, const float* __restrict__ beta, Sink sink = Sink{}) {
+  const int c0 = (int)(t % (size_t)(C >> 2)) * 4;
+  float mu[4], is[4], k0[4], k1[4], k2[4], msc[4], msh[4];
+  const bool premask = act != PCG_ACT_NONE && y == nullptr;
+#pragma unroll
+  for (int e = 0; e < 4; ++e) {
+    const int c = c0 + e;
+    mu[e] = mean[c]; is[e] = invstd[c]; k0[e] = coef[c]; k1[e] = coef[C + c]; k2[e] = coef[2 * C + c];
+    msc[e] = 0.f; msh[e] = 0.f;
+    if (premask) bn_fold(gamma[c], beta[c], mean[c], invstd[c], msc[e], msh[e]);
+  }
+  const bool has_act = act != PCG_ACT_NONE;
+  auto one = [&](float4 g, float4 xv, float4 yv) {
+    float gg[4] = {g.x, g.y, g.z, g.w}, xx[4] = {xv.x, xv.y, xv.z, xv.w}, yy[4] = {yv.x, yv.y, yv.z, yv.w};
+#pragma unroll
+    for (int e = 0; e < 4; ++e) {
+      if (premask) yy[e] = fmaf(xx[e], msc[e], msh[e]);
+      const float grad = has_act ? act_grad_from_out(yy[e], act, slope) : 1.f;
+      const float xh = (xx[e] - mu[e]) * is[e];
+      gg[e] = k0[e] * fmaf(-xh, k2[e], fmaf(dy_scale * gg[e], grad, -k1[e]));
+    }
+    return make_float4(gg[0], gg[1], gg[2], gg[3]);
+  };
+  const float4 ones = make_float4(1.f, 1.f, 1.f, 1.f);
+  const size_t end = first + count;
+  size_t i = first + t;
+  for (; i + stride < end; i += 2 * stride) {
+    const float4 g0 = dy[i], g1 = dy[i + stride], x0 = x[i], x1 = x[i + stride];
+    const float4 y0 = (has_act && !premask) ? y[i] : ones, y1 = (has_act && !premask) ? y[i + stride] : ones;
+    const float4 o0 = one(g0, x0, y0), o1 = one(g1, x1, y1);
+    bn_store4<NT>(dx + i, o0);
+    bn_store4<NT>(dx + i + stride, o1);
+    sink(o0); sink(o1);
+  }
+  if (i < end) {
+    const float4 o = one(dy[i], x[i], (has_act && !premask) ? y[i] : ones);
+    bn_store4<NT>(dx + i, o);
+    sink(o);
+  }
+}
+
+struct BnApplyRider {
+  const float* dm; const float* x; float* dx;
+  const float* mean; const float* invstd; const float* coef;
+  unsigned long long n4, group_n4;
+  unsigned per, rem;
+  int groups, C, nt, pad_;
+};
+__host__ __device__ inline unsigned long long bn_share_start(unsigned b, unsigned per, unsigned rem, int C) {
+  return ((unsigned long long)b * per + (b < rem ? b : rem)) * (unsigned long long)(C >> 2);
+}
+
+__device__ __forceinline__ void bn_apply_rider_share(const BnApplyRider& r, unsigned b, unsigned t, unsigned nthreads) {
+  const size_t first = bn_share_start(b, r.per, r.rem, r.C), end = bn_share_start(b + 1, r.per, r.rem, r.C);
+  for (int g = 0; g < r.groups; ++g) {
+    const size_t g0 = (size_t)g * r.group_n4, g1 = g0 + r.group_n4;
+    const size_t lo = first > g0 ? first : g0, hi = end < g1 ? end : g1;
+    if (lo >= hi) continue;
+    const float4* dm = reinterpret_cast<const float4*>(r.dm);
+    const float4* x = reinterpret_cast<const float4*>(r.x);
+    float4* dx = reinterpret_cast<float4*>(r.dx);
+    const float* mean = r.mean + (size_t)g * r.C, *invstd = r.invstd + (size_t)g * r.C, *coef = r.coef + (size_t)g * 3 * r.C;
+    if (r.nt) bn_bwd_apply_range<true>(dm, x, dm, dx, lo, hi - lo, nthreads, t, r.C, mean, invstd, coef, PCG_ACT_NONE, 0.f, 1.f, nullptr, nullptr);
+    else bn_bwd_apply_range<false>(dm, x, dm, dx, lo, hi - lo, nthreads, t, r.C, mean, invstd, coef, PCG_ACT_NONE, 0.f, 1.f, nullptr, nullptr);
+  }
+}
+
+}
diff --git a/promptable-counterfactual-gan_amd/csrc/conv_igemm.hip b/promptable-counterfactual-gan_amd/csrc/conv_igemm.hip
--- a/promptable-counterfactual-gan_amd/csrc/conv_igemm.hip
+++ b/promptable-counterfactual-gan_amd/csrc/conv_igemm.hip
@@ -6,6 +6,7 @@
 #include "conv_pixtab.h"
 #include "conv_cliptab.h"
 #include "thin_conv.h"
+#include "bn_apply_share.h"
 
 namespace pcg {
 namespace {
@@ -335,10 +336,25 @@
   dgrad_sk_segment<Cfg, XF>(p, phases, sk, s1, tiles_per_phase, smem, rowpix);
 }
 
+constexpr int WGRAD_RIDER_SHIFT = 1;
+constexpr int WGRAD_RIDER_DEFAULT = 1;
+template <class Cfg, bool XFA, bool XFB>
+constexpr bool wgrad_carries_rider = !Cfg::BF16 && !XFA && !XFB;
+__device__ __forceinline__ unsigned wgrad_linear_block() { return blockIdx.y * gridDim.x + blockIdx.x; }
 template <class Cfg, bool XFA, bool XFB, bool TAB = false>
 __global__ void __launch_bounds__(IG_THREADS, 4) conv_wgrad_kernel(ConvP p, int ktiles_total, int ktiles_per_split, int tiles,
-                                                                   int slice_major) {
+                                                                   int flags, BnApplyRider rider) {
   extern __shared__ __attribute__((aligned(16))) float smem[];
+  const int slice_major = flags & 1;
+  bool ride_after = false;
+  if constexpr (wgrad_carries_rider<Cfg, XFA, XFB>) {
+    const int mode = flags >> WGRAD_RIDER_SHIFT;
+    if (mode) {
+      const unsigned b = wgrad_linear_block(), G = gridDim.x * gridDim.y;
+      if (mode == 2 || b < G / 2) bn_apply_rider_share(rider, b, threadIdx.x, IG_THREADS);
+      else ride_after = true;
+    }
+  }
   prio_entry(p);
   uint32_t tile, split;
   if (slice_major) {
@@ -358,16 +374,22 @@
     WgradALoader<Cfg::BM, XFA> la(p, m_block, kt_begin, tid);
     WgradBLoader<Cfg::BN, XFB, TAB> lb(p, n_block, kt_begin, tid);
     igemm_produce<Cfg>(la, lb, ktiles, smem, tid, ClockStamp{p.stamps, p.stamp_slots});
-    return;
-  }
-  f32x16 acc[Cfg::TM][Cfg::TN];
-  igemm_consume<Cfg, false, false>(ktiles, acc, smem, ClockStamp{p.stamps, p.stamp_slots});
-  prio_epilogue(p);
-  float* slab = p.out + (size_t)split * (size_t)p.M * (size_t)p.N;
-  igemm_store_tile<Cfg>(acc, smem, n_block, p.N, nullptr, [&](int row) -> float* {
-    const int m = m_block + row;
-    return m < p.M ? slab + (size_t)m * p.N + n_block : nullptr;
-  });
+  } else {
+    f32x16 acc[Cfg::TM][Cfg::TN];
+    igemm_consume<Cfg, false, false>(ktiles, acc, smem, ClockStamp{p.stamps, p.stamp_slots});
+    prio_epilogue(p);
+    float* slab = p.out + (size_t)split * (size_t)p.M * (size_t)p.N;
+    igemm_store_tile<Cfg>(acc, smem, n_block, p.N, nullptr, [&](int row) -> float* {
+      const int m = m_block + row;
+      return m < p.M ? slab + (size_t)m * p.N + n_block : nullptr;
+    });
+  }
+  if constexpr (wgrad_carries_rider<Cfg, XFA, XFB>) {
+    if (ride_after) {
+      __builtin_amdgcn_s_setprio(0);
+      bn_apply_rider_share(rider, wgrad_linear_block(), threadIdx.x, IG_THREADS);
+    }
+  }
 }
 
 
@@ -582,7 +604,7 @@
   return PCG_OK;
 }
 
-struct Tune { int edge_prio = -1, dgrad_swz3 = -1, wgrad_rounds = -1, korder = -1, wgrad_order = -1, dgrad_interleave = -1, fwd_splits = -1, stream_k = -1, sk_blocks = -1, dgrad_gemm = -1, t64 = -1, wgrad_pixtab = -1, pad_clip = -1, pad_clip_dgrad = -1; unsigned long long* stamps = nullptr; int stamp_slots = 0; };
+struct Tune { int edge_prio = -1, dgrad_swz3 = -1, wgrad_rounds = -1, korder = -1, wgrad_order = -1, dgrad_interleave = -1, fwd_splits = -1, stream_k = -1, sk_blocks = -1, dgrad_gemm = -1, t64 = -1, wgrad_pixtab = -1, pad_clip = -1, pad_clip_dgrad = -1, wgrad_rider = -1; unsigned long long* stamps = nullptr; int stamp_slots = 0; };
 Tune g_tune;
 
 ConvP make_params(const pcg_conv_geom* g) {
@@ -1672,15 +1694,25 @@
 }
 
 template <class Cfg, bool XFA, bool XFB, bool TAB = false>
-static int launch_wgrad_x(const ConvP& p, const WgradPlan& wp, int slice_major, hipStream_t s) {
+static int launch_wgrad_x(const ConvP& p, const WgradPlan& wp, int slice_major, hipStream_t s, const BnApplyRider* rider = nullptr, int rider_mode = 0) {
   if constexpr (!TAB) {
-    if (p.pixtab) return launch_wgrad_x<Cfg, XFA, XFB, true>(p, wp, slice_major, s);
+    if (p.pixtab) return launch_wgrad_x<Cfg, XFA, XFB, true>(p, wp, slice_major, s, rider, rider_mode);
+  }
+  BnApplyRider r{};
+  int flags = slice_major ? 1 : 0;
+  if (rider) {
+    PCG_REQUIRE((wgrad_carries_rider<Cfg, XFA, XFB>), "conv_wgrad_kernel: this instantiation carries no rider");
+    r = *rider;
+    const unsigned G = (unsigned)wp.tiles * (unsigned)wp.splits;
+    const unsigned long long nrows = r.n4 / (unsigned long long)(r.C >> 2);
+    r.per = (unsigned)(nrows / G); r.rem = (unsigned)(nrows % G);
+    flags |= rider_mode << WGRAD_RIDER_SHIFT;
   }
   constexpr size_t smem = smem_bytes<Cfg, false, false>();
   static int once = set_smem(conv_wgrad_kernel<Cfg, XFA, XFB, TAB>, smem);
   if (once != PCG_OK) return once;
   hipLaunchKernelGGL((conv_wgrad_kernel<Cfg, XFA, XFB, TAB>), slice_major ? dim3((unsigned)wp.tiles * wp.splits) : dim3((unsigned)wp.tiles, wp.splits),
-                     dim3(IG_THREADS), smem, s, p, wp.ktiles_total, wp.ktiles_per_split, wp.tiles, slice_major);
+                     dim3(IG_THREADS), smem, s, p, wp.ktiles_total, wp.ktiles_per_split, wp.tiles, flags, r);
   return launch_status("conv_wgrad_kernel");
 }
 template <class Cfg, bool XFA, bool XFB, bool TAB = false>
@@ -1710,22 +1742,25 @@
   return launch_status("conv_wgrad192_kernel");
 }
 template <class Cfg>
-static int launch_wgrad(const ConvP& p, const WgradPlan& wp, int slice_major, int xf_side, hipStream_t s) {
+static int launch_wgrad(const ConvP& p, const WgradPlan& wp, int slice_major, int xf_side, hipStream_t s, const BnApplyRider* rider = nullptr,
+                        int rider_mode = 0) {
   if constexpr (!Cfg::BF16) {
     if (conv_bf16()) return launch_wgrad<Bf16Twin<Cfg>>(p, wp, slice_major, xf_side, s);
   }
   if (xf_side == 1) return launch_wgrad_x<Cfg, false, true>(p, wp, slice_major, s);
   if (xf_side == 2) return launch_wgrad_x<Cfg, true, false>(p, wp, slice_major, s);
-  return launch_wgrad_x<Cfg, false, false>(p, wp, slice_major, s);
-}
-
-extern "C" int pcg_conv2d_wgrad_xf(const pcg_conv_geom* g, const float* x, const pcg_in_xform* xf_x, const float* dy,
-                                   const pcg_in_xform* xf_dy, float* dw, int accumulate, void* workspace, size_t workspace_bytes,
-                                   pcg_stream_t stream) {
+  return launch_wgrad_x<Cfg, false, false>(p, wp, slice_major, s, rider, rider_mode);
+}
+
+namespace pcg { bool bn_apply_fast_channels(int C); bool bn_apply_use_nt(size_t n4); }
+static int wgrad_impl(const pcg_conv_geom* g, const float* x, const pcg_in_xform* xf_x, const float* dy, const pcg_in_xform* xf_dy, float* dw,
+                      int accumulate, void* workspace, size_t workspace_bytes, pcg_stream_t stream, const BnApplyRider* rider) {
   if (int e = check_geom(g)) return e;
   PCG_REQUIRE(x && dy && dw, "pcg_conv2d_wgrad: null pointer");
   const bool hx = xf_x && xf_x->scale, hy = xf_dy && xf_dy->scale;
   PCG_REQUIRE(!(hx && hy), "pcg_conv2d_wgrad_xf: at most one operand can carry an input transform");
+  const int rider_mode = pcg_conv2d_wgrad_rider_mode();
+  if (rider && (thin_is_cin(g) || thin_is_cout(g) || rider_mode == 0 || conv_bf16())) return PCG_RIDER_NOT_CARRIED;
   if (thin_is_cin(g) || thin_is_cout(g)) {
     PCG_REQUIRE(!hx && (!hy || thin_conv_xf_ok(g)), "pcg_conv2d_wgrad: input transforms on the MFMA path (Cin > 3 and Cout > 3) and, on the dy side, on the thin forms of pcg_conv2d_xf_thin_ok only");
     PCG_REQUIRE(!hy || (xf_dy->act == PCG_ACT_NONE || xf_dy->act == PCG_ACT_RELU || xf_dy->act == PCG_ACT_LRELU), "pcg_conv2d_wgrad: transform activation %d", hy ? xf_dy->act : 0);
@@ -1755,6 +1790,7 @@
     SkPlan sk{};
     bool take = plan_sk(wp.tiles, wp.ktiles_total, s, &sk);
     if (!take && wp.splits == 1) { sk = SkPlan{wp.tiles, 0, 0, wp.ktiles_total, nullptr, nullptr}; take = true; }
+    if (take && rider) return PCG_RIDER_NOT_CARRIED;
     if (take) {
       p.out = dw;
       if (accumulate) { p.epi.mode = EPI_ADD; p.epi.neg = 1.f; p.epi.delta_bytes = 0; }
@@ -1763,6 +1799,7 @@
     }
   }
   int rc;
+  if (rider && wp.wide192) return PCG_RIDER_NOT_CARRIED;
   if (wp.wide192 && side == 0) {
     p.tilesN = p.N / 192;
     rc = conv_bf16() ? launch_wgrad192<Bf16Twin<Cfg64x192>>(p, wp, slice_major, s) : launch_wgrad192<Cfg64x192>(p, wp, slice_major, s);
@@ -1772,11 +1809,58 @@
       wq.wide192 = false;
       wq.tiles = ceil_div(p.M, 64) * ceil_div(p.N, 128);
     }
-    rc = wq.narrow ? launch_wgrad<TileCfg<64, 128, 1, 4>>(p, wq, slice_major, side, s) : launch_wgrad<Cfg128x128>(p, wq, slice_major, side, s);
+    rc = wq.narrow ? launch_wgrad<TileCfg<64, 128, 1, 4>>(p, wq, slice_major, side, s, rider, rider_mode)
+                   : launch_wgrad<Cfg128x128>(p, wq, slice_major, side, s, rider, rider_mode);
   }
   if (rc != PCG_OK) return rc;
   const size_t n = (size_t)p.M * p.N;
   return launch_slab_reduce((const float*)workspace, dw, n, n, wp.splits, accumulate, s, true);
+}
+
+extern "C" int pcg_conv2d_wgrad_xf(const pcg_conv_geom* g, const float* x, const pcg_in_xform* xf_x, const float* dy,
+                                   const pcg_in_xform* xf_dy, float* dw, int accumulate, void* workspace, size_t workspace_bytes,
+                                   pcg_stream_t stream) {
+  return wgrad_impl(g, x, xf_x, dy, xf_dy, dw, accumulate, workspace, workspace_bytes, stream, nullptr);
+}
+
+static bool rider_shape_ok(const pcg_bn_apply_rider* r) {
+  return r->rows > 0 && r->groups >= 1 && r->groups <= 8 && r->rows % r->groups == 0 && bn_apply_fast_channels(r->C) &&
+         (((uintptr_t)r->dm | (uintptr_t)r->x | (uintptr_t)r->dx) & 15) == 0;
+}
+extern "C" int pcg_conv2d_wgrad_rider(const pcg_conv_geom* g, const float* x, const float* dy, float* dw, int accumulate,
+                                      const pcg_bn_apply_rider* rider, void* workspace, size_t workspace_bytes, pcg_stream_t stream) {
+  PCG_REQUIRE(rider && rider->dm && rider->x && rider->dx && rider->mean && rider->invstd && rider->coef, "pcg_conv2d_wgrad_rider: null pointer");
+  PCG_REQUIRE(rider->rows > 0 && rider->C > 0 && rider->groups >= 1 && rider->rows % rider->groups == 0,
+              "pcg_conv2d_wgrad_rider: rows %lld, C %d, groups %d", (long long)rider->rows, rider->C, rider->groups);
+  if (!rider_shape_ok(rider)) return PCG_RIDER_NOT_CARRIED;
+  BnApplyRider r{};
+  r.dm = rider->dm; r.x = rider->x; r.dx = rider->dx; r.mean = rider->mean; r.invstd = rider->invstd; r.coef = rider->coef;
+  r.n4 = (unsigned long long)rider->rows * (unsigned)rider->C / 4; r.group_n4 = r.n4 / (unsigned)rider->groups;
+  r.groups = rider->groups; r.C = rider->C; r.nt = bn_apply_use_nt((size_t)r.n4) ? 1 : 0;
+  return wgrad_impl(g, x, nullptr, dy, nullptr, dw, accumulate, workspace, workspace_bytes, stream, &r);
+}
+extern "C" int32_t pcg_conv2d_wgrad_rider_mode(void) {
+  if (dp_sync_bn()) return 0;
+  return g_tune.wgrad_rider >= 0 ? g_tune.wgrad_rider : WGRAD_RIDER_DEFAULT;
+}
+extern "C" int32_t pcg_conv2d_wgrad_rider_ok(const pcg_conv_geom* g, pcg_stream_t stream) {
+  if (check_geom(g) != PCG_OK || thin_is_cin(g) || thin_is_cout(g) || g->Cin % 4 || g->Cout % 4) return 0;
+  if (pcg_conv2d_wgrad_rider_mode() == 0 || conv_bf16()) return 0;
+  const WgradPlan wp = plan_wgrad(g);
+  if (wp.wide192) return 0;
+  if (!wp.narrow && wp.tiles > 96 && sk_mode() != 0) {
+    SkPlan sk{};
+    if (plan_sk(wp.tiles, wp.ktiles_total, (hipStream_t)stream, &sk) || wp.splits == 1) return 0;
+  }
+  return 1;
+}
+extern "C" int pcg_bn_rider_share(uint64_t n4, int32_t C, uint32_t grid, uint32_t b, uint64_t* first, uint64_t* count) {
+  PCG_REQUIRE(first && count && grid > 0 && b < grid && bn_apply_fast_channels(C) && n4 % (uint64_t)(C / 4) == 0, "pcg_bn_rider_share: bad arguments");
+  const uint64_t nrows = n4 / (uint64_t)(C / 4);
+  const unsigned per = (unsigned)(nrows / grid), rem = (unsigned)(nrows % grid);
+  *first = bn_share_start(b, per, rem, C);
+  *count = bn_share_start(b + 1, per, rem, C) - *first;
+  return PCG_OK;
 }
 
 extern "C" int pcg_conv2d_wgrad(const pcg_conv_geom* g, const float* x, const float* dy, float* dw, int accumulate,
@@ -1883,6 +1967,10 @@
   else if (!strcmp(name, "dgrad_gemm")) g_tune.dgrad_gemm = value;
   else if (!strcmp(name, "t64")) g_tune.t64 = value;
   else if (!strcmp(name, "wgrad_pixtab")) g_tune.wgrad_pixtab = value;
+  else if (!strcmp(name, "wgrad_rider")) {
+    PCG_REQUIRE(value >= -1 && value <= 2, "pcg_tune_set: wgrad_rider is 0, 1 or 2 (-1: built-in), not %d", (int)value);
+    g_tune.wgrad_rider = value;
+  }
   else if (!strcmp(name, "pad_clip")) g_tune.pad_clip = value;
   else if (!strcmp(name, "pad_clip_dgrad")) {
     PCG_REQUIRE(value >= -1 && value <= 2, "pcg_tune_set: pad_clip_dgrad is 0, 1 or 2 (-1: built-in), not %d", (int)value);
@@ -1890,7 +1978,7 @@
   }
   else {
     set_error("pcg_tune_set: unknown switch '%s' (korder, edge_prio, dgrad_swz3, wgrad_rounds, wgrad_order, dgrad_interleave, fwd_splits, "
-              "stream_k, sk_blocks, dgrad_gemm, t64); the loader switches wgrad_pixtab, pad_clip and pad_clip_dgrad are accepted as well", name);
+              "stream_k, sk_blocks, dgrad_gemm, t64); the loader switches wgrad_pixtab, pad_clip and pad_clip_dgrad and wgrad_rider are accepted as well", name);
     return PCG_ERR_INVALID;
   }
   return PCG_OK;
diff --git a/promptable-counterfactual-gan_amd/csrc/runtime.hip b/promptable-counterfactual-gan_amd/csrc/runtime.hip
--- a/promptable-counterfactual-gan_amd/csrc/runtime.hip
+++ b/promptable-counterfactual-gan_amd/csrc/runtime.hip
@@ -30,7 +30,7 @@
 extern "C" size_t pcg_abi_struct_bytes(const char* name) {
 #define PCG_STRUCT(T) {#T, sizeof(T)}
   static const struct { const char* name; size_t bytes; } table[] = {
-      PCG_STRUCT(pcg_conv_geom), PCG_STRUCT(pcg_in_xform), PCG_STRUCT(pcg_wgrad_item), PCG_STRUCT(pcg_sn_fwd_batch), PCG_STRUCT(pcg_sn_bwd_batch),
+      PCG_STRUCT(pcg_conv_geom), PCG_STRUCT(pcg_in_xform), PCG_STRUCT(pcg_bn_apply_rider), PCG_STRUCT(pcg_wgrad_item), PCG_STRUCT(pcg_sn_fwd_batch), PCG_STRUCT(pcg_sn_bwd_batch),
       PCG_STRUCT(pcg_house_g_desc), PCG_STRUCT(pcg_house_g_fwd_args), PCG_STRUCT(pcg_house_g_bwd_args), PCG_STRUCT(pcg_house_critic_fwd_args),
       PCG_STRUCT(pcg_house_critic_bwd_args), PCG_STRUCT(pcg_house_cls_fwd_args), PCG_STRUCT(pcg_house_cls_bwd_args),
       PCG_STRUCT(pcg_house_res_fwd_args), PCG_STRUCT(pcg_house_res_bwd_args), PCG_STRUCT(pcg_house_loss_args), PCG_STRUCT(pcg_house_diag_args),
diff --git a/promptable-counterfactual-gan_amd/nn.py b/promptable-counterfactual-gan_amd/nn.py
--- a/promptable-counterfactual-gan_amd/nn.py
+++ b/promptable-counterfactual-gan_amd/nn.py
@@ -302,6 +302,23 @@
             self.join()
             fn()
         self.join()
+
+
+class _WgradRide:
+
+    def __init__(self):
+        self.job = None
+
+    def take(self):
+        job, self.job = self.job, None
+        return job
+
+
+def _wgrad_with_rider(job, rider, d):
+    if not job(rider=rider, dm=d):
+        job()
+        rider.dm = rider.dx = d.data_ptr()
+        ops.bn_bwd_apply_coef(rider)
 
 
 class _SeqFn(torch.autograd.Function):
@@ -564,14 +581,15 @@
         d, own = dy, False
         fused = None
         defer = self._defer()
+        ride = self._ride(None, defer)
         try:
             with ops.slab_reductions_deferred(self.defer_slab_reductions and defer is None):
-                self._run_backward_groups_impl(saved, G, B, d, own, fused, defer)
+                self._run_backward_groups_impl(saved, G, B, d, own, fused, defer, ride)
         finally:
             if defer is not None:
                 defer.finish()
 
-    def _run_backward_groups_impl(self, saved, G, B, d, own, fused, defer):
+    def _run_backward_groups_impl(self, saved, G, B, d, own, fused, defer, ride=None):
         for idx in range(len(self._blocks) - 1, -1, -1):
             b = self._blocks[idx]
             g, a, z, mean, invstd, y, bn_eval, xf_in = saved[idx]
@@ -579,6 +597,10 @@
             C = c.out_channels
             if defer is not None:
                 defer.start_pending()
+            held = ride.take() if ride is not None else None
+            if held is not None and not (b.bn is not None and not bn_eval and fused is not None and fused[0] == "bn"):
+                held()
+                held = None
             if b.bn is not None:
                 if bn_eval:
                     raise PcgError("backward through an eval-mode BatchNorm2d is not implemented")
@@ -589,6 +611,10 @@
                     dg, acc = self._grad_view(bn.weight)
                     db, _ = self._grad_view(bn.bias)
                 if fused is not None and fused[0] == "done":
+                    dz = d
+                elif held is not None:
+                    _wgrad_with_rider(held, ops.bn_bwd_partial_finalize(z, C, mean, invstd, bn.weight.data, fused[1], fused[2], dg, db, acc,
+                                                                        groups=G, nphases=fused[3]), d)
                     dz = d
                 elif fused is not None:
                     dz = ops.bn_bwd_partial_g(d, z, C, mean, invstd, bn.weight.data, fused[1], fused[2], fused[3], dg, db, acc, G, out=d)
@@ -604,8 +630,11 @@
                 gw, acc = self._grad_view(c.weight)
                 gw = _w_ohwi(gw)
 
-                def wgrad_job(idx=idx, g=g, a=a, dz=dz, gw=gw, acc=acc, c=c, C=C, xf_in=xf_in):
-                    if idx == 0:
+                def wgrad_job(idx=idx, g=g, a=a, dz=dz, gw=gw, acc=acc, c=c, C=C, xf_in=xf_in, rider=None, dm=None):
+                    if rider is not None:
+                        if not ops.conv2d_wgrad_rider(g, a, dz, gw, acc, rider, dm, dm):
+                            return False
+                    elif idx == 0:
                         for k, x in enumerate(a):
                             ops.conv2d_wgrad(g, x, dz[k * B:(k + 1) * B], gw, acc or k > 0)
                     else:
@@ -613,10 +642,13 @@
                     if c.bias is not None and c.bias.requires_grad:
                         gb, accb = self._grad_view(c.bias)
                         ops.colsum(dz.numel() // C, C, dz, gb, accb)
+                    return True
                 if defer is not None:
                     defer.join()
                 if defer is not None and idx > 0 and g.Cin > 3 and g.Cout > 3:
                     defer.submit(wgrad_job, (dz, a))
+                elif ride is not None and idx > 0 and xf_in is None and self._ride_expected(idx, g, saved):
+                    ride.job = wgrad_job
                 else:
                     wgrad_job()
             elif defer is not None:
@@ -656,6 +688,20 @@
 
     wgrad_overlap = None
 
+    wgrad_rider = True
+
+    def _ride(self, side, defer):
+        if (not self.wgrad_rider or side is not None or defer is not None or self.defer_slab_reductions or not self.fuse_backward_epilogue
+                or ops.wgrad_rider_mode() == 0):
+            return None
+        return _WgradRide()
+
+    def _ride_expected(self, idx, g, saved):
+        lo = self._blocks[idx - 1]
+        return (g.Cin > 3 and g.Cout > 3 and g.Cin % 4 == 0 and g.Cout % 4 == 0 and lo.bn is not None and lo.bn.training
+                and lo.act in (ACT_NONE, ACT_RELU, ACT_LRELU) and saved[idx - 1][2] is not None and not saved[idx - 1][6]
+                and ops.wgrad_rider_ok(g, lo.conv.out_channels))
+
     def _defer(self):
         if self.wgrad_overlap != "bn":
             return None
@@ -671,16 +717,17 @@
         side = self.wgrad_stream
         main = torch.cuda.current_stream() if side is not None else None
         defer = self._defer() if side is None else None
+        ride = self._ride(side, defer)
         try:
             with ops.slab_reductions_deferred(self.defer_slab_reductions and side is None and defer is None):
-                return self._run_backward_impl(saved, dy, need_x, need_p, side, main, defer)
+                return self._run_backward_impl(saved, dy, need_x, need_p, side, main, defer, ride)
         finally:
             if side is not None:
                 main.wait_stream(side)
             if defer is not None:
                 defer.finish()
 
-    def _run_backward_impl(self, saved, dy, need_x, need_p, side, main, defer=None):
+    def _run_backward_impl(self, saved, dy, need_x, need_p, side, main, defer=None, ride=None):
         d = dy
         own = False
         nblk = len(self._blocks)
@@ -692,6 +739,10 @@
             C = c.out_channels
             if defer is not None:
                 defer.start_pending()
+            held = ride.take() if ride is not None else None
+            if held is not None and not (b.bn is not None and not bn_eval and fused is not None and fused[0] == "bn"):
+                held()
+                held = None
             if b.bn is not None:
                 if bn_eval:
                     raise PcgError("backward through an eval-mode BatchNorm2d is not implemented")
@@ -704,6 +755,9 @@
                     if acc != acc2:
                         raise PcgError("inconsistent .grad state on BatchNorm weight/bias")
                 if fused is not None and fused[0] == "done":
+                    dz = d
+                elif held is not None:
+                    _wgrad_with_rider(held, ops.bn_bwd_partial_finalize(z, C, mean, invstd, bn.weight.data, fused[1], fused[2], dg, db, acc), d)
                     dz = d
                 elif fused is not None:
                     dz = ops.bn_bwd_partial(d, z, C, mean, invstd, bn.weight.data, fused[1], fused[2], dg, db, acc, out=d)
@@ -722,18 +776,26 @@
                     side.wait_stream(main)
                     dz.record_stream(side); a.record_stream(side)
 
-                def wgrad_job(b=b, g=g, a=a, dz=dz, gw=gw, acc=acc, xf_in=xf_in, c=c, C=C):
-                    if not b.transposed:
+                def wgrad_job(b=b, g=g, a=a, dz=dz, gw=gw, acc=acc, xf_in=xf_in, c=c, C=C, rider=None, dm=None):
+                    xd = (a, dz) if not b.transposed else (dz, a)
+                    if rider is not None:
+                        if not ops.conv2d_wgrad_rider(g, xd[0], xd[1], gw, acc, rider, dm, dm):
+                            return False
+                    elif not b.transposed:
                         ops.conv2d_wgrad(g, a, dz, gw, acc, xf_x=xf_in)
                     else:
                         ops.conv2d_wgrad(g, dz, a, gw, acc, xf_dy=xf_in)
                     if c.bias is not None and c.bias.requires_grad:
                         gb, accb = self._grad_view(c.bias)
                         ops.colsum(dz.numel() // C, C, dz, gb, accb)
+                    return True
                 mfma = g.Cin > 3 and g.Cout > 3
                 if defer is not None and mfma and idx > 0:
                     defer.join()
                     defer.submit(wgrad_job, (dz, a))
+                elif (ride is not None and idx > 0 and xf_in is None and not (b.transposed and b.flat)
+                      and self._ride_expected(idx, g, saved)):
+                    ride.job = wgrad_job
                 else:
                     if defer is not None:
                         defer.join()
diff --git a/promptable-counterfactual-gan_amd/ops.py b/promptable-counterfactual-gan_amd/ops.py
--- a/promptable-counterfactual-gan_amd/ops.py
+++ b/promptable-counterfactual-gan_amd/ops.py
@@ -542,6 +542,64 @@
     return dw
 
 
+RIDER_NOT_CARRIED = 1
+_RIDER_COEF_SLOT = 3
+
+
+def bn_bwd_partial_finalize(x, C, mean, invstd, gamma, partial, nparts, dgamma, dbeta, accumulate, groups=1, nphases=1):
+    _chk(x, "x")
+    lib = _lib.load()
+    rows = x.numel() // C
+    if groups == 1:
+        ws = _scratch(_RIDER_COEF_SLOT, lib.pcg_bn_bwd_partial_workspace_bytes(C), x.device)
+        check(lib.pcg_bn_bwd_partial_finalize(rows, C, _p(mean), _p(invstd), _p(gamma), _p(partial), int(nparts), _p(dgamma), _p(dbeta),
+                                              int(bool(accumulate)), _p(ws), ws.numel(), _stream()), "pcg_bn_bwd_partial_finalize")
+    else:
+        ws = _scratch(_RIDER_COEF_SLOT, lib.pcg_bn_bwd_partial_g_workspace_bytes(C, int(groups)), x.device)
+        check(lib.pcg_bn_bwd_partial_finalize_g(rows, C, _p(mean), _p(invstd), _p(gamma), _p(partial), int(nparts), int(nphases), _p(dgamma),
+                                                _p(dbeta), int(bool(accumulate)), int(groups), _p(ws), ws.numel(), _stream()),
+              "pcg_bn_bwd_partial_finalize_g")
+    r = _lib.BnApplyRider()
+    r.x, r.rows, r.C, r.groups = x.data_ptr(), rows, C, int(groups)
+    r.mean, r.invstd, r.coef = mean.data_ptr(), invstd.data_ptr(), ws.data_ptr()
+    return r
+
+
+def wgrad_rider_mode():
+    return _lib.load().pcg_conv2d_wgrad_rider_mode()
+
+
+def wgrad_rider_ok(g, C):
+    q = C // 4
+    if C % 4 or q > 256 or q & (q - 1) or getattr(_slab_defer, "on", False):
+        return False
+    _conv_scratch()
+    return bool(_lib.load().pcg_conv2d_wgrad_rider_ok(ctypes.byref(g), _stream()))
+
+
+def bn_bwd_apply_coef(rider):
+    check(_lib.load().pcg_bn_bwd_apply_coef(ctypes.byref(rider), _stream()), "pcg_bn_bwd_apply_coef")
+
+
+def conv2d_wgrad_rider(g, x, dy, dw, accumulate, rider, dm, out):
+    _chk(x, "x"); _chk(dy, "dy"); _chk(dw, "dw"); _chk(dm, "dm"); _chk(out, "out")
+    assert dw.numel() == g.Cout * g.KH * g.KW * g.Cin and dm.numel() == out.numel() == rider.rows * rider.C
+    rider.dm, rider.dx = dm.data_ptr(), out.data_ptr()
+    if getattr(_slab_defer, "on", False):
+        return False
+    lib = _lib.load()
+    ws = workspace(lib.pcg_conv2d_wgrad_workspace_bytes(ctypes.byref(g)), x.device)
+    if g.Cin > 3 and g.Cout > 3 and _pixtab_key(g, x.device.index) not in _pixtabs:
+        prepare_conv_pixtab(g, x.device)
+    with _Timed(g, "wgrad"):
+        rc = lib.pcg_conv2d_wgrad_rider(ctypes.byref(g), _p(x), _p(dy), _p(dw), int(bool(accumulate)), ctypes.byref(rider), _p(ws), ws.numel(),
+                                        _stream())
+    if rc == RIDER_NOT_CARRIED:
+        return False
+    check(rc, "pcg_conv2d_wgrad_rider")
+    return True
+
+
 def colsum(dy2d_rows, C, dy, db, accumulate):
     lib = _lib.load()
     need = lib.pcg_colsum_workspace_bytes(dy2d_rows, C)
```

Result: no change. 53750, median of 6 (+0.6%).
